# AnnaUshnova/tinyrenderder

Hardware: AMD Instinct MI355X
Metric: triangles/sec (+ Mpixels/sec) at 4096x4096; achieved HBM GB/s vs peak (higher is better)
Workload: dtype f64

## Files before the change

### profiles/summarize_rocprof.py

```python
import csv
import re
import glob
import os
import sys
from collections import defaultdict

out = sys.argv[1]


def short(name):
    m = re.search(r"k_raster<(\d)(?:, (\d))?(?:, (true|false))?>", name)
    if m:
        return "k_raster<" + ["flat", "gouraud", "phong", "eye", "checker", "any"][int(m.group(1))] + (", bpp " + m.group(2) if m.group(2) and m.group(2) != "0" else "") + (", all well scaled" if m.group(3) == "true" else "") + ">"
    m = re.search(r"k_shade<(\d)>", name)
    if m:
        return "k_shade<" + ["flat", "gouraud", "phong", "eye", "checker", "any"][int(m.group(1))] + ">"
    for k in ("k_setup", "k_chunk_spine", "k_radix_scan_rows", "k_expand", "k_radix_hist", "k_radix_scatter",
              "k_bounds", "k_make_items", "k_fold_stats", "k_selftest_division"):
        if k in name:
            return k
    return name.split("(")[0][:60]


print("== kernel trace stats (rocprofv3 --kernel-trace --stats) ==")
def newest(pattern):
    files = sorted(glob.glob(pattern, recursive=True), key=os.path.getmtime)
    return files[-1:]


for f in newest(os.path.join(out, "trace", "**", "*kernel_stats.csv")):
    rows = list(csv.DictReader(open(f)))
    print(f"{'kernel':28s} {'calls':>6s} {'total_ms':>10s} {'avg_us':>10s} {'min_us':>10s} {'max_us':>10s} {'%':>6s}")
    for r in rows:
        print(f"{short(r['Name']):28s} {r['Calls']:>6s} {float(r['TotalDurationNs'])/1e6:10.3f} {float(r['AverageNs'])/1e3:10.1f} "
              f"{float(r['MinNs'])/1e3:10.1f} {float(r['MaxNs'])/1e3:10.1f} {float(r['Percentage']):6.2f}")

for f in newest(os.path.join(out, "trace_writeout", "**", "*kernel_stats.csv")):
    print("\n== write-out-only frames at 4096x4096 (profiles/writeout_probe.py 4096: RGB then RGBA framebuffer, 25 frames each) ==")
    for r in csv.DictReader(open(f)):
        if "k_raster" in r["Name"]:
            avg = float(r["AverageNs"])
            print(f"{short(r['Name']):28s} calls {r['Calls']}  avg {avg/1e3:.1f} us  min {float(r['MinNs'])/1e3:.1f} us  -> "
                  f"{4096*4096*11.5/avg:.0f} GB/s average over RGB (11 B/px) and RGBA (12 B/px) frames = {4096*4096*11.5/avg/8000*100:.1f} % of 8 TB/s")
    log = os.path.join(out, "writeout.log")
    if os.path.exists(log):
        print("\n".join(l for l in open(log).read().splitlines() if l[:1].isdigit()))

for tag in ("pmc_fetch", "pmc_write", "pmc_sq"):
    files = newest(os.path.join(out, tag, "**", "*counter_collection.csv"))
    if not files:
        continue
    acc = defaultdict(lambda: defaultdict(list))
    for f in files:
        for r in csv.DictReader(open(f)):
            acc[short(r["Kernel_Name"])][r["Counter_Name"]].append(float(r["Counter_Value"]))
    print(f"\n== {tag}: per-dispatch mean of each counter ==")
    for k, cs in sorted(acc.items()):
        print(f"{k:28s} " + "  ".join(f"{c}={sum(v)/len(v):.4g} (n={len(v)})" for c, v in sorted(cs.items())))

def per_launch(tag, counter, kernel="k_raster"):
    vals = []
    for f in newest(os.path.join(out, tag, "**", "*counter_collection.csv")):
        for r in csv.DictReader(open(f)):
            if kernel in r["Kernel_Name"] and r["Counter_Name"] == counter:
                vals.append(float(r["Counter_Value"]))
    vals = [v for v in vals if v > 0.2 * max(vals)] if vals else vals
    return sum(vals) / len(vals) if vals else None


fetch, write = per_launch("pmc_fetch", "FETCH_SIZE"), per_launch("pmc_write", "WRITE_SIZE")
if fetch and write:
    import json
    traffic = (2.0 * fetch + write) * 1024.0
    print(f"\n== k_raster HBM traffic per launch: FETCH_SIZE={fetch:.4g} KiB (x2 gfx950 wide-read correction), "
          f"WRITE_SIZE={write:.4g} KiB -> {traffic/1e6:.1f} MB ==")
    json.dump({"workload": "c4_4096x4096_10000000", "round": os.path.basename(os.path.normpath(out)).replace("prof_", ""), "raster_hbm_bytes_per_launch": traffic,
               "fetch_size_kib": fetch, "write_size_kib": write,
               "note": "rocprofv3 --pmc FETCH_SIZE / WRITE_SIZE in separate passes; bytes = (2*FETCH_SIZE + WRITE_SIZE)*1024"},
              open(os.path.join(out, "traffic.json"), "w"), indent=1)
```

### tinyrenderder_amd/csrc/kernels_bin.hip

```cpp
#include <hip/hip_runtime.h>
#include "trgl_device.h"
#include "launch.h"

namespace {

__device__ __forceinline__ double dmin3(double a, double b, double c) { double m = a; if (b < m) m = b; if (c < m) m = c; return m; }
__device__ __forceinline__ double dmax3(double a, double b, double c) { double m = a; if (m < b) m = b; if (m < c) m = c; return m; }
__device__ __forceinline__ double dot4(const double* m, const double* v) {
    double sum = 0;
    sum += m[0] * v[0]; sum += m[1] * v[1]; sum += m[2] * v[2]; sum += m[3] * v[3];
    return sum;
}

__device__ __forceinline__ int wave_min_i(int v) {
    for (int o = 32; o; o >>= 1) { int t = __shfl_xor(v, o); v = t < v ? t : v; }
    return v;
}
__device__ __forceinline__ int wave_max_i(int v) {
    for (int o = 32; o; o >>= 1) { int t = __shfl_xor(v, o); v = t > v ? t : v; }
    return v;
}

constexpr int SETUP_THREADS = 256;

__global__ __launch_bounds__(SETUP_THREADS) void k_setup(FrameParams fp, DrawDesc d, DrawDesc* __restrict__ draws_out, int draw_idx,
                                                         TriRec* __restrict__ recs, TriW* __restrict__ recs_w, uint32_t* __restrict__ cnt,
                                                         uint2* __restrict__ tilebox, DevStats* __restrict__ stats,
                                                         uint32_t* __restrict__ blk_sums, uint32_t blk_base) {
    __shared__ __attribute__((aligned(16))) double s_buf[SETUP_THREADS * 16];
    if (blockIdx.x == 0 && threadIdx.x == 0) draws_out[draw_idx] = d;
    const uint32_t b0 = blockIdx.x * SETUP_THREADS;
    const uint32_t nb = min((uint32_t)SETUP_THREADS, d.n - b0);
    const uint32_t tid = threadIdx.x;
    const uint32_t i = b0 + tid;
    const bool in_range = tid < nb;

    const double* src = d.clip + (size_t)b0 * 12;
    if ((reinterpret_cast<uintptr_t>(src) & 15) == 0) {
        const double2* s2 = reinterpret_cast<const double2*>(src);
        double2* l2 = reinterpret_cast<double2*>(s_buf);
        typedef double f64x2 __attribute__((ext_vector_type(2)));
        for (uint32_t k = tid; k < nb * 6; k += SETUP_THREADS)
            *reinterpret_cast<f64x2*>(&l2[k]) = __builtin_nontemporal_load(reinterpret_cast<const f64x2*>(&s2[k]));
    } else {
        for (uint32_t k = tid; k < nb * 12; k += SETUP_THREADS) s_buf[k] = src[k];
    }
    __syncthreads();
    double v[12];
#pragma unroll
    for (int k = 0; k < 12; ++k) v[k] = in_range ? s_buf[tid * 12 + k] : 0.0;
    __syncthreads();

    int bx0 = INT_MAX, by0 = INT_MAX, bx1 = INT_MIN, by1 = INT_MIN;
    uint32_t ntiles = 0;
    bool large = false;
    uint2 tb = make_uint2(0, 0);
    TriRec r;
    {
        uint4* z4 = reinterpret_cast<uint4*>(&r);
#pragma unroll
        for (int k = 0; k < 8; ++k) z4[k] = make_uint4(0, 0, 0, 0);
    }
    if (in_range) {
        bool ok = !(v[3] <= 1e-12 || v[7] <= 1e-12 || v[11] <= 1e-12);
        double ndc[12];
#pragma unroll
        for (int q = 0; q < 3; ++q) {
#pragma unroll
            for (int k = 0; k < 3; ++k) ndc[4 * q + k] = v[4 * q + k] / v[4 * q + 3];
            ndc[4 * q + 3] = __builtin_isfinite(v[4 * q + 3]) ? 1.0 : __builtin_nan("");
        }
        bool zo0 = (ndc[2] < -1.0 || ndc[2] > 1.0), zo1 = (ndc[6] < -1.0 || ndc[6] > 1.0),
             zo2 = (ndc[10] < -1.0 || ndc[10] > 1.0);
        ok = ok && !(zo0 && zo1 && zo2);
#pragma unroll
        for (int k = 0; k < 12; ++k) ok = ok && __builtin_isfinite(ndc[k]);
        double sx[3], sy[3];
#pragma unroll
        for (int q = 0; q < 3; ++q) { sx[q] = dot4(fp.vp, ndc + 4 * q); sy[q] = dot4(fp.vp + 4, ndc + 4 * q); }
        double e1x = sx[1] - sx[0], e1y = sy[1] - sy[0], e2x = sx[2] - sx[0], e2y = sy[2] - sy[0];
        double cross_product = e1x * e2y - e1y * e2x;
        ok = ok && !(cross_product <= 0);
        int min_x_px = max(0, x86_cvttsd2si(floor(dmin3(sx[0], sx[1], sx[2]))));
        int max_x_px = min(fp.W - 1, x86_cvttsd2si(ceil(dmax3(sx[0], sx[1], sx[2]))));
        int min_y_px = max(0, x86_cvttsd2si(floor(dmin3(sy[0], sy[1], sy[2]))));
        int max_y_px = min(fp.H - 1, x86_cvttsd2si(ceil(dmax3(sy[0], sy[1], sy[2]))));
        ok = ok && !(min_x_px > max_x_px || min_y_px > max_y_px);
        if (ok) {
            bx0 = min_x_px; by0 = min_y_px; bx1 = max_x_px; by1 = max_y_px;
            r.ax = sx[0]; r.ay = sy[0];
            r.s0x = sx[2] - sx[0]; r.s0y = sx[1] - sx[0];
            r.s1x = sy[2] - sy[0]; r.s1y = sy[1] - sy[0];
            r.uz = r.s0x * r.s1y - r.s0y * r.s1x;
            {
                const double BIG = 0x1p200, SMALL = 0x1p-250;
                bool ws = r.uz < 0.0 && !(fabs(r.uz) < 1e-12);
#pragma unroll
                for (int q = 0; q < 3; ++q) ws = ws && fabs(sx[q]) < BIG && fabs(sy[q]) < BIG;
                const double dl[4] = { r.s0x, r.s0y, r.s1x, r.s1y };
#pragma unroll
                for (int q = 0; q < 4; ++q) ws = ws && (dl[q] == 0.0 || fabs(dl[q]) >= SMALL);
                {
                    const double S = (fabs(r.s0x) + fabs(r.s0y)) + (fabs(r.s1x) + fabs(r.s1y));
                    const double rx = fmax(fabs(r.ax - ((double)bx0 + 0.5)), fabs(r.ax - ((double)bx1 + 0.5)));
                    const double ry = fmax(fabs(r.ay - ((double)by0 + 0.5)), fabs(r.ay - ((double)by1 + 0.5)));
                    ws = ws && 0x1p-40 * (S * S) * (rx + ry + 17.0 + S) < fabs(r.uz);
                }
                r.ruz = ws ? 1.0 / r.uz : 0.0;
            }
            r.z0 = ndc[2]; r.z1 = ndc[6]; r.z2 = ndc[10];
            r.bx0 = (uint16_t)bx0; r.by0 = (uint16_t)by0; r.bx1 = (uint16_t)bx1; r.by1 = (uint16_t)by1;
            r.color = d.colors ? d.colors[i] : 0xffffffffu;
            r.dl = ((uint32_t)draw_idx << 24) | i | (r.ruz == 0.0 ? TRGL_DL_LITERAL : 0u);
            r.c0 = -__builtin_inf(); r.g1 = 0.0; r.g2 = 0.0;
            if (r.ruz != 0.0) {
                const double zabs = dmax3(fabs(r.z0), fabs(r.z1), fabs(r.z2));
                const double dz1 = r.z1 - r.z0, dz2 = r.z2 - r.z0;
                const double h1 = (r.s1x * dz1 - r.s1y * dz2) * r.ruz, h2 = (r.s0y * dz2 - r.s0x * dz1) * r.ruz;
                const double rx = fmax(fabs(r.ax - ((double)bx0 + 0.5)), fabs(r.ax - ((double)bx1 + 0.5)));
                const double ry = fmax(fabs(r.ay - ((double)by0 + 0.5)), fabs(r.ay - ((double)by1 + 0.5)));
                const double Ssum = (fabs(r.s0x) + fabs(r.s0y)) + (fabs(r.s1x) + fabs(r.s1y));
                const double R = rx + ry + 1.0 + Ssum;
                const double mz = zabs * 0x1p-39 * (R * Ssum * fabs(r.ruz) + 1.0) + 0x1p-600;
                const bool okp = zabs < 0x1p1000 && R * fabs(h1) < 0x1p900 && R * fabs(h2) < 0x1p900 && mz < 0x1p1000;
                if (okp) { r.c0 = r.z0 - mz; r.g1 = h1; r.g2 = h2; }
            }
            if (d.kind != TRGL_SHADER_FLAT) {
                TriW w;
                w.iw0 = (fabs(v[3]) > 1e-12) ? (1.0 / v[3]) : 0.0;
                w.iw1 = (fabs(v[7]) > 1e-12) ? (1.0 / v[7]) : 0.0;
                w.iw2 = (fabs(v[11]) > 1e-12) ? (1.0 / v[11]) : 0.0;
                w.pad = 0.0;
                recs_w[d.first + i] = w;
            }
            int y_lo = max(by0, fp.strip_y0), y_hi = min(by1, fp.strip_y1 - 1);
            if (!(fabs(r.uz) < 1e-12) && y_lo <= y_hi) {
                uint32_t tx0 = bx0 >> TRGL_TILE_LOG2, tx1 = bx1 >> TRGL_TILE_LOG2;
                uint32_t ty0 = y_lo >> TRGL_TILE_LOG2, ty1 = y_hi >> TRGL_TILE_LOG2;
                const uint32_t rows = fp.il_tiles ? (uint32_t)(il_owned_below(fp, (int)ty1 + 1) - il_owned_below(fp, (int)ty0)) : ty1 - ty0 + 1;
                ntiles = (tx1 - tx0 + 1) * rows;
                tb = make_uint2(((uint32_t)bx0 >> TRGL_BLOCK_LOG2) | (((uint32_t)y_lo >> TRGL_BLOCK_LOG2) << 16),
                                ((uint32_t)bx1 >> TRGL_BLOCK_LOG2) | (((uint32_t)y_hi >> TRGL_BLOCK_LOG2) << 16));
                uint32_t zq = 0;
                if (r.c0 > -__builtin_inf()) {
                    const double zv = dmin3(r.c0, __builtin_fma(-r.s0y, r.g1, __builtin_fma(-r.s1y, r.g2, r.c0)),
                                            __builtin_fma(-r.s0x, r.g1, __builtin_fma(-r.s1x, r.g2, r.c0)));
                    const double t = (zv + 1.0) * 64.0 - 0x1p-20;
                    if (t >= 1.0) zq = t >= 127.0 ? 127u : (uint32_t)x86_cvttsd2si(floor(t));
                }
                tb.x |= (zq & 7u) << 13; tb.y |= ((zq >> 3) & 7u) << 13; tb.y |= (zq >> 6) << 29;
                large = bx1 - bx0 >= 64 || y_hi - y_lo >= 64;
            }
        }
        cnt[d.first + i] = ntiles;
        tilebox[d.first + i] = tb;
    }
    const uint32_t lane = tid & 63, wbase = tid & ~63u;
    {
        uint4* l4 = reinterpret_cast<uint4*>(s_buf);
        const uint4* r4 = reinterpret_cast<const uint4*>(&r);
#pragma unroll
        for (int c = 0; c < 8; ++c) l4[tid * 8 + (c ^ (tid & 7))] = r4[c];
        const unsigned long long keep = __ballot(ntiles != 0);
        __builtin_amdgcn_wave_barrier();
        uint4* dst = reinterpret_cast<uint4*>(recs + d.first + b0 + wbase);
#pragma unroll
        for (int it = 0; it < 8; ++it) {
            const uint32_t k = lane + 64u * it, t = k >> 3, c = k & 7;
            if ((keep >> t) & 1ull) {
                typedef uint32_t u32x4 __attribute__((ext_vector_type(4)));
                __builtin_nontemporal_store(*reinterpret_cast<const u32x4*>(&l4[(wbase + t) * 8 + (c ^ (t & 7))]), reinterpret_cast<u32x4*>(&dst[k]));
            }
        }
    }
    {
        uint32_t ws = ntiles;
        for (int o = 32; o; o >>= 1) ws += __shfl_xor(ws, o);
        __syncthreads();
        uint32_t* s_ws = reinterpret_cast<uint32_t*>(s_buf);
        if (lane == 0) s_ws[tid >> 6] = ws;
        __syncthreads();
        if (tid == 0) blk_sums[blk_base + blockIdx.x] = s_ws[0] + s_ws[1] + s_ws[2] + s_ws[3];
    }
    {
        const unsigned long long lit = __ballot(ntiles != 0 && r.ruz == 0.0);
        if (lit && lane == 0) atomicAdd(&stats->literal_tris, (unsigned long long)__popcll(lit));
        const unsigned long long lrg = __ballot(large);
        if (lrg && lane == 0) atomicAdd(&stats->large_tris, (unsigned long long)__popcll(lrg));
    }
    int wx0 = wave_min_i(bx0), wy0 = wave_min_i(by0), wx1 = wave_max_i(bx1), wy1 = wave_max_i(by1);
    if ((threadIdx.x & 63) == 0 && wx0 != INT_MAX) {
        if (wx0 < __builtin_nontemporal_load(&stats->min_x)) atomicMin(&stats->min_x, wx0);
        if (wy0 < __builtin_nontemporal_load(&stats->min_y)) atomicMin(&stats->min_y, wy0);
        if (wx1 > __builtin_nontemporal_load(&stats->max_x)) atomicMax(&stats->max_x, wx1);
        if (wy1 > __builtin_nontemporal_load(&stats->max_y)) atomicMax(&stats->max_y, wy1);
    }
}

constexpr int SCAN_THREADS = 256;

__device__ __forceinline__ uint32_t wave_incl_scan(uint32_t v) {
    int lane = threadIdx.x & 63;
    for (int o = 1; o < 64; o <<= 1) { uint32_t t = __shfl_up(v, o); if (lane >= o) v += t; }
    return v;
}

__device__ __forceinline__ uint32_t block_excl_scan(uint32_t v, uint32_t* smem , uint32_t* total) {
    uint32_t inc = wave_incl_scan(v);
    int w = threadIdx.x >> 6, lane = threadIdx.x & 63;
    __syncthreads();
    if (lane == 63) smem[w] = inc;
    __syncthreads();
    uint32_t base = 0, tot = 0;
#pragma unroll
    for (int k = 0; k < SCAN_THREADS / 64; ++k) { uint32_t s = smem[k]; if (k < w) base += s; tot += s; }
    *total = tot;
    return base + inc - v;
}

constexpr int EXPAND_CHUNK = 16;

constexpr int SPINE_THREADS = 1024;
__global__ __launch_bounds__(SPINE_THREADS) void k_chunk_spine(const uint32_t* __restrict__ blk_sums, uint32_t nblk,
                                                               uint32_t* __restrict__ chunk_off,
                                                               unsigned long long* __restrict__ total64, unsigned long long* __restrict__ host_copy,
                                                               uint4* __restrict__ zero16, uint32_t n_zero16) {
    __shared__ unsigned long long s_wave[SPINE_THREADS / 64];
    for (uint32_t k = threadIdx.x; k < n_zero16; k += SPINE_THREADS) zero16[k] = make_uint4(0, 0, 0, 0);
    const uint32_t nchunks = (nblk + EXPAND_CHUNK - 1) / EXPAND_CHUNK;
    const int lane = threadIdx.x & 63, w = threadIdx.x >> 6;
    unsigned long long running = 0;
    for (uint32_t start = 0; start < nchunks; start += SPINE_THREADS) {
        const uint32_t c = start + threadIdx.x;
        unsigned long long v = 0;
        if (c < nchunks) {
            const uint32_t q0 = c * EXPAND_CHUNK;
            if (q0 + EXPAND_CHUNK <= nblk) {
                const uint4* p4 = reinterpret_cast<const uint4*>(blk_sums + q0);
#pragma unroll
                for (int k = 0; k < EXPAND_CHUNK / 4; ++k) { const uint4 t = p4[k]; v += (unsigned long long)t.x + t.y + t.z + t.w; }
            } else {
                for (uint32_t q = q0; q < nblk; ++q) v += blk_sums[q];
            }
        }
        unsigned long long inc = v;
        for (int o = 1; o < 64; o <<= 1) { const unsigned long long t = __shfl_up(inc, o); if (lane >= o) inc += t; }
        if (lane == 63) s_wave[w] = inc;
        __syncthreads();
        unsigned long long base = 0, tot = 0;
#pragma unroll
        for (int k = 0; k < SPINE_THREADS / 64; ++k) { const unsigned long long t = s_wave[k]; if (k < w) base += t; tot += t; }
        if (c < nchunks) chunk_off[c] = (uint32_t)(running + base + inc - v);
        running += tot;
        __syncthreads();
    }
    if (threadIdx.x == 0) {
        *total64 = running;
        host_copy[0] = running; host_copy[1] = total64[1]; host_copy[2] = total64[2];
        __threadfence_system();
    }
}

constexpr uint32_t EXPAND_STAGE = 3072;
__device__ __forceinline__ uint32_t tile_block_mask(uint32_t tx, uint32_t ty, uint32_t qx0, uint32_t qy0, uint32_t qx1, uint32_t qy1) {
    const uint32_t c0 = qx0 > 4 * tx ? qx0 - 4 * tx : 0u, c1 = qx1 < 4 * tx + 3 ? qx1 - 4 * tx : 3u;
    const uint32_t r0 = qy0 > 4 * ty ? qy0 - 4 * ty : 0u, r1 = qy1 < 4 * ty + 3 ? qy1 - 4 * ty : 3u;
    return (((2u << c1) - (1u << c0)) & 0xfu) * 0x1111u & ((0xffffu >> (12 - 4 * r1)) & (0xffffu << (4 * r0)));
}
template <typename K>
__global__ __launch_bounds__(256) void k_expand(FrameParams fp, uint32_t first, uint32_t n, int tiles_x, const uint32_t* __restrict__ cnt,
                                                const uint32_t* __restrict__ blk_sums, const uint32_t* __restrict__ chunk_off,
                                                uint32_t blk_base, const uint2* __restrict__ tilebox,
                                                K* __restrict__ keys, uint32_t* __restrict__ vals, uint16_t* __restrict__ bmask,
                                                const unsigned long long* __restrict__ pairs_total, uint32_t cap) {
    __shared__ uint32_t smem[4];
    __shared__ uint32_t s_v[EXPAND_STAGE];
    __shared__ K s_k[EXPAND_STAGE];
    __shared__ uint16_t s_m[EXPAND_STAGE];
    if (*pairs_total > cap) return;
    const uint32_t local = blockIdx.x * blockDim.x + threadIdx.x;
    const uint32_t i = first + local;
    const uint32_t blk = blk_base + blockIdx.x;
    uint32_t c = 0; uint2 tb = make_uint2(0, 0);
    if (local < n) { c = cnt[i]; if (c) tb = tilebox[i]; }
    uint32_t base;
    {
        const uint32_t q0 = blk - blk % EXPAND_CHUNK, l = threadIdx.x & 63u;
        uint32_t part = l < blk - q0 ? blk_sums[q0 + l] : 0u;
        for (int o = 8; o; o >>= 1) part += __shfl_xor(part, o);
        base = chunk_off[blk / EXPAND_CHUNK] + (uint32_t)__builtin_amdgcn_readfirstlane((int)part);
    }
    uint32_t tot;
    const uint32_t o = block_excl_scan(c, smem, &tot);
    const bool staged = tot <= EXPAND_STAGE;
    K* const kdst = keys + base; uint32_t* const vdst = vals + base; uint16_t* const mdst = bmask + base;
    constexpr uint32_t SMALL = 8;
    if (c && c <= SMALL) {
        const uint32_t qx0 = tb.x & 0x1fff, qy0 = (tb.x >> 16) & 0x1fff, qx1 = tb.y & 0x1fff, qy1 = (tb.y >> 16) & 0x1fff;
        const uint32_t iz = i | ((((tb.x >> 13) & 7u) | (((tb.y >> 13) & 7u) << 3) | ((tb.y >> 29) << 6)) << 25);
        const uint32_t tx0 = qx0 >> 2, ty0 = qy0 >> 2, tx1 = qx1 >> 2;
        uint32_t tx = tx0, row = 0;
        uint32_t ty = fp.il_tiles ? (uint32_t)il_nth_owned_from(fp, (int)ty0, 0) : ty0;
        for (uint32_t k = 0; k < c; ++k) {
            const K key = (K)(ty * tiles_x + tx);
            const uint16_t m = (uint16_t)tile_block_mask(tx, ty, qx0, qy0, qx1, qy1);
            if (staged) { s_k[o + k] = key; s_v[o + k] = iz; s_m[o + k] = m; } else { kdst[o + k] = key; vdst[o + k] = iz; mdst[o + k] = m; }
            if (++tx > tx1) { tx = tx0; ++row; ty = fp.il_tiles ? (uint32_t)il_nth_owned_from(fp, (int)ty0, (int)row) : ty0 + row; }
        }
    }
    unsigned long long big = __ballot(c > SMALL);
    int lane = threadIdx.x & 63;
    while (big) {
        int src = __ffsll((long long)big) - 1;
        big &= big - 1;
        uint32_t cc = __shfl(c, src), oo = __shfl(o, src), ii = __shfl(i, src);
        uint32_t bx = __shfl(tb.x, src), by = __shfl(tb.y, src);
        const uint32_t qx0 = bx & 0x1fff, qy0 = (bx >> 16) & 0x1fff, qx1 = by & 0x1fff, qy1 = (by >> 16) & 0x1fff;
        ii |= (((bx >> 13) & 7u) | (((by >> 13) & 7u) << 3) | ((by >> 29) << 6)) << 25;
        uint32_t tx0 = qx0 >> 2, ty0 = qy0 >> 2, tx1 = qx1 >> 2;
        uint32_t wdt = tx1 - tx0 + 1;
        for (uint32_t k = lane; k < cc; k += 64) {
            uint32_t ty = fp.il_tiles ? (uint32_t)il_nth_owned_from(fp, (int)ty0, (int)(k / wdt)) : ty0 + k / wdt, tx = tx0 + k % wdt;
            const K key = (K)(ty * tiles_x + tx);
            const uint16_t m = (uint16_t)tile_block_mask(tx, ty, qx0, qy0, qx1, qy1);
            if (staged) { s_k[oo + k] = key; s_v[oo + k] = ii; s_m[oo + k] = m; } else { kdst[oo + k] = key; vdst[oo + k] = ii; mdst[oo + k] = m; }
        }
    }
    if (staged) {
        __syncthreads();
        for (uint32_t j = threadIdx.x; j < tot; j += 256) { kdst[j] = s_k[j]; vdst[j] = s_v[j]; mdst[j] = s_m[j]; }
    }
}

constexpr int RADIX_CHUNK = 4096;
constexpr int RADIX_WAVE_CHUNK = RADIX_CHUNK / 4;
constexpr int RADIX_ROUNDS = RADIX_WAVE_CHUNK / 64;
constexpr int RADIX_MAX_BITS = 8;

template <typename K> __device__ __forceinline__ void load4(const K* __restrict__ keys, uint64_t p, uint32_t k[4]);
template <> __device__ __forceinline__ void load4<uint32_t>(const uint32_t* __restrict__ keys, uint64_t p, uint32_t k[4]) {
    const uint4 q = *reinterpret_cast<const uint4*>(keys + p);
    k[0] = q.x; k[1] = q.y; k[2] = q.z; k[3] = q.w;
}
template <> __device__ __forceinline__ void load4<uint16_t>(const uint16_t* __restrict__ keys, uint64_t p, uint32_t k[4]) {
    const uint2 q = *reinterpret_cast<const uint2*>(keys + p);
    k[0] = q.x & 0xffffu; k[1] = q.x >> 16; k[2] = q.y & 0xffffu; k[3] = q.y >> 16;
}

template <typename K>
__global__ __launch_bounds__(256) void k_radix_hist(const K* __restrict__ keys, const unsigned long long* __restrict__ pairs_total,
                                                    uint32_t cap, int shift, int bits,
                                                    uint32_t nblocks, uint32_t* __restrict__ hist) {
    __shared__ uint32_t s_cnt[1 << RADIX_MAX_BITS];
    const unsigned long long P64 = *pairs_total;
    const uint32_t P = P64 > cap ? 0u : (uint32_t)P64;
    const uint32_t nb = 1u << bits, mask = nb - 1;
    for (uint32_t b = threadIdx.x; b < nb; b += 256) s_cnt[b] = 0;
    __syncthreads();
    const uint64_t beg = (uint64_t)blockIdx.x * RADIX_CHUNK;
    uint64_t end = beg + RADIX_CHUNK; if (end > P) end = P;
    for (uint64_t p = beg + 4u * threadIdx.x; p < end; p += 1024) {
        uint32_t k[4];
        load4<K>(keys, p, k);
#pragma unroll
        for (int q = 0; q < 4; ++q) if (p + q < end) atomicAdd(&s_cnt[(k[q] >> shift) & mask], 1u);
    }
    __syncthreads();
    for (uint32_t b = threadIdx.x; b < nb; b += 256) hist[(size_t)b * nblocks + blockIdx.x] = s_cnt[b];
}

constexpr int ROWSCAN_THREADS = 1024, ROWSCAN_PER = 8;
__global__ __launch_bounds__(ROWSCAN_THREADS) void k_radix_scan_rows(uint32_t* __restrict__ hist, uint32_t nblocks, uint32_t* __restrict__ totals) {
    __shared__ uint32_t s_wave[ROWSCAN_THREADS / 64];
    uint32_t* row = hist + (size_t)blockIdx.x * nblocks;
    const int lane = threadIdx.x & 63, w = threadIdx.x >> 6;
    uint32_t running = 0;
    for (uint32_t start = 0; start < nblocks; start += ROWSCAN_THREADS * ROWSCAN_PER) {
        const uint32_t base = start + threadIdx.x * ROWSCAN_PER;
        uint32_t v[ROWSCAN_PER], sum = 0;
#pragma unroll
        for (int k = 0; k < ROWSCAN_PER; ++k) { v[k] = (base + k < nblocks) ? row[base + k] : 0; sum += v[k]; }
        uint32_t inc = sum;
        for (int o = 1; o < 64; o <<= 1) { const uint32_t t = __shfl_up(inc, o); if (lane >= o) inc += t; }
        if (lane == 63) s_wave[w] = inc;
        __syncthreads();
        uint32_t wbase = 0, tot = 0;
#pragma unroll
        for (int k = 0; k < ROWSCAN_THREADS / 64; ++k) { const uint32_t t = s_wave[k]; if (k < w) wbase += t; tot += t; }
        uint32_t run = running + wbase + inc - sum;
#pragma unroll
        for (int k = 0; k < ROWSCAN_PER; ++k) { if (base + k < nblocks) row[base + k] = run; run += v[k]; }
        running += tot;
        __syncthreads();
    }
    if (threadIdx.x == 0) totals[blockIdx.x] = running;
}

template <typename K>
__global__ __launch_bounds__(256) void k_radix_scatter(const K* __restrict__ keys_in, const uint32_t* __restrict__ vals_in,
                                                       const uint16_t* __restrict__ msk_in,
                                                       const unsigned long long* __restrict__ pairs_total, uint32_t cap,
                                                       int shift, int bits, uint32_t nblocks,
                                                       const uint32_t* __restrict__ base, const uint32_t* __restrict__ totals,
                                                       K* __restrict__ keys_out, uint32_t* __restrict__ vals_out, uint16_t* __restrict__ msk_out) {
    __shared__ uint32_t s_cnt[4][1 << RADIX_MAX_BITS];
    __shared__ uint32_t s_start[1 << RADIX_MAX_BITS];
    __shared__ uint32_t s_gbase[1 << RADIX_MAX_BITS];
    __shared__ uint32_t s_val[RADIX_CHUNK];
    __shared__ K s_key[RADIX_CHUNK];
    __shared__ uint16_t s_msk[RADIX_CHUNK];
    const int w = threadIdx.x >> 6, lane = threadIdx.x & 63;
    const unsigned long long P64 = *pairs_total;
    const uint32_t P = P64 > cap ? 0u : (uint32_t)P64;
    if ((uint64_t)blockIdx.x * RADIX_CHUNK >= P) return;
    const uint32_t nb = 1u << bits, mask = nb - 1;
    for (uint32_t b = threadIdx.x; b < nb; b += 256) {
        s_cnt[0][b] = 0; s_cnt[1][b] = 0; s_cnt[2][b] = 0; s_cnt[3][b] = 0;
        s_gbase[b] = base[(size_t)b * nblocks + blockIdx.x];
    }
    if (w == 0) {
        uint32_t tot[4], run = 0;
#pragma unroll
        for (int q = 0; q < 4; ++q) { const uint32_t d = lane * 4 + q; tot[q] = d < nb ? totals[d] : 0; run += tot[q]; }
        uint32_t inc = run;
        for (int o = 1; o < 64; o <<= 1) { const uint32_t t = __shfl_up(inc, o); if (lane >= o) inc += t; }
        uint32_t ex = inc - run;
#pragma unroll
        for (int q = 0; q < 4; ++q) { const uint32_t d = lane * 4 + q; if (d < nb) s_start[d] = ex; ex += tot[q]; }
    }
    __syncthreads();
    for (uint32_t b = threadIdx.x; b < nb; b += 256) s_gbase[b] += s_start[b];
    __syncthreads();
    const uint64_t cbeg = (uint64_t)blockIdx.x * RADIX_CHUNK;
    uint64_t cend = cbeg + RADIX_CHUNK; if (cend > P) cend = P;
    const uint32_t n_chunk = (uint32_t)(cend - cbeg);
    const uint64_t wbeg = cbeg + (uint64_t)w * RADIX_WAVE_CHUNK;
    const unsigned long long lt = (1ull << lane) - 1ull;

    uint32_t k[RADIX_ROUNDS], v[RADIX_ROUNDS], rk[RADIX_ROUNDS];
    uint16_t mk[RADIX_ROUNDS];
#pragma unroll
    for (int r = 0; r < RADIX_ROUNDS; ++r) {
        const uint64_t p = wbeg + (uint64_t)r * 64 + lane;
        const bool act = p < cend;
        k[r] = act ? (uint32_t)keys_in[p] : 0; v[r] = act ? vals_in[p] : 0; mk[r] = act ? msk_in[p] : (uint16_t)0;
    }
#pragma unroll
    for (int r = 0; r < RADIX_ROUNDS; ++r) {
        const bool act = wbeg + (uint64_t)r * 64 + lane < cend;
        const uint32_t dgt = (k[r] >> shift) & mask;
        unsigned long long same = __ballot(act);
        for (int b = 0; b < bits; ++b) {
            const unsigned long long bal = __ballot((dgt >> b) & 1u);
            same &= ((dgt >> b) & 1u) ? bal : ~bal;
        }
        const uint32_t cur = act ? s_cnt[w][dgt] : 0;
        __builtin_amdgcn_wave_barrier();
        const uint32_t r_in = __popcll(same & lt);
        rk[r] = cur + r_in;
        if (act && r_in == 0) s_cnt[w][dgt] = cur + (uint32_t)__popcll(same);
        __builtin_amdgcn_wave_barrier();
    }
    __syncthreads();
    if (w == 0) {
        uint32_t tot[4], run = 0;
#pragma unroll
        for (int q = 0; q < 4; ++q) {
            const uint32_t d = lane * 4 + q;
            tot[q] = d < nb ? s_cnt[0][d] + s_cnt[1][d] + s_cnt[2][d] + s_cnt[3][d] : 0;
            run += tot[q];
        }
        uint32_t inc = run;
        for (int o = 1; o < 64; o <<= 1) { const uint32_t t = __shfl_up(inc, o); if (lane >= o) inc += t; }
        uint32_t ex = inc - run;
#pragma unroll
        for (int q = 0; q < 4; ++q) { const uint32_t d = lane * 4 + q; if (d < nb) s_start[d] = ex; ex += tot[q]; }
    }
    __syncthreads();
    for (uint32_t d = threadIdx.x; d < nb; d += 256) {
        uint32_t run = s_start[d];
#pragma unroll
        for (int ww = 0; ww < 4; ++ww) { const uint32_t c = s_cnt[ww][d]; s_cnt[ww][d] = run; run += c; }
    }
    __syncthreads();
#pragma unroll
    for (int r = 0; r < RADIX_ROUNDS; ++r) {
        if (wbeg + (uint64_t)r * 64 + lane < cend) {
            const uint32_t dgt = (k[r] >> shift) & mask;
            const uint32_t lp = s_cnt[w][dgt] + rk[r];
            s_key[lp] = (K)k[r]; s_val[lp] = v[r]; s_msk[lp] = mk[r];
        }
    }
    __syncthreads();
    for (uint32_t i = threadIdx.x; i < n_chunk; i += 256) {
        const uint32_t key = s_key[i];
        const uint32_t dgt = (key >> shift) & mask;
        const uint32_t dst = s_gbase[dgt] + (i - s_start[dgt]);
        keys_out[dst] = (K)key; vals_out[dst] = s_val[i]; msk_out[dst] = s_msk[i];
    }
}

template <typename K>
__global__ __launch_bounds__(256) void k_bounds(const K* __restrict__ keys, const unsigned long long* __restrict__ pairs_total, uint32_t cap,
                                                uint32_t* __restrict__ tile_start, uint32_t* __restrict__ tile_end) {
    const unsigned long long P64 = *pairs_total;
    const uint32_t P = P64 > cap ? 0u : (uint32_t)P64;
    const uint32_t p0 = (blockIdx.x * blockDim.x + threadIdx.x) * 4u;
    if (p0 >= P) return;
    uint32_t k[4];
    load4<K>(keys, p0, k);
    uint32_t prev = p0 ? (uint32_t)keys[p0 - 1] : 0u;
    const uint32_t after = (p0 + 4 < P) ? (uint32_t)keys[p0 + 4] : 0u;
#pragma unroll
    for (int i = 0; i < 4; ++i) {
        const uint32_t p = p0 + (uint32_t)i;
        if (p < P) {
            const uint32_t next = i < 3 ? k[i + 1] : after;
            if (p == 0 || prev != k[i]) tile_start[k[i]] = p;
            if (p == P - 1 || next != k[i]) tile_end[k[i]] = p + 1;
        }
        prev = k[i];
    }
}

}

namespace trgl {

uint32_t setup_num_blocks(uint32_t n) { return (n + SETUP_THREADS - 1) / SETUP_THREADS; }

void launch_setup(hipStream_t s, const FrameParams& fp, const DrawDesc& draw, DrawDesc* draws_dev, int draw_idx, uint32_t n,
                  TriRec* recs, TriW* recs_w, uint32_t* cnt, uint2* tilebox, DevStats* stats, uint32_t* blk_sums, uint32_t blk_base) {
    if (!n) return;
    hipLaunchKernelGGL(k_setup, dim3(setup_num_blocks(n)), dim3(SETUP_THREADS), 0, s, fp, draw, draws_dev, draw_idx, recs, recs_w, cnt, tilebox,
                       stats, blk_sums, blk_base);
}

void launch_chunk_spine(hipStream_t s, const uint32_t* blk_sums, uint32_t nblk, uint32_t* chunk_off, unsigned long long* total64, unsigned long long* host_copy,
                        void* zero, size_t zero_bytes) {
    hipLaunchKernelGGL(k_chunk_spine, dim3(1), dim3(SPINE_THREADS), 0, s, blk_sums, nblk, chunk_off, total64, host_copy, (uint4*)zero, (uint32_t)(zero_bytes / 16));
}

void launch_expand(hipStream_t s, const FrameParams& fp, uint32_t first, uint32_t n, int tiles_x, const uint32_t* cnt, const uint32_t* blk_sums,
                   const uint32_t* chunk_off, uint32_t blk_base, const uint2* tilebox, void* keys, bool key16, uint32_t* vals, uint16_t* bmask,
                   const unsigned long long* pairs_total, uint32_t cap) {
    if (!n) return;
    if (key16)
        hipLaunchKernelGGL(k_expand<uint16_t>, dim3(setup_num_blocks(n)), dim3(SETUP_THREADS), 0, s, fp, first, n, tiles_x, cnt, blk_sums, chunk_off,
                           blk_base, tilebox, (uint16_t*)keys, vals, bmask, pairs_total, cap);
    else
        hipLaunchKernelGGL(k_expand<uint32_t>, dim3(setup_num_blocks(n)), dim3(SETUP_THREADS), 0, s, fp, first, n, tiles_x, cnt, blk_sums, chunk_off,
                           blk_base, tilebox, (uint32_t*)keys, vals, bmask, pairs_total, cap);
}

uint32_t radix_num_workers(uint32_t P) { return (uint32_t)(((uint64_t)P + RADIX_CHUNK - 1) / RADIX_CHUNK); }

template <typename K>
static void radix_pass_t(hipStream_t s, const K* keys_in, const uint32_t* vals_in, const uint16_t* msk_in, K* keys_out, uint32_t* vals_out, uint16_t* msk_out,
                         const unsigned long long* pairs_total, uint32_t cap, int shift, int bits, uint32_t* hist, uint32_t* scan_tmp) {
    uint32_t nblk = radix_num_workers(cap);
    hipLaunchKernelGGL(k_radix_hist<K>, dim3(nblk), dim3(256), 0, s, keys_in, pairs_total, cap, shift, bits, nblk, hist);
    hipLaunchKernelGGL(k_radix_scan_rows, dim3(1u << bits), dim3(ROWSCAN_THREADS), 0, s, hist, nblk, scan_tmp);
    hipLaunchKernelGGL(k_radix_scatter<K>, dim3(nblk), dim3(256), 0, s, keys_in, vals_in, msk_in, pairs_total, cap, shift, bits, nblk, hist, scan_tmp,
                       keys_out, vals_out, msk_out);
}

void launch_radix_pass(hipStream_t s, const void* keys_in, const uint32_t* vals_in, const uint16_t* msk_in, void* keys_out,
                       uint32_t* vals_out, uint16_t* msk_out, bool key16, const unsigned long long* pairs_total, uint32_t cap, int shift, int bits,
                       uint32_t* hist, uint32_t* scan_tmp) {
    if (!cap) return;
    if (key16) radix_pass_t<uint16_t>(s, (const uint16_t*)keys_in, vals_in, msk_in, (uint16_t*)keys_out, vals_out, msk_out, pairs_total, cap, shift, bits, hist, scan_tmp);
    else radix_pass_t<uint32_t>(s, (const uint32_t*)keys_in, vals_in, msk_in, (uint32_t*)keys_out, vals_out, msk_out, pairs_total, cap, shift, bits, hist, scan_tmp);
}

void launch_bounds(hipStream_t s, const void* keys, bool key16, const unsigned long long* pairs_total, uint32_t cap,
                   uint32_t* tile_start, uint32_t* tile_end) {
    if (!cap) return;
    if (key16) hipLaunchKernelGGL(k_bounds<uint16_t>, dim3((unsigned)(((uint64_t)cap + 1023) / 1024)), dim3(256), 0, s, (const uint16_t*)keys, pairs_total, cap, tile_start, tile_end);
    else hipLaunchKernelGGL(k_bounds<uint32_t>, dim3((unsigned)(((uint64_t)cap + 1023) / 1024)), dim3(256), 0, s, (const uint32_t*)keys, pairs_total, cap, tile_start, tile_end);
}

}
```

### tinyrenderder_amd/csrc/kernels_raster.hip

```cpp
#include <hip/hip_runtime.h>
#include "trgl_device.h"
#include "launch.h"
#include "shade_common.h"

namespace {
using namespace trgl_shade;

__device__ __forceinline__ double vmax(double a, double b) { double r; asm("v_max_f64 %0, %1, %2" : "=v"(r) : "v"(a), "v"(b)); return r; }
__device__ __forceinline__ double vmin(double a, double b) { double r; asm("v_min_f64 %0, %1, %2" : "=v"(r) : "v"(a), "v"(b)); return r; }
__device__ __forceinline__ float fmin3(float a, float b, float c) { float r; asm("v_min3_f32 %0, %1, %2, %3" : "=v"(r) : "v"(a), "v"(b), "v"(c)); return r; }
__device__ __forceinline__ float fmax2(float a, float b) { float r; asm("v_max_f32 %0, %1, %2" : "=v"(r) : "v"(a), "v"(b)); return r; }
__device__ __forceinline__ float wave_max_f32(float v) {
    float t;
    asm volatile("s_nop 1\n\tv_max_f32_dpp %0, %1, %1 quad_perm:[1,0,3,2] row_mask:0xf bank_mask:0xf" : "=&v"(t) : "v"(v)); v = t;
    asm volatile("s_nop 1\n\tv_max_f32_dpp %0, %1, %1 quad_perm:[2,3,0,1] row_mask:0xf bank_mask:0xf" : "=&v"(t) : "v"(v)); v = t;
    asm volatile("s_nop 1\n\tv_max_f32_dpp %0, %1, %1 row_half_mirror row_mask:0xf bank_mask:0xf" : "=&v"(t) : "v"(v)); v = t;
    asm volatile("s_nop 1\n\tv_max_f32_dpp %0, %1, %1 row_mirror row_mask:0xf bank_mask:0xf" : "=&v"(t) : "v"(v)); v = t;
    asm volatile("s_nop 1\n\tv_max_f32_dpp %0, %1, %1 row_bcast:15 row_mask:0xa bank_mask:0xf" : "=&v"(t) : "v"(v), "0"(v)); v = t;
    asm volatile("s_nop 1\n\tv_max_f32_dpp %0, %1, %1 row_bcast:31 row_mask:0xc bank_mask:0xf" : "=&v"(t) : "v"(v), "0"(v)); v = t;
    return __builtin_bit_cast(float, __builtin_amdgcn_readlane(__builtin_bit_cast(int, v), 63));
}
__device__ __forceinline__ float f32_up(double d) {
    float f = (float)d;
    if ((double)f < d) { const uint32_t b = __float_as_uint(f); f = __uint_as_float((b >> 31) ? b - 1u : b + 1u); }
    return f;
}
__device__ __forceinline__ float f32_down(double d) {
    float f = (float)d;
    if ((double)f > d) { const uint32_t b = __float_as_uint(f); f = __uint_as_float((b >> 31) ? b + 1u : b - 1u); }
    return f;
}
__device__ __forceinline__ double dot3(const double* a, const double* b) {
    double sum = 0; sum += a[0] * b[0]; sum += a[1] * b[1]; sum += a[2] * b[2]; return sum;
}
__device__ __forceinline__ void normalized3(const double* v, double* out) {
    double length = sqrt(dot3(v, v));
    if (length == 0) { out[0] = v[0]; out[1] = v[1]; out[2] = v[2]; return; }
    out[0] = v[0] / length; out[1] = v[1] / length; out[2] = v[2] / length;
}

__device__ __forceinline__ void interp(const double* v0, const double* v1, const double* v2, const double* b, int n, double* out) {
    for (int i = 0; i < n; ++i) out[i] = (v0[i] * b[0] + v1[i] * b[1]) + v2[i] * b[2];
}
__device__ __forceinline__ double spec_pow(double x, double y) {
    return (y == 1.0) ? x : pow(x, y);
}

template <class UN, class TX>
__device__ __forceinline__ Color frag_phong(const UN& u, TX tx, const double* vary, const double* b) {
    const double* uvv = vary; const double* pos = vary + 6; const double* nrm = vary + 15;
    double position_eye[3], geometry_normal[3], uv[2];
    interp(pos, pos + 3, pos + 6, b, 3, position_eye);
    interp(nrm, nrm + 3, nrm + 6, b, 3, geometry_normal);
    interp(uvv, uvv + 2, uvv + 4, b, 2, uv);

    const TX td = tex_slot(tx, u.tex_diffuse);
    const TX ts = tex_slot(tx, u.tex_specular);
    const TX tn = tex_slot(tx, u.tex_normal);
    uint32_t raw_d = 0, raw_s = 0, raw_n = 0;
    if (td) raw_d = tex_fetch_raw(td, uv);
    if (ts) raw_s = tex_fetch_raw(ts, uv);
    if (tn) raw_n = tex_fetch_raw(tn, uv);
    Color base = td ? Color{ raw_d & tex_mask(td), td->bpp } : Color{ 0xffffffffu, 4 };
    float specf = ts ? (float)(int)(raw_s & 0xff) / 255.0f : 1.0f;
    double specular_power = dmax(1.0, (double)specf);

    int bsum = (int)(base.bgra & 0xff) + (int)((base.bgra >> 8) & 0xff) + (int)((base.bgra >> 16) & 0xff);
    double brightness = bsum / (3.0 * 255.0);
    bool is_eye_pixel = (brightness >= 0.85) && (specular_power <= 5.0);

    double nmv[3] = { 0, 0, 1 };
    if (tn) {
        const uint32_t c = raw_n & tex_mask(tn);
        double n[3];
        n[0] = (double)((c >> 16) & 0xff) / 255.0 * 2.0 - 1.0;
        n[1] = (double)((c >> 8) & 0xff) / 255.0 * 2.0 - 1.0;
        n[2] = (double)(c & 0xff) / 255.0 * 2.0 - 1.0;
        normalized3(n, nmv);
    }
    double nme[3];
    for (int r = 0; r < 3; ++r) {
        const auto* m = u.model_view + 4 * r;
        double sum = 0; sum += m[0] * nmv[0]; sum += m[1] * nmv[1]; sum += m[2] * nmv[2]; sum += m[3] * 0.0;
        nme[r] = sum;
    }
    double N[3];
    if (is_eye_pixel) { N[0] = geometry_normal[0]; N[1] = geometry_normal[1]; N[2] = geometry_normal[2]; }
    else {
        double s = u.normal_map_strength, mix[3];
        for (int i = 0; i < 3; ++i) mix[i] = geometry_normal[i] * (1.0 - s) + nme[i] * s;
        normalized3(mix, N);
    }
    double negp[3], V[3];
    for (int i = 0; i < 3; ++i) negp[i] = position_eye[i] * -1.0;
    normalized3(negp, V);

    const double Lk[3] = { u.key_light_dir_eye[0], u.key_light_dir_eye[1], u.key_light_dir_eye[2] };
    double key_diffuse = dmax(0.0, dot3(N, Lk)) * 1.0;
    double k2 = 2.0 * dot3(N, Lk), rr[3], R[3];
    for (int i = 0; i < 3; ++i) rr[i] = N[i] * k2 - Lk[i];
    normalized3(rr, R);
    double rvd = dmax(0.0, dot3(R, V));
    double key_specular = (rvd > 0.0 ? spec_pow(rvd, specular_power) : 0.0) * 1.0;
    const double Lf[3] = { u.fill_light_dir_eye[0], u.fill_light_dir_eye[1], u.fill_light_dir_eye[2] };
    double fill_diffuse = dmax(0.0, dot3(N, Lf)) * 0.35;
    const double Lr[3] = { u.rim_light_dir_eye[0], u.rim_light_dir_eye[1], u.rim_light_dir_eye[2] };
    double rim_diffuse = dmax(0.0, dot3(N, Lr)) * 0.6;
    double total_diffuse = key_diffuse + fill_diffuse + rim_diffuse;
    double total_specular = key_specular;
    double ambient = 0.10;

    uint32_t out = base.bgra & 0xff000000u;
    for (int ch = 0; ch < 3; ++ch) {
        double channel_value = (double)((base.bgra >> (8 * ch)) & 0xff);
        double final_value = channel_value * (ambient + total_diffuse) + 255.0 * (0.35 * total_specular);
        out |= (uint32_t)(unsigned char)dmin(255.0, final_value) << (8 * ch);
    }
    return Color{ out, base.bytespp };
}

template <class UN, class TX>
__device__ __forceinline__ Color frag_eye(const UN& u, TX tx, const double* vary, const double* b) {
    const double* uvv = vary; const double* pos = vary + 6; const double* nrm = vary + 15;
    double position_eye[3], ni[3], N[3], uv[2];
    interp(pos, pos + 3, pos + 6, b, 3, position_eye);
    interp(nrm, nrm + 3, nrm + 6, b, 3, ni);
    normalized3(ni, N);
    interp(uvv, uvv + 2, uvv + 4, b, 2, uv);

    const TX td = tex_slot(tx, u.tex_diffuse);
    const TX ts = tex_slot(tx, u.tex_specular);
    uint32_t raw_d = 0, raw_s = 0;
    if (td) raw_d = tex_fetch_raw(td, uv);
    if (ts) raw_s = tex_fetch_raw(ts, uv);
    Color base = td ? Color{ raw_d & tex_mask(td), td->bpp } : Color{ 0xffffffffu, 4 };
    double negp[3], V[3];
    for (int i = 0; i < 3; ++i) negp[i] = position_eye[i] * -1.0;
    normalized3(negp, V);

    const double Lk[3] = { u.key_light_dir_eye[0], u.key_light_dir_eye[1], u.key_light_dir_eye[2] };
    double key_diffuse = dmax(0.0, dot3(N, Lk)) * 1.0;
    const double Lr[3] = { u.rim_light_dir_eye[0], u.rim_light_dir_eye[1], u.rim_light_dir_eye[2] };
    double rim_diffuse = dmax(0.0, dot3(N, Lr)) * 0.6;
    double total_diffuse = key_diffuse + rim_diffuse;

    float specf = ts ? (float)(int)(raw_s & 0xff) / 255.0f : 1.0f;
    double specular_power = dmax(1.0, (double)specf) * 8.0;
    double k2 = 2.0 * dot3(N, Lk), rr[3], R[3];
    for (int i = 0; i < 3; ++i) rr[i] = N[i] * k2 - Lk[i];
    normalized3(rr, R);
    double rvd = dmax(0.0, dot3(R, V));
    double specular = (rvd > 0.0 ? spec_pow(rvd, specular_power) : 0.0);

    uint32_t out = base.bgra & 0xff000000u;
    for (int ch = 0; ch < 3; ++ch) {
        double channel_value = (double)((base.bgra >> (8 * ch)) & 0xff);
        double final_value = channel_value * (0.1 + total_diffuse) + 255.0 * (1.5 * specular);
        out |= (uint32_t)(unsigned char)dmin(255.0, final_value) << (8 * ch);
    }
    return Color{ out, base.bytespp };
}

__device__ __forceinline__ uint32_t frag_gouraud(uint32_t base, const double* vary, const double* b) {
    double id = (vary[0] * b[0] + vary[1] * b[1]) + vary[2] * b[2];
    float intensity = (float)id;
    if (intensity < 0.f) intensity = 0.f;
    if (intensity > 1.f) intensity = 1.f;
    uint32_t out = 0;
    for (int i = 0; i < 4; ++i) {
        float c = (float)(int)((base >> (8 * i)) & 0xff) * intensity;
        out |= (uint32_t)(uint8_t)c << (8 * i);
    }
    return out;
}


__device__ __forceinline__ bool frag_checker_discards(int cells, const double* b) {
    const int a = x86_cvttsd2si(b[0] * (double)cells), c = x86_cvttsd2si(b[1] * (double)cells);
    return ((a ^ c) & 1) != 0;
}

constexpr int KIND_ANY = TRGL_NUM_SHADERS;
constexpr int RING = 512;

#ifdef TRGL_DEBUG_COUNTERS
#define TRGL_DBG(i, n) do { S.dbg[i] += (unsigned long long)(n); } while (0)
#ifdef TRGL_DEBUG_NOSTAMP
#define TRGL_STAMP(i) ((void)0)
#else
#define TRGL_STAMP(i) do { const unsigned long long t_ = __builtin_amdgcn_s_memtime(); S.dbg[i] += t_ - S.t_prev; S.t_prev = t_; } while (0)
#endif
#else
#define TRGL_DBG(i, n) ((void)0)
#define TRGL_STAMP(i) ((void)0)
#endif

typedef const __attribute__((address_space(4))) TriRec CRec;
typedef unsigned short us2 __attribute__((ext_vector_type(2)));

struct TriScan {
    double ax, ay, s0x, s0y, s1x, s1y, c0, uz, g1, g2;
    uint32_t bx, by;
    uint32_t color, dl;
    double ruz, z0, z1, z2;
    typedef uint32_t u32x16 __attribute__((ext_vector_type(16)));
    u32x16 lo, hi;
};
__device__ __forceinline__ TriScan load_scan(const TriRec* __restrict__ recs, uint32_t tri) {
    TriScan T;
#ifdef TRGL_EXP_SAMEREC
    tri &= 63u;
#endif
#if __HIP_DEVICE_COMPILE__
    TriScan::u32x16 g, h;
    asm volatile("s_load_dwordx16 %0, %2, %3 offset:0x0\n\ts_load_dwordx16 %1, %2, %3 offset:0x40" : "=&s"(g), "=&s"(h) : "s"(recs), "s"(tri << 7));
    T.lo = g; T.hi = h;
#ifdef TRGL_DEBUG_COUNTERS
    asm volatile("s_waitcnt lgkmcnt(0)" : "+s"(T.lo), "+s"(T.hi) :: "memory");
    g = T.lo; h = T.hi;
#endif
    auto dg = [&](int i) { return __builtin_bit_cast(double, ((unsigned long long)g[i + 1] << 32) | g[i]); };
    auto dh = [&](int i) { return __builtin_bit_cast(double, ((unsigned long long)h[i + 1] << 32) | h[i]); };
    T.ax = dg(0); T.ay = dg(2); T.s0x = dg(4); T.s0y = dg(6); T.s1x = dg(8); T.s1y = dg(10); T.c0 = dg(12); T.uz = dg(14);
    T.g1 = dh(0); T.g2 = dh(2); T.ruz = dh(4); T.z0 = dh(6); T.z1 = dh(8); T.z2 = dh(10);
    T.bx = h[12]; T.by = h[13]; T.color = h[14]; T.dl = h[15];
#endif
    return T;
}
__device__ __forceinline__ void scan_wait(const TriScan& T) { asm volatile("s_waitcnt lgkmcnt(0)" :: "s"(T.lo), "s"(T.hi) : "memory"); }

struct BlockState {
    double z;
    uint32_t color;
    uint32_t id;
    double pxc, pyc;
    double pux, puy; uint32_t ptri;
    double puz, pruz, pz0, pz1, pz2;
    uint32_t pcd;
    uint32_t frags; double zmax;
    us2 xy;
#ifdef TRGL_DEBUG_COUNTERS
    unsigned long long dbg[16];
    unsigned long long t_prev;
#endif
};

template <int KIND, bool ALLWS, bool DEFERRED>
__device__ __forceinline__ void resolve(BlockState& S, unsigned long long pend, const TriRec* __restrict__ recs, const TriW* __restrict__ recs_w,
                                        const DrawDesc* __restrict__ draws, DevStats* __restrict__ stats, bool zero_locked) {
    TRGL_DBG(6, 1); TRGL_DBG(7, __popcll(pend));
#ifdef TRGL_DEBUG_COUNTERS
    const unsigned long long t_res = __builtin_amdgcn_s_memtime();
#endif
    constexpr bool PLAIN = KIND == TRGL_SHADER_FLAT || KIND == TRGL_SHADER_PHONG || KIND == TRGL_SHADER_EYE;
    if (__builtin_amdgcn_inverse_ballot_w64(pend)) {
        const double uz = S.puz, ruz = S.pruz, z0 = S.pz0, z1 = S.pz1, z2 = S.pz2;
        const double ux = S.pux, uy = S.puy, us = ux + uy;
        double b0, b1, b2;
        if (ALLWS || ruz != 0.0) {
            b0 = 1.0 - div_by_uz(us, uz, ruz);
            b1 = div_by_uz(uy, uz, ruz);
            b2 = div_by_uz(ux, uz, ruz);
        } else {
            b0 = 1.0 - us / uz;
            b1 = uy / uz;
            b2 = ux / uz;
        }
        const double z = b0 * z0 + b1 * z1 + b2 * z2;
        if (__builtin_isfinite(z) && (z < S.z)) {
            uint32_t color = S.pcd, id = 0xffffffffu;
            bool discard = false;
            if (KIND == TRGL_SHADER_PHONG || KIND == TRGL_SHADER_EYE) id = TRGL_DL_ID(S.pcd);
            if (!PLAIN) {
                const uint32_t dl = S.pcd;
                color = recs[S.ptri].color;
                const DrawDesc* d = draws + TRGL_DL_DRAW(dl);
                const int kind = KIND == KIND_ANY ? d->kind : KIND;
                if (kind == TRGL_SHADER_PHONG || kind == TRGL_SHADER_EYE || kind >= TRGL_SHADER_USER_FIRST) {
                    id = TRGL_DL_ID(dl);
                } else if (kind != TRGL_SHADER_FLAT) {
                    const TriW w = recs_w[S.ptri];
                    double pc[3];
                    const double denom = b0 * w.iw0 + b1 * w.iw1 + b2 * w.iw2;
                    if (fabs(denom) < 1e-15) { pc[0] = b0; pc[1] = b1; pc[2] = b2; }
                    else { pc[0] = (b0 * w.iw0) / denom; pc[1] = (b1 * w.iw1) / denom; pc[2] = (b2 * w.iw2) / denom; }
                    if (kind == TRGL_SHADER_GOURAUD) {
                        const double* vary = d->vary + (size_t)TRGL_DL_LOCAL(dl) * 3;
                        const double vv[3] = { vary[0], vary[1], vary[2] };
                        color = frag_gouraud(color, vv, pc);
                    } else {
                        discard = frag_checker_discards(d->u.reserved, pc);
                    }
                }
            }
            if (!discard) {
                asm volatile(
                    "v_mov_b64 %[sz], %[z]\n\t"
                    "v_add_u32 %[fr], 1, %[fr]\n\t"
                    "v_max_f64 %[zmax], %[zmax], %[z]"
                    : [sz] "+v"(S.z), [fr] "+v"(S.frags), [zmax] "+v"(S.zmax)
                    : [z] "v"(z));
                if (KIND == TRGL_SHADER_PHONG || KIND == TRGL_SHADER_EYE) {
                    asm volatile("v_mov_b32 %0, %1" : "+v"(S.id) : "v"(id));
                } else {
                    const uint32_t ncol = (!DEFERRED || id == 0xffffffffu) ? color : S.color;
                    asm volatile("v_mov_b32 %0, %1" : "+v"(S.color) : "v"(ncol));
                    if (DEFERRED) asm volatile("v_mov_b32 %0, %1" : "+v"(S.id) : "v"(id));
                }
                TRGL_DBG(8, 1);
                if (z == 0.0 && !zero_locked) {
                    const uint32_t xy = __builtin_bit_cast(uint32_t, S.xy);
                    unsigned long long order = ((unsigned long long)S.ptri << 32) | ((unsigned long long)(xy & 0xffffu) << 16) | (unsigned long long)(xy >> 16);
                    atomicMin(__builtin_signbit(z) ? &stats->zero_neg_key : &stats->zero_pos_key, order);
                }
            }
        }
    }
#if defined(TRGL_DEBUG_COUNTERS) && !defined(TRGL_DEBUG_NOSTAMP)
    S.dbg[14] += __builtin_amdgcn_s_memtime() - t_res;
#endif
}

#ifndef TRGL_RASTER_WAVES
#define TRGL_RASTER_WAVES 5
#endif

template <int KIND, int BPP = 0, bool ALLWS = false>
__global__ __launch_bounds__(256) __attribute__((amdgpu_waves_per_eu(TRGL_RASTER_WAVES, 8))) void k_raster(FrameParams fp, const TriRec* __restrict__ recs, const TriW* __restrict__ recs_w,
                                                const uint32_t* __restrict__ vals, const uint16_t* __restrict__ bmask,
                                                const uint32_t* __restrict__ tile_start,
                                                const uint32_t* __restrict__ tile_end,
                                                const DrawDesc* __restrict__ draws, DevStats* __restrict__ stats,
                                                const uint4* __restrict__ items, const uint32_t* __restrict__ n_items,
                                                unsigned long long* __restrict__ item_stats) {
    constexpr bool DEFERRED = KIND == TRGL_SHADER_PHONG || KIND == TRGL_SHADER_EYE || KIND == KIND_ANY;
    __shared__ uint32_t s_ring[4][RING];
    __shared__ uint32_t s_out[4][64];
    const int lane = threadIdx.x & 63;
    const int w = __builtin_amdgcn_readfirstlane(threadIdx.x >> 6);
    const uint32_t G = n_items[0];
    const uint32_t per = (G + 7u) >> 3, xj = blockIdx.x >> 3;
    const uint32_t g = (blockIdx.x & 7u) * per + xj;
    if (xj >= per || g >= G) return;
    const uint4 item4 = items[g];
    const uint32_t item = item4.x;
    const int t = (int)(item & 0xffffffu);
    const int tile_y = t / fp.tiles_x, tile_x = t - tile_y * fp.tiles_x;
    const int px0 = tile_x << TRGL_TILE_LOG2, py0 = tile_y << TRGL_TILE_LOG2;
    unsigned long long* my_stats = item_stats + (size_t)g * 4;
    if (item & TRGL_ITEM_CLEAR) {
        const int ya = max(py0 + 8 * w, fp.strip_y0), yb = min(min(py0 + 8 * w + 7, fp.H - 1), fp.strip_y1 - 1);
        if (ya <= yb) clear_rows(fp, lane, px0, ya, yb);
        if (threadIdx.x == 0) {
            ulonglong2* dst = reinterpret_cast<ulonglong2*>(my_stats);
            dst[0] = make_ulonglong2(0ull, ~0ull); dst[1] = make_ulonglong2(0ull, 0ull);
        }
        return;
    }
    const int brow = (int)((item >> 24) & 3u);
    const int kblk = 4 * brow + w;
    const int X0 = px0 + 8 * w, Y0 = py0 + 8 * brow;

    BlockState S;
    const int lx = X0 + (lane & 7), ly = Y0 + (lane >> 3);
    S.xy = __builtin_bit_cast(us2, (uint32_t)lx | ((uint32_t)ly << 16));
    const bool owned = lx < fp.W && ly < fp.H && ly >= fp.strip_y0 && ly < fp.strip_y1;
    const size_t pix = (size_t)lx + (size_t)ly * fp.W;
    S.pxc = (double)lx + 0.5; S.pyc = (double)ly + 0.5;
    S.z = -__builtin_inf();
    if (owned) S.z = fp.init_from_clear ? fp.clear_z : fp.zb[pix];
    S.color = fp.clear_color;
    S.id = 0xffffffffu;
    S.pux = 0.0; S.puy = 0.0; S.ptri = 0;
    S.puz = -1.0; S.pruz = -1.0; S.pz0 = 0.0; S.pz1 = 0.0; S.pz2 = 0.0; S.pcd = 0;
    S.frags = 0; S.zmax = -__builtin_inf();
    const bool zero_locked = stats->zero_locked != 0;
#ifdef TRGL_DEBUG_COUNTERS
    for (int k = 0; k < 16; ++k) S.dbg[k] = 0;
    S.t_prev = __builtin_amdgcn_s_memtime();
#endif
    unsigned long long pend = 0;

    const uint32_t beg = item4.y, end = item4.z;
    uint32_t* ring = s_ring[w];
    uint32_t head = 0, cnt = 0;
    uint32_t pn = 0, ptri = 0;
    double2 pq0 = make_double2(0, 0), pq1 = pq0, pq2 = pq0, pq3 = pq0, pq4 = pq0;
    uint4 pq5 = make_uint4(0, 0, 0, 0);
    auto visit = [&](const TriScan& T, uint32_t tcur) {
        auto note = [&](unsigned long long m, double ux, double uy) {
            unsigned long long sv;
            asm volatile("s_mov_b64 %[sv], exec\n\ts_mov_b64 exec, %[m]\n\tv_mov_b64 %[px], %[ux]\n\tv_mov_b64 %[py], %[uy]\n\t"
                         "v_mov_b32 %[pt], %[t]\n\tv_mov_b64 %[puz], %[uz]\n\tv_mov_b64 %[pruz], %[ruz]\n\t"
                         "v_mov_b64 %[pz0], %[z0]\n\tv_mov_b64 %[pz1], %[z1]\n\tv_mov_b64 %[pz2], %[z2]\n\tv_mov_b32 %[pcd], %[cd]\n\ts_mov_b64 exec, %[sv]"
                         : [px] "+v"(S.pux), [py] "+v"(S.puy), [pt] "+v"(S.ptri), [sv] "=&s"(sv),
                           [puz] "+v"(S.puz), [pruz] "+v"(S.pruz), [pz0] "+v"(S.pz0), [pz1] "+v"(S.pz1), [pz2] "+v"(S.pz2), [pcd] "+v"(S.pcd)
                         : [ux] "v"(ux), [uy] "v"(uy), [t] "s"(tcur), [m] "s"(m), [cd] "s"(KIND == TRGL_SHADER_FLAT ? T.color : T.dl),
                           [uz] "s"(T.uz), [ruz] "s"(T.ruz), [z0] "s"(T.z0), [z1] "s"(T.z1), [z2] "s"(T.z2));
        };
        double ux, uy;
        unsigned long long cm;
        unsigned long long both, sv, sx;
#ifdef TRGL_DEBUG_COUNTERS
        unsigned long long am = 0;
#endif
        const uint32_t ext = T.by - T.bx;
        if (ALLWS || !(T.dl & TRGL_DL_LITERAL)) {
            double s0z, s1z, ta, tb2;
#ifdef TRGL_DEBUG_COUNTERS
            am = __ballot(__builtin_bit_cast(uint32_t, __builtin_elementwise_max(S.xy - __builtin_bit_cast(us2, T.bx), __builtin_bit_cast(us2, ext))) == ext);
#endif
            asm volatile(
                "v_add_f64 %[s0z], %[ax], -%[pxc]\n\t"
                "v_add_f64 %[s1z], %[ay], -%[pyc]\n\t"
                "v_mov_b64 %[ta], %[c0]\n\t"
                "v_fmac_f64 %[ta], %[g2], %[s1z]\n\t"
                "v_fmac_f64 %[ta], %[g1], %[s0z]\n\t"
                "v_cmp_nge_f64_e32 vcc, %[ta], %[z]\n\t"
#ifdef TRGL_DEBUG_COUNTERS
                "s_mov_b64 %[cm], 0\n\t"
#endif
                "s_cbranch_vccz .Lvisit_end%=\n\t"
                "v_mul_f64 %[ta], %[s0y], %[s1z]\n\t"
                "v_mul_f64 %[tb], %[s1y], %[s0z]\n\t"
                "v_add_f64 %[ux], %[ta], -%[tb]\n\t"
                "v_mul_f64 %[ta], %[s1x], %[s0z]\n\t"
                "v_mul_f64 %[tb], %[s0x], %[s1z]\n\t"
                "v_add_f64 %[uy], %[ta], -%[tb]\n\t"
                "v_add_f64 %[ta], %[ux], %[uy]\n\t"
                "v_max_f64 %[tb], %[ux], %[uy]\n\t"
                "v_cmp_nlt_f64_e64 %[cm], %[ta], %[uz]\n\t"
                "s_and_b64 %[cm], %[cm], vcc\n\t"
                "v_cmp_nlt_f64_e32 vcc, 0, %[tb]\n\t"
                "s_and_b64 %[cm], %[cm], vcc\n\t"
                "s_cbranch_scc0 .Lvisit_end%=\n\t"
                "s_andn2_b64 %[sv], %[cm], %[pend]\n\t"
                "s_cbranch_scc0 .Lvisit_noted%=\n\t"
                "s_mov_b64 %[sx], exec\n\t"
                "s_mov_b64 exec, %[sv]\n\t"
                "v_mov_b64 %[pux], %[ux]\n\t"
                "v_mov_b64 %[puy], %[uy]\n\t"
                "v_mov_b32 %[ptri], %[tcur]\n\t"
                "v_mov_b64 %[puz], %[uz]\n\t"
                "v_mov_b64 %[pruz], %[ruz]\n\t"
                "v_mov_b64 %[pz0], %[z0]\n\t"
                "v_mov_b64 %[pz1], %[z1]\n\t"
                "v_mov_b64 %[pz2], %[z2]\n\t"
                "v_mov_b32 %[pcd], %[cd]\n\t"
                "s_mov_b64 exec, %[sx]\n"
                ".Lvisit_noted%=:\n\t"
                "s_or_b64 %[pend], %[pend], %[cm]\n\t"
                "s_xor_b64 %[both], %[cm], %[sv]\n\t"
                "s_branch .Lvisit_done%=\n"
                ".Lvisit_end%=:\n\t"
                "s_mov_b64 %[both], 0\n"
                ".Lvisit_done%=:"
                : [cm] "=&s"(cm), [ux] "=&v"(ux), [uy] "=&v"(uy), [s0z] "=&v"(s0z), [s1z] "=&v"(s1z), [ta] "=&v"(ta), [tb] "=&v"(tb2),
                  [both] "=&s"(both), [sv] "=&s"(sv), [sx] "=&s"(sx), [pend] "+s"(pend), [pux] "+v"(S.pux), [puy] "+v"(S.puy), [ptri] "+v"(S.ptri),
                  [puz] "+v"(S.puz), [pruz] "+v"(S.pruz), [pz0] "+v"(S.pz0), [pz1] "+v"(S.pz1), [pz2] "+v"(S.pz2), [pcd] "+v"(S.pcd)
                : [pxc] "v"(S.pxc), [pyc] "v"(S.pyc), [z] "v"(S.z), [tcur] "s"(tcur),
                  [ax] "s"(T.ax), [ay] "s"(T.ay), [c0] "s"(T.c0), [g1] "s"(T.g1), [g2] "s"(T.g2),
                  [s0x] "s"(T.s0x), [s0y] "s"(T.s0y), [s1x] "s"(T.s1x), [s1y] "s"(T.s1y), [uz] "s"(T.uz),
                  [ruz] "s"(T.ruz), [z0] "s"(T.z0), [z1] "s"(T.z1), [z2] "s"(T.z2), [cd] "s"(KIND == TRGL_SHADER_FLAT ? T.color : T.dl)
                : "vcc", "scc");
        } else {
            const us2 off = S.xy - __builtin_bit_cast(us2, T.bx);
            const bool act = __builtin_bit_cast(uint32_t, __builtin_elementwise_max(off, __builtin_bit_cast(us2, ext))) == ext;
            const double s0z = T.ax - S.pxc, s1z = T.ay - S.pyc;
            const double zpl = __builtin_fma(s0z, T.g1, __builtin_fma(s1z, T.g2, T.c0));
            ux = T.s0y * s1z - s0z * T.s1y;
            uy = s0z * T.s1x - T.s0x * s1z;
            const double us = ux + uy;
            const double b0 = 1.0 - us / T.uz, b1 = uy / T.uz, b2 = ux / T.uz;
            cm = __ballot(act && !(zpl >= S.z) && !(b0 < 0 || b1 < 0 || b2 < 0));
#ifdef TRGL_DEBUG_COUNTERS
            am = __ballot(act);
#endif
            both = cm & pend;
            note(cm & ~pend, ux, uy);
            pend |= cm;
        }
        TRGL_DBG(2, tcur < fp.n_tris ? 1 : 0); TRGL_DBG(3, __popcll(am)); TRGL_DBG(4, cm ? 1 : 0); TRGL_DBG(5, __popcll(cm));
        if (both) {
            resolve<KIND, ALLWS, DEFERRED>(S, pend, recs, recs_w, draws, stats, zero_locked);
            note(both, ux, uy);
            asm volatile("s_mov_b64 %0, %1" : "+s"(pend) : "s"(both));
        }
    };
    const uint32_t p_first = beg & ~3u;
    auto load_step = [&](uint32_t p0, uint4& tri4, uint2& m) {
        const uint32_t pl = p0 + 4u * (uint32_t)lane, p = min(pl, (end - 1u) & ~3u);
        tri4 = *reinterpret_cast<const uint4*>(vals + p);
        m = *reinterpret_cast<const uint2*>(bmask + p);
    };
    uint4 tri_n = make_uint4(0, 0, 0, 0); uint2 m_n = make_uint2(0, 0);
    if (beg < end) load_step(p_first, tri_n, m_n);
    for (uint32_t p0 = p_first; p0 < end; p0 += 256) {
        const uint4 tri_c = tri_n; const uint2 m_c = m_n;
        TRGL_STAMP(10);
        load_step(p0 + 256, tri_n, m_n);
        {
            uint32_t c0 = (m_c.x >> kblk) & 1u, c1 = (m_c.x >> (16 + kblk)) & 1u, c2 = (m_c.y >> kblk) & 1u, c3 = (m_c.y >> (16 + kblk)) & 1u;
            if (p0 < beg || p0 + 256u > end) {
                const uint32_t pl = p0 + 4u * (uint32_t)lane;
                const uint32_t lo = min(beg - min(pl, beg), 4u), hi = min(end - min(pl, end), 4u);
                const uint32_t v = (0xfu << lo) & (0xfu >> (4u - hi));
                c0 &= v; c1 &= v >> 1; c2 &= v >> 2; c3 &= v >> 3;
            }
            if (fp.zq_cull) {
                const float zmb = wave_max_f32(f32_up(S.z));
                const float tq = (zmb + 1.0f) * 64.0f + 0x1p-10f;
                const uint32_t qb = !(tq < 128.0f) ? 128u : (tq <= 1.0f ? 1u : (uint32_t)__builtin_ceilf(tq));
                c0 = TRGL_VAL_ZQ(tri_c.x) < qb ? c0 : 0u; c1 = TRGL_VAL_ZQ(tri_c.y) < qb ? c1 : 0u;
                c2 = TRGL_VAL_ZQ(tri_c.z) < qb ? c2 : 0u; c3 = TRGL_VAL_ZQ(tri_c.w) < qb ? c3 : 0u;
            }
            const unsigned long long b0 = __ballot(c0), b1 = __ballot(c1), b2 = __ballot(c2), b3 = __ballot(c3);
            if (b0 | b1 | b2 | b3) {
                uint32_t pos = head + cnt;
                pos += __builtin_amdgcn_mbcnt_hi((uint32_t)(b0 >> 32), __builtin_amdgcn_mbcnt_lo((uint32_t)b0, 0u));
                pos += __builtin_amdgcn_mbcnt_hi((uint32_t)(b1 >> 32), __builtin_amdgcn_mbcnt_lo((uint32_t)b1, 0u));
                pos += __builtin_amdgcn_mbcnt_hi((uint32_t)(b2 >> 32), __builtin_amdgcn_mbcnt_lo((uint32_t)b2, 0u));
                pos += __builtin_amdgcn_mbcnt_hi((uint32_t)(b3 >> 32), __builtin_amdgcn_mbcnt_lo((uint32_t)b3, 0u));
                if (c0) ring[pos & (RING - 1)] = tri_c.x;
                pos += c0;
                if (c1) ring[pos & (RING - 1)] = tri_c.y;
                pos += c1;
                if (c2) ring[pos & (RING - 1)] = tri_c.z;
                pos += c2;
                if (c3) ring[pos & (RING - 1)] = tri_c.w;
#ifdef TRGL_DEBUG_COUNTERS
                {
                    const uint32_t trs[4] = { tri_c.x, tri_c.y, tri_c.z, tri_c.w };
                    const uint32_t cs[4] = { c0, c1, c2, c3 };
                    for (int j = 0; j < 4; ++j)
                        if (cs[j] && TRGL_VAL_TRI(trs[j]) >= fp.n_tris && atomicCAS(&stats->dbg[10], 0ull, 1ull) == 0ull) {
                            stats->dbg[11] = ((unsigned long long)(p0 + 4u * (uint32_t)lane + (uint32_t)j) << 32) | trs[j];
                            stats->dbg[12] = ((unsigned long long)beg << 32) | end;
                            stats->dbg[13] = ((unsigned long long)(uint32_t)t << 32) | (uint32_t)kblk;
                        }
                }
#endif
                const uint32_t added = (uint32_t)(__popcll(b0) + __popcll(b1) + __popcll(b2) + __popcll(b3));
                cnt += added;
                TRGL_DBG(0, added);
            }
        }
        const bool last = p0 + 256 >= end;
        TRGL_STAMP(11);
        for (;;) {
            const bool can = cnt >= 64 || (last && cnt);
            bool keep = false;
            if (pn) {
                if (!can && !last) break;
                const double zmaxb = (double)wave_max_f32(f32_up(S.z));
                keep = (uint32_t)lane < pn;
#ifdef TRGL_DEBUG_COUNTERS
                if (keep && ptri >= fp.n_tris) { atomicAdd(&stats->dbg[9], 1ull); keep = false; }
#endif
                if (keep) {
                    const double2 q0 = pq0, q1 = pq1, q2 = pq2, q3 = pq3, q4 = pq4;
                    const uint4 q5 = pq5;
                    if (ALLWS || !(q5.w & TRGL_DL_LITERAL)) {
                        const double ax = q0.x, ay = q0.y, s0x = q1.x, s0y = q1.y, s1x = q2.x, s1y = q2.y, c0 = q3.x, uz = q3.y, g1 = q4.x, g2 = q4.y;
                        const int bx0 = (int)(q5.x & 0xffffu), by0 = (int)(q5.x >> 16), bx1 = (int)(q5.y & 0xffffu), by1 = (int)(q5.y >> 16);
                        const int xl = max(bx0, X0), xr = min(bx1, X0 + 7), yl = max(by0, Y0), yr = min(by1, Y0 + 7);
                        const double xm = __builtin_fma((double)(xl + xr), 0.5, 0.5), xh = (double)(xr - xl) * 0.5;
                        const double ym = __builtin_fma((double)(yl + yr), 0.5, 0.5), yh = (double)(yr - yl) * 0.5;
                        const double dxm = ax - xm, dym = ay - ym;
                        const double uxc = s0y * dym - dxm * s1y;
                        const double uyc = dxm * s1x - s0x * dym;
                        const double gx = s1y - s1x, gy = s0x - s0y;
                        const double sp1 = __builtin_fma(fabs(s1y), xh, fabs(s0y) * yh);
                        const double sp2 = __builtin_fma(fabs(s1x), xh, fabs(s0x) * yh);
                        const double sp3 = __builtin_fma(fabs(gx), xh, fabs(gy) * yh);
                        const double R = ((fabs(dxm) + xh) + (fabs(dym) + yh)) + 16.0;
                        const double ma = 0x1p-40 * ((fabs(s0y) + fabs(s1y)) * R) + 0x1p-1000;
                        const double mb = 0x1p-40 * ((fabs(s0x) + fabs(s1x)) * R) + 0x1p-1000;
                        const double zpl = __builtin_fma(dxm, g1, __builtin_fma(dym, g2, c0)) - __builtin_fma(fabs(g1), xh, fabs(g2) * yh);
                        const double zv = vmin(vmin(c0, __builtin_fma(-s0y, g1, __builtin_fma(-s1y, g2, c0))), __builtin_fma(-s0x, g1, __builtin_fma(-s1x, g2, c0)));
                        if (uxc - sp1 > ma || uyc - sp2 > mb || (uxc + uyc) + sp3 < uz - (ma + mb) || vmax(zpl, zv) >= zmaxb) keep = false;
                    }
                }
            } else if (!can) break;
            const unsigned long long surv = __ballot(keep);
            const uint32_t tri = ptri;
            TRGL_DBG(1, __popcll(surv));
            TRGL_STAMP(12);
            if (can) {
                const uint32_t n = cnt < 64 ? cnt : 64;
                __builtin_amdgcn_wave_barrier();
                ptri = TRGL_VAL_TRI(ring[(head + lane) & (RING - 1)]);
                __builtin_amdgcn_wave_barrier();
                head += n; cnt -= n; pn = n;
                if ((uint32_t)lane < n
#ifdef TRGL_DEBUG_COUNTERS
                    && ptri < fp.n_tris
#endif
                    ) {
                    const double2* q = reinterpret_cast<const double2*>(recs + ptri);
                    pq0 = q[0]; pq1 = q[1]; pq2 = q[2]; pq3 = q[3]; pq4 = q[4];
                    pq5 = reinterpret_cast<const uint4*>(q)[7];
                }
            } else pn = 0;
            if (surv) {
                const uint32_t ns = (uint32_t)__popcll(surv);
                uint32_t* comp = s_out[w];
                if (keep) comp[__builtin_amdgcn_mbcnt_hi((uint32_t)(surv >> 32), __builtin_amdgcn_mbcnt_lo((uint32_t)surv, 0u))] = tri;
                __builtin_amdgcn_wave_barrier();
                uint32_t tri_s = comp[lane];
                if ((uint32_t)lane >= ns) tri_s = fp.n_tris;
                uint32_t i = 0;
                uint32_t ta = (uint32_t)__builtin_amdgcn_readlane((int)tri_s, 0), tb;
                TriScan A = load_scan(recs, ta), B;
                scan_wait(A);
                do {
                    tb = (uint32_t)__builtin_amdgcn_readlane((int)tri_s, (int)(i + 1u));
                    B = load_scan(recs, tb);
                    __builtin_amdgcn_sched_barrier(0);
                    visit(A, ta);
                    __builtin_amdgcn_sched_barrier(0);
                    scan_wait(B);
                    ta = (uint32_t)__builtin_amdgcn_readlane((int)tri_s, (int)(i + 2u));
                    A = load_scan(recs, ta);
                    __builtin_amdgcn_sched_barrier(0);
                    visit(B, tb);
                    __builtin_amdgcn_sched_barrier(0);
                    scan_wait(A);
                    i += 2;
                } while (i < ns);
            }
            TRGL_STAMP(13);
        }
    }
    if (pend) resolve<KIND, ALLWS, DEFERRED>(S, pend, recs, recs_w, draws, stats, zero_locked);

    TRGL_STAMP(13);
    if (owned) __builtin_nontemporal_store(S.z, &fp.zb[pix]);
    if (DEFERRED && fp.idbuf && owned) fp.idbuf[pix] = S.id;
    {
        const int bpp = BPP ? BPP : fp.bpp;
        const bool whole = fp.init_from_clear && X0 + 7 < fp.W;
        if (bpp == 4) {
            if (owned && (fp.init_from_clear || S.frags)) *reinterpret_cast<uint32_t*>(fp.fb + pix * 4) = S.color;
        } else if (bpp == 3 && whole) {
            uint32_t* so = s_out[w];
            so[lane] = S.color;
            __builtin_amdgcn_wave_barrier();
            const int r = lane >> 3, dw = lane & 7;
            if (dw < 6) {
                const int y = Y0 + r;
                if (y < fp.H && y >= fp.strip_y0 && y < fp.strip_y1) {
                    const int p0 = (4 * dw) / 3, sh = (4 * dw) % 3;
                    const uint32_t ca = so[8 * r + p0] & 0xffffffu, cb2 = so[8 * r + p0 + 1] & 0xffffffu;
                    const unsigned long long bytes = ((unsigned long long)ca | ((unsigned long long)cb2 << 24)) >> (8 * sh);
                    uint32_t* dst = reinterpret_cast<uint32_t*>(fp.fb + ((size_t)X0 + (size_t)y * fp.W) * 3) + dw;
                    *dst = (uint32_t)bytes;
                }
            }
        } else {
            if (owned && (fp.init_from_clear || S.frags)) {
                uint8_t* dst = fp.fb + pix * bpp;
                if (bpp == 3) { *reinterpret_cast<uint16_t*>(dst) = (uint16_t)S.color; dst[2] = (uint8_t)(S.color >> 16); }
                else dst[0] = (uint8_t)S.color;
            }
        }
    }

    TRGL_STAMP(15);
    {
        unsigned long long* red = reinterpret_cast<unsigned long long*>(ring);
        red[lane] = zkey(S.frags ? S.z : __builtin_inf());
        red[64 + lane] = zkey(S.zmax);
        ring[256 + lane] = S.frags;
    }
#ifdef TRGL_DEBUG_COUNTERS
    for (int o = 32; o; o >>= 1) S.dbg[8] += __shfl_xor(S.dbg[8], o);
    if (lane == 0) for (int k = 0; k < 16; ++k) if (S.dbg[k]) atomicAdd(&stats->dbg[k], S.dbg[k]);
#endif
    __syncthreads();
    if (w == 0) {
        unsigned long long frags = 0, kmin = ~0ull, kmax = 0ull;
        for (int k = 0; k < 4; ++k) {
            const unsigned long long* red = reinterpret_cast<const unsigned long long*>(s_ring[k]);
            const unsigned long long a = red[lane], b = red[64 + lane];
            frags += s_ring[k][256 + lane]; kmin = a < kmin ? a : kmin; kmax = b > kmax ? b : kmax;
        }
        for (int o = 32; o; o >>= 1) {
            frags += __shfl_xor(frags, o);
            unsigned long long a = __shfl_xor(kmin, o); kmin = a < kmin ? a : kmin;
            unsigned long long b = __shfl_xor(kmax, o); kmax = b > kmax ? b : kmax;
        }
        if (lane == 0) {
            ulonglong2* dst = reinterpret_cast<ulonglong2*>(my_stats);
            dst[0] = make_ulonglong2(frags, kmin);
            dst[1] = make_ulonglong2(kmax, 0ull);
        }
    }
}

template <int KIND>
__global__ __launch_bounds__(256) __attribute__((amdgpu_waves_per_eu(4, 4))) void k_shade(FrameParams fp, const TriRec* __restrict__ recs, const TriW* __restrict__ recs_w,
                                                const DrawDesc* __restrict__ draws,
                                                const DevTexture* __restrict__ tex, const uint4* __restrict__ items,
                                                const uint32_t* __restrict__ n_items) {
    const int lane = threadIdx.x & 63;
    const uint32_t item_idx = blockIdx.x;
    if (item_idx >= *n_items) return;
    const uint32_t item = items[item_idx].x;
    if (item & TRGL_ITEM_CLEAR) return;
    const int t = (int)(item & 0xffffffu);
    const int tile_y = t / fp.tiles_x, tile_x = t - tile_y * fp.tiles_x;
    const int x = (tile_x << TRGL_TILE_LOG2) + 8 * (int)(threadIdx.x >> 6) + (lane & 7);
    const int y = (tile_y << TRGL_TILE_LOG2) + 8 * (int)((item >> 24) & 3u) + (lane >> 3);
    const bool mine = x < fp.W && y < fp.H && y >= fp.strip_y0 && y < fp.strip_y1;
    const size_t idx = (size_t)x + (size_t)y * fp.W;
    const uint32_t dl = mine ? fp.idbuf[idx] : 0xffffffffu;
    if (dl == 0xffffffffu) return;
    uint32_t color = 0;
    bool user = false;
    typedef const __attribute__((address_space(4))) DrawDesc CDrawK;
    unsigned long long todo = __ballot(true);
    while (todo) {
        const int src = __builtin_ctzll(todo);
        const uint32_t di = (uint32_t)__builtin_amdgcn_readlane((int)(dl >> 24), src);
        const bool here = (dl >> 24) == di;
        todo &= ~__ballot(here);
        if (KIND == KIND_ANY && here && ((CDrawK*)draws)[di].kind >= TRGL_SHADER_USER_FIRST) {
            user = true;
        } else if (here) {
            typedef const __attribute__((address_space(4))) DrawDesc CDraw;
            typedef const __attribute__((address_space(4))) DevTexture CTex;
            const uint32_t di_s = (uint32_t)__builtin_amdgcn_readfirstlane((int)(dl >> 24));
            CDraw& d = ((CDraw*)draws)[di_s];
            CTex* const ctex = (CTex*)tex;
            const uint32_t local = dl & 0xffffffu;
            const TriRec& r = recs[d.first + local];
            const TriW& rw = recs_w[d.first + local];
            const double* vary = d.vary + (size_t)local * 24;
            double pc[3];
            TRGL_OWNER_BARYCENTRICS(r, rw, x, y, pc);
            const int kind = KIND == KIND_ANY ? d.kind : KIND;
            color = kind == TRGL_SHADER_PHONG ? frag_phong(d.u, ctex, vary, pc).bgra : frag_eye(d.u, ctex, vary, pc).bgra;
        }
    }
    if (KIND == KIND_ANY && user) return;
    store_pixel(fp, idx, color);
}

__device__ __forceinline__ unsigned long long sm64(unsigned long long& st) {
    unsigned long long z = (st += 0x9E3779B97F4A7C15ull);
    z = (z ^ (z >> 30)) * 0xBF58476D1CE4E5B9ull; z = (z ^ (z >> 27)) * 0x94D049BB133111EBull;
    return z ^ (z >> 31);
}
__device__ __forceinline__ double mk_double(unsigned long long mant, int exp2, bool neg) {
    unsigned long long bits = (mant & 0x000fffffffffffffull) | ((unsigned long long)(exp2 + 1023) << 52) | (neg ? 0x8000000000000000ull : 0ull);
    return __longlong_as_double((long long)bits);
}
__global__ void k_selftest_division(unsigned long long n_per_thread, unsigned long long seed, unsigned long long* mismatches) {
    unsigned long long st = seed + 0x1000003ull * (blockIdx.x * (unsigned long long)blockDim.x + threadIdx.x);
    unsigned long long bad = 0;
    for (unsigned long long it = 0; it < n_per_thread; ++it) {
        unsigned long long r0 = sm64(st), r1 = sm64(st), r2 = sm64(st);
        int mode = (int)(r2 & 7);
        int eb = (int)((r2 >> 8) % 440) - 40;
        int ea = (int)((r2 >> 24) % 700) - 350;
        unsigned long long mb = r1;
        if (mode == 1) mb = 0x000fffffffffffffull;
        if (mode == 2) mb = 0x000fffffffffffffull ^ (1ull << (r1 % 52));
        if (mode == 3) mb = 0;
        double uz = mk_double(mb, eb, true);
        double a = mk_double(r0, ea, (r2 >> 40) & 1);
        if (mode >= 4 && mode <= 6) {
            double q = mk_double(r0, ea - eb, (r2 >> 41) & 1);
            double half_ulp = mk_double(0, ea - eb - 53, false);
            a = __builtin_fma(uz, q, uz * half_ulp);
            if (mode == 5) a = __longlong_as_double(__double_as_longlong(a) + 1);
            if (mode == 6) a = __longlong_as_double(__double_as_longlong(a) - 1);
        }
        if (mode == 7) a = (r2 >> 42) & 1 ? 0.0 : -0.0;
        double ruz = 1.0 / uz;
        double ref = a / uz, got = div_by_uz(a, uz, ruz);
        if (__double_as_longlong(ref) != __double_as_longlong(got)) ++bad;
        if ((ref < 0) != (a > 0.0)) ++bad;
        if (((1.0 - ref) < 0) != (a < uz)) ++bad;
        double a2 = __longlong_as_double(__double_as_longlong(uz) + (long long)(r1 % 5) - 2);
        double ref2 = a2 / uz;
        if (__double_as_longlong(ref2) != __double_as_longlong(div_by_uz(a2, uz, ruz))) ++bad;
        if (((1.0 - ref2) < 0) != (a2 < uz)) ++bad;
    }
    if (bad) atomicAdd(mismatches, bad);
}

__global__ void k_selftest_sampler(const DevTexture* __restrict__ tex, int slot, const double* __restrict__ uv, unsigned long long n,
                                   uint8_t* __restrict__ out) {
    const unsigned long long i = blockIdx.x * (unsigned long long)blockDim.x + threadIdx.x;
    if (i >= n) return;
    const DevTexture* t = tex_slot(tex, slot);
    Color c = t ? tex_fetch(t, uv + 2 * i) : Color{ 0xffffffffu, 4 };
    for (int k = 0; k < 4; ++k) out[5 * i + k] = (uint8_t)(c.bgra >> (8 * k));
    out[5 * i + 4] = (uint8_t)c.bytespp;
}

__global__ __launch_bounds__(256) void k_make_items(FrameParams fp, const uint32_t* __restrict__ tile_start,
                                                    const uint32_t* __restrict__ tile_end,
                                                    uint4* __restrict__ items, uint32_t* __restrict__ n_items, TriRec* __restrict__ recs) {
    const int ntiles_strip = (fp.strip_ty1 - fp.strip_ty0) * fp.tiles_x;
    const int k = blockIdx.x * blockDim.x + threadIdx.x;
    if (k == 0 && fp.n_tris) {
        TriRec d;
        d.ax = d.ay = d.s0x = d.s0y = d.s1x = d.s1y = 0.0; d.c0 = __builtin_inf(); d.uz = 1.0; d.g1 = d.g2 = 0.0;
        d.ruz = 0.0; d.z0 = d.z1 = d.z2 = 0.0; d.bx0 = d.by0 = 1; d.bx1 = d.by1 = 0; d.color = 0; d.dl = 0;
        recs[fp.n_tris] = d;
    }
    uint32_t nb = 0, t = 0, rows = 0;
    uint32_t beg = 0, end = 0;
    bool clear_only = false;
    if (k < ntiles_strip) {
        t = (uint32_t)(fp.strip_ty0 * fp.tiles_x + k);
        beg = tile_start[t]; end = tile_end[t];
        const uint32_t n = end - beg;
        const int ty = (int)(t / (uint32_t)fp.tiles_x);
        if ((n || fp.init_from_clear) && tile_row_owned(fp, ty)) {
            if (n) {
                for (int r = 0; r < 4; ++r) {
                    const int y0 = ty * TRGL_TILE + 8 * r, y1 = y0 + 7;
                    if (y0 < fp.H && y1 >= fp.strip_y0 && y0 < fp.strip_y1) rows |= 1u << r;
                }
                nb = (uint32_t)__popc(rows);
            } else { clear_only = true; nb = 1; }
        }
    }
    uint32_t inc = nb;
    const int lane = threadIdx.x & 63;
    for (int o = 1; o < 64; o <<= 1) { const uint32_t v = __shfl_up(inc, o); if (lane >= o) inc += v; }
    const uint32_t total = __shfl(inc, 63);
    uint32_t base = 0;
    if (lane == 63 && total) base = atomicAdd(n_items, total);
    base = __shfl(base, 63) + inc - nb;
    if (clear_only) items[base] = make_uint4(t | TRGL_ITEM_CLEAR, 0u, 0u, 0u);
    else for (uint32_t r = 0; r < 4; ++r) if ((rows >> r) & 1u) items[base++] = make_uint4(t | (r << 24), beg, end, 0u);
}

constexpr int FOLD_BLOCKS = 32;
__global__ __launch_bounds__(1024) void k_fold_stats(DevStats* __restrict__ s, uint32_t* __restrict__ n_items,
                                                     const unsigned long long* __restrict__ item_stats) {
    __shared__ unsigned long long sh[3][16];
    __shared__ bool s_last;
    const uint32_t n = *n_items;
    unsigned long long fr = 0, kmin = ~0ull, kmax = 0ull;
    for (uint32_t i = blockIdx.x * blockDim.x + threadIdx.x; i < n; i += gridDim.x * blockDim.x) {
        const ulonglong2 a = reinterpret_cast<const ulonglong2*>(item_stats + (size_t)i * 4)[0];
        const unsigned long long c = item_stats[(size_t)i * 4 + 2];
        fr += a.x; kmin = a.y < kmin ? a.y : kmin; kmax = c > kmax ? c : kmax;
    }
    for (int o = 32; o; o >>= 1) {
        fr += __shfl_xor(fr, o);
        unsigned long long a = __shfl_xor(kmin, o); kmin = a < kmin ? a : kmin;
        unsigned long long b = __shfl_xor(kmax, o); kmax = b > kmax ? b : kmax;
    }
    const int w = threadIdx.x >> 6, lane = threadIdx.x & 63;
    if (lane == 0) { sh[0][w] = fr; sh[1][w] = kmin; sh[2][w] = kmax; }
    __syncthreads();
    if (threadIdx.x == 0) {
        for (int k = 1; k < (int)(blockDim.x >> 6); ++k) {
            fr += sh[0][k]; kmin = sh[1][k] < kmin ? sh[1][k] : kmin; kmax = sh[2][k] > kmax ? sh[2][k] : kmax;
        }
        if (fr) {
            atomicAdd(&s->fragments, fr);
            atomicMin(&s->zmin_key, kmin);
            atomicMax(&s->zmax_key, kmax);
        }
        __threadfence();
        s_last = atomicAdd(&n_items[1], 1u) == gridDim.x - 1;
    }
    __syncthreads();
    if (s_last && threadIdx.x == 0) {
        __threadfence();
        if (!s->zero_locked && (s->zero_pos_key != TRGL_ZERO_KEY_EMPTY || s->zero_neg_key != TRGL_ZERO_KEY_EMPTY)) {
            s->zero_sign = s->zero_neg_key < s->zero_pos_key ? 1u : 0u;
            s->zero_locked = 1u;
        }
        s->literal_tris = 0; s->large_tris = 0;
        s->zero_pos_key = TRGL_ZERO_KEY_EMPTY;
        s->zero_neg_key = TRGL_ZERO_KEY_EMPTY;
        n_items[0] = 0;
        n_items[1] = 0;
    }
}

}

namespace trgl {

void launch_selftest_division(hipStream_t s, unsigned long long n_per_thread, unsigned long long seed, unsigned long long* mismatches) {
    hipLaunchKernelGGL(k_selftest_division, dim3(1024), dim3(256), 0, s, n_per_thread, seed, mismatches);
}

void launch_selftest_sampler(hipStream_t s, const DevTexture* tex, int slot, const double* uv, unsigned long long n, uint8_t* out) {
    if (n) hipLaunchKernelGGL(k_selftest_sampler, dim3((unsigned)((n + 255) / 256)), dim3(256), 0, s, tex, slot, uv, n, out);
}

uint32_t owned_tiles(const FrameParams& fp) {
    if (fp.il_tiles == 0) return (uint32_t)((fp.strip_ty1 - fp.strip_ty0) * fp.tiles_x);
    return (uint32_t)(il_owned_below(fp, fp.tiles_y) * fp.tiles_x);
}

uint32_t raster_max_items(const FrameParams& fp) { return owned_tiles(fp) * 4u; }

void launch_raster(hipStream_t s, const FrameParams& fp, int kind , bool all_well_scaled,
                   const TriRec* recs, const TriW* recs_w, const uint32_t* vals, const uint16_t* bmask,
                   const uint32_t* tile_start, const uint32_t* tile_end, const DrawDesc* draws,
                   const DevTexture* tex, DevStats* stats, uint32_t max_items, uint4* items,
                   uint32_t* n_items, unsigned long long* item_stats, bool builtin_shade, const UserShade* user, int n_user,
                   hipFunction_t user_raster, hipEvent_t ev_before, hipEvent_t ev_after) {
    const int tiles = (fp.strip_ty1 - fp.strip_ty0) * fp.tiles_x;
    if (tiles <= 0 || max_items == 0) {
        if (ev_before) (void)hipEventRecord(ev_before, s);
        if (ev_after) (void)hipEventRecord(ev_after, s);
        hipLaunchKernelGGL(k_fold_stats, dim3(FOLD_BLOCKS), dim3(1024), 0, s, stats, n_items, item_stats);
        return;
    }
    hipLaunchKernelGGL(k_make_items, dim3((tiles + 255) / 256), dim3(256), 0, s, fp, tile_start, tile_end, items, n_items, const_cast<TriRec*>(recs));
    dim3 grid(((max_items + 7u) / 8u) * 8u);
    if (ev_before) (void)hipEventRecord(ev_before, s);
    if (user_raster) {
        FrameParams fpa = fp; const TriRec* a1 = recs; const TriW* a2 = recs_w; const uint32_t* a3 = vals; const uint16_t* a4 = bmask;
        const DrawDesc* a5 = draws; const DevTexture* a6 = tex; DevStats* a7 = stats; const uint4* a8 = items; const uint32_t* a9 = n_items;
        unsigned long long* a10 = item_stats;
        void* args[] = { &fpa, &a1, &a2, &a3, &a4, &a5, &a6, &a7, &a8, &a9, &a10 };
        (void)hipModuleLaunchKernel(user_raster, grid.x, 1, 1, 256, 1, 1, 0, s, args, nullptr);
        if (ev_after) (void)hipEventRecord(ev_after, s);
        hipLaunchKernelGGL(k_fold_stats, dim3(FOLD_BLOCKS), dim3(1024), 0, s, stats, n_items, item_stats);
        return;
    }
#define TRGL_LAUNCH_RASTER(...) hipLaunchKernelGGL((k_raster<__VA_ARGS__>), grid, dim3(256), 0, s, fp, recs, recs_w, vals, bmask, tile_start, tile_end, draws, stats, items, n_items, item_stats)
    switch (kind) {
    case TRGL_SHADER_FLAT:
        if (all_well_scaled) {
            if (fp.bpp == 3) TRGL_LAUNCH_RASTER(TRGL_SHADER_FLAT, 3, true);
            else if (fp.bpp == 4) TRGL_LAUNCH_RASTER(TRGL_SHADER_FLAT, 4, true);
            else TRGL_LAUNCH_RASTER(TRGL_SHADER_FLAT, 0, true);
        } else {
            TRGL_LAUNCH_RASTER(TRGL_SHADER_FLAT);
        }
        break;
    case TRGL_SHADER_GOURAUD: if (all_well_scaled) TRGL_LAUNCH_RASTER(TRGL_SHADER_GOURAUD, 0, true); else TRGL_LAUNCH_RASTER(TRGL_SHADER_GOURAUD); break;
    case TRGL_SHADER_PHONG:   if (all_well_scaled) TRGL_LAUNCH_RASTER(TRGL_SHADER_PHONG, 0, true); else TRGL_LAUNCH_RASTER(TRGL_SHADER_PHONG); break;
    case TRGL_SHADER_EYE:     if (all_well_scaled) TRGL_LAUNCH_RASTER(TRGL_SHADER_EYE, 0, true); else TRGL_LAUNCH_RASTER(TRGL_SHADER_EYE); break;
    case TRGL_SHADER_CHECKER: TRGL_LAUNCH_RASTER(TRGL_SHADER_CHECKER); break;
    default:                  TRGL_LAUNCH_RASTER(KIND_ANY); break;
    }
#undef TRGL_LAUNCH_RASTER
    if (ev_after) (void)hipEventRecord(ev_after, s);
    if (fp.idbuf && builtin_shade) {
#define TRGL_LAUNCH_SHADE(K) hipLaunchKernelGGL(k_shade<K>, dim3(max_items), dim3(256), 0, s, fp, recs, recs_w, draws, tex, items, n_items)
        if (kind == TRGL_SHADER_PHONG) TRGL_LAUNCH_SHADE(TRGL_SHADER_PHONG);
        else if (kind == TRGL_SHADER_EYE) TRGL_LAUNCH_SHADE(TRGL_SHADER_EYE);
        else TRGL_LAUNCH_SHADE(KIND_ANY);
#undef TRGL_LAUNCH_SHADE
    }
    for (int i = 0; i < n_user && fp.idbuf; ++i) {
        FrameParams fpa = fp; const TriRec* a1 = recs; const TriW* a2 = recs_w; const DrawDesc* a3 = draws; const DevTexture* a4 = tex;
        const uint4* a5 = items; const uint32_t* a6 = n_items; int a7 = user[i].kind;
        void* args[] = { &fpa, &a1, &a2, &a3, &a4, &a5, &a6, &a7 };
        (void)hipModuleLaunchKernel(user[i].fn, max_items, 1, 1, 256, 1, 1, 0, s, args, nullptr);
    }
    hipLaunchKernelGGL(k_fold_stats, dim3(FOLD_BLOCKS), dim3(1024), 0, s, stats, n_items, item_stats);
}

}
```

### tinyrenderder_amd/csrc/launch.h

```cpp
#pragma once
#include <hip/hip_runtime.h>
#include "trgl_device.h"

namespace trgl {

uint32_t setup_num_blocks(uint32_t n);
void launch_setup(hipStream_t s, const FrameParams& fp, const DrawDesc& draw, DrawDesc* draws_dev, int draw_idx, uint32_t n,
                  TriRec* recs, TriW* recs_w, uint32_t* cnt, uint2* tilebox, DevStats* stats, uint32_t* blk_sums, uint32_t blk_base);
void launch_chunk_spine(hipStream_t s, const uint32_t* blk_sums, uint32_t nblk, uint32_t* chunk_off, unsigned long long* total64, unsigned long long* host_copy,
                        void* zero, size_t zero_bytes);


void launch_expand(hipStream_t s, const FrameParams& fp, uint32_t first, uint32_t n, int tiles_x, const uint32_t* cnt, const uint32_t* blk_sums,
                   const uint32_t* chunk_off, uint32_t blk_base, const uint2* tilebox, void* keys, bool key16, uint32_t* vals, uint16_t* bmask,
                   const unsigned long long* pairs_total, uint32_t cap);

uint32_t radix_num_workers(uint32_t P);
void launch_radix_pass(hipStream_t s, const void* keys_in, const uint32_t* vals_in, const uint16_t* msk_in, void* keys_out,
                       uint32_t* vals_out, uint16_t* msk_out, bool key16, const unsigned long long* pairs_total, uint32_t cap, int shift, int bits,
                       uint32_t* hist, uint32_t* scan_tmp);

void launch_bounds(hipStream_t s, const void* keys, bool key16, const unsigned long long* pairs_total, uint32_t cap,
                   uint32_t* tile_start, uint32_t* tile_end);

uint32_t owned_tiles(const FrameParams& fp);
uint32_t raster_max_items(const FrameParams& fp);
struct UserShade { hipFunction_t fn; int kind; };
void launch_raster(hipStream_t s, const FrameParams& fp, int kind, bool all_well_scaled, const TriRec* recs, const TriW* recs_w,
                   const uint32_t* vals, const uint16_t* bmask,
                   const uint32_t* tile_start, const uint32_t* tile_end, const DrawDesc* draws,
                   const DevTexture* tex, DevStats* stats, uint32_t max_items, uint4* items,
                   uint32_t* n_items, unsigned long long* item_stats, bool builtin_shade, const UserShade* user, int n_user,
                   hipFunction_t user_raster,
                   hipEvent_t ev_before = nullptr, hipEvent_t ev_after = nullptr);

void launch_vertex_stage(hipStream_t s, const double mv[16], const double proj[16], const double* vertices, int stride,
                         const uint32_t* indices, uint32_t nfaces, double* clip, double* vary);
void launch_zimage(hipStream_t s, const double* zb, int W, int H, unsigned long long* keys2, uint8_t* out);
void launch_ssao(hipStream_t s, const double* zb, int W, int H, const double* dir_x, const double* dir_y, int ndir, int steps,
                 double radius, double threshold, double intensity, uint8_t* out);
void launch_composite(hipStream_t s, const uint8_t* fb, int bpp, const uint8_t* ao, int W, int H, uint8_t* out);

void launch_selftest_sampler(hipStream_t s, const DevTexture* tex, int slot, const double* uv, unsigned long long n, uint8_t* out);
void launch_selftest_division(hipStream_t s, unsigned long long n_per_thread, unsigned long long seed,
                              unsigned long long* mismatches);

}
```

### tinyrenderder_amd/csrc/trgl_api.cpp

```cpp
#include <hip/hip_runtime.h>
#include <dlfcn.h>

#include <cmath>
#include <cstdio>
#include <cstdlib>
#include <cstring>
#include <limits>
#include <new>
#include <string>
#include <vector>

#include "../../include/trgl.h"
#include "launch.h"
#include "trgl_device.h"
#include "user_shaders.h"
#include "../shim/trgl_image.h"
#include "../shim/trgl_obj.h"

using namespace trgl;

static thread_local std::string g_create_error;
void trgl::set_global_error(const std::string& msg) { g_create_error = msg; }

struct StageChunk { char* base; size_t cap, used; };
struct trgl_ctx;

static size_t headroom(size_t need) { return need + need / 4 + 1024; }
template <class T> struct DevBuf {
    T* p = nullptr;
    size_t cap = 0;
    DevBuf() = default;
    DevBuf(const DevBuf&) = delete;
    ~DevBuf() { if (p) (void)hipFree(p); }
    int alloc(trgl_ctx* c, size_t n);
    int grow(trgl_ctx* c, size_t need, size_t ncap) { return need <= cap ? TRGL_OK : alloc(c, ncap); }
    int grow(trgl_ctx* c, size_t need) { return grow(c, need, headroom(need)); }
};
static size_t pair_capacity(size_t need) {
    const size_t ncap = (headroom(need) + 3) & ~size_t(3);
    return ncap > 0xffffe000ull ? 0xffffe000ull : ncap;
}

struct PendingRaster { bool active = false; FrameParams fp; int flush_kind = 0; uint32_t cap = 0; int cur = 0; uint64_t N = 0;
                       bool builtin_shade = false; uint32_t user_kinds = 0; };
struct UserKind { hipModule_t mod; hipFunction_t fn; int K; bool may_discard; };

struct trgl_ctx {
    int device = 0;
    int num_cus = 256;
    int W = 0, H = 0, bpp = 0, tiles_x = 0, tiles_y = 0;
    hipStream_t stream = nullptr;
    hipStream_t own_stream = nullptr;
    DevBuf<uint8_t> fb;
    DevBuf<double> zb;
    double vp[16];
    bool clear_pending = true;
    uint32_t clear_color = 0xff000000u;
    double clear_z = std::numeric_limits<double>::infinity();
    int strip_y0 = 0, strip_y1 = 0;
    int il_tiles = 0, il_world = 1, il_rank = 0;

    DevTexture tex_host[TRGL_MAX_TEXTURES];
    DevBuf<DevTexture> tex_dev;

    std::vector<DrawDesc> draws;
    uint64_t queued_tris = 0;
    std::vector<StageChunk> stage;
    int stage_hold = 0;

    DevBuf<TriRec> recs; DevBuf<TriW> recs_w; DevBuf<uint32_t> cnt; DevBuf<uint2> tilebox;
    PendingRaster rp;
    hipEvent_t ev_pairs = nullptr;
    DevBuf<uint32_t> idbuf;
    DevBuf<uint8_t> pp_out;
    DevBuf<uint32_t> blk_sums;
    DevBuf<uint32_t> chunk_off;
    DevBuf<uint32_t> keys[2], vals[2]; DevBuf<uint16_t> bmask[2];
    DevBuf<uint32_t> hist, scan_tmp;
    DevBuf<uint32_t> tile_start;
    DevBuf<uint4> items; DevBuf<uint32_t> n_items;
    DevBuf<unsigned long long> item_stats;
    DevBuf<DrawDesc> draws_dev;
    DevBuf<DevStats> stats_dev;
    DevStats* stats_pinned = nullptr;

    uint64_t triangles_total = 0;
    uint64_t last_tris = 0, last_pairs = 0;

    bool profiling = false, events_pending = false;
    hipEvent_t ev[6] = { nullptr, nullptr, nullptr, nullptr, nullptr, nullptr };
    double phase_ms[TRGL_NUM_PHASES] = { 0, 0, 0, 0, 0 };
    uint64_t flushes_timed = 0;

    std::vector<UserKind> user;

    std::string err;

    uint32_t* tile_end() const { return tile_start.p + (size_t)tiles_x * tiles_y; }
};

#define HIPCHK(ctx, expr)                                                                      \
    do {                                                                                       \
        hipError_t e_ = (expr);                                                                \
        if (e_ != hipSuccess) {                                                                \
            (ctx)->err = std::string(#expr) + ": " + hipGetErrorString(e_);                    \
            return TRGL_E_HIP;                                                                 \
        }                                                                                      \
    } while (0)

#define CHKCTX(ctx) do { if (!(ctx)) return TRGL_E_INVALID; if (hipSetDevice((ctx)->device) != hipSuccess) return TRGL_E_HIP; } while (0)

template <class T> int DevBuf<T>::alloc(trgl_ctx* c, size_t n) {
    if (p) { HIPCHK(c, hipStreamSynchronize(c->stream)); HIPCHK(c, hipFree(p)); p = nullptr; cap = 0; }
    HIPCHK(c, hipMalloc((void**)&p, n * sizeof(T)));
    cap = n;
    return TRGL_OK;
}

struct StageHold { trgl_ctx* c; explicit StageHold(trgl_ctx* x) : c(x) { ++c->stage_hold; } ~StageHold() { --c->stage_hold; } };

static int fail(trgl_ctx* c, int code, const char* msg) { c->err = msg; return code; }

static int reset_dev_stats(trgl_ctx* c) {
    DevStats s;
    s.fragments = 0;
    s.zmin_key = zkey(std::numeric_limits<double>::infinity());
    s.zmax_key = zkey(-std::numeric_limits<double>::infinity());
    s.min_x = INT32_MAX; s.min_y = INT32_MAX; s.max_x = INT32_MIN; s.max_y = INT32_MIN;
    s.pairs_total = 0; s.literal_tris = 0; s.large_tris = 0;
    s.zero_pos_key = s.zero_neg_key = TRGL_ZERO_KEY_EMPTY;
    s.zero_locked = 0; s.zero_sign = 0;
    for (int k = 0; k < 16; ++k) s.dbg[k] = 0;
    *c->stats_pinned = s;
    HIPCHK(c, hipMemcpyAsync(c->stats_dev.p, c->stats_pinned, sizeof(DevStats), hipMemcpyHostToDevice, c->stream));
    HIPCHK(c, hipStreamSynchronize(c->stream));
    return TRGL_OK;
}

static int end_pending_raster(trgl_ctx* c) { return c->rp.active ? trgl_flush_end(c) : TRGL_OK; }
static int flush_queued(trgl_ctx* c) { return c->draws.empty() ? TRGL_OK : trgl_flush(c); }
static int flush_sync(trgl_ctx* c) {
    int r = trgl_flush(c); if (r) return r;
    HIPCHK(c, hipStreamSynchronize(c->stream));
    return TRGL_OK;
}

static int init_ctx(trgl_ctx* c) {
    const size_t npx = (size_t)c->W * c->H, ntiles = (size_t)c->tiles_x * c->tiles_y;
    HIPCHK(c, hipStreamCreateWithFlags(&c->own_stream, hipStreamNonBlocking));
    c->stream = c->own_stream;
    int r;
    if ((r = c->fb.alloc(c, npx * c->bpp)) || (r = c->zb.alloc(c, npx)) || (r = c->tex_dev.alloc(c, TRGL_MAX_TEXTURES))) return r;
    HIPCHK(c, hipMemset(c->tex_dev.p, 0, sizeof(c->tex_host)));
    if ((r = c->tile_start.alloc(c, ntiles * 2 + 4))) return r;
    if ((r = c->n_items.alloc(c, 2))) return r;
    HIPCHK(c, hipMemset(c->n_items.p, 0, 8));
    if ((r = c->draws_dev.alloc(c, TRGL_MAX_DRAWS)) || (r = c->stats_dev.alloc(c, 1))) return r;
    HIPCHK(c, hipHostMalloc((void**)&c->stats_pinned, sizeof(DevStats)));
    for (int i = 0; i < 6; ++i) HIPCHK(c, hipEventCreate(&c->ev[i]));
    HIPCHK(c, hipEventCreateWithFlags(&c->ev_pairs, hipEventDisableTiming));
    trgl_init_viewport(c, 0, 0, c->W, c->H);
    return reset_dev_stats(c);
}

extern "C" {

const char* trgl_last_error(const trgl_ctx* ctx) { return ctx ? ctx->err.c_str() : g_create_error.c_str(); }

int trgl_create(int device, int width, int height, int bpp, trgl_ctx** out) {
    if (!out || width <= 0 || height <= 0 || width > 65535 || height > 65535 || !(bpp == 1 || bpp == 3 || bpp == 4)) {
        g_create_error = "trgl_create: bad arguments (width/height in 1..65535, bpp in {1,3,4})";
        return TRGL_E_INVALID;
    }
    hipError_t e = hipSetDevice(device);
    if (e != hipSuccess) { g_create_error = std::string("hipSetDevice: ") + hipGetErrorString(e); return TRGL_E_HIP; }
    trgl_ctx* c = new trgl_ctx();
    c->device = device; c->W = width; c->H = height; c->bpp = bpp;
    c->tiles_x = (width + TRGL_TILE - 1) / TRGL_TILE;
    c->tiles_y = (height + TRGL_TILE - 1) / TRGL_TILE;
    c->strip_y0 = 0; c->strip_y1 = height;
    { int n = 0; if (hipDeviceGetAttribute(&n, hipDeviceAttributeMultiprocessorCount, device) == hipSuccess && n > 0) c->num_cus = n; }
    std::memset(c->tex_host, 0, sizeof(c->tex_host));
    if (int r = init_ctx(c)) { g_create_error = c->err; trgl_destroy(c); return r; }
    *out = c;
    return TRGL_OK;
}

int trgl_destroy(trgl_ctx* c) {
    if (!c) return TRGL_E_INVALID;
    (void)hipSetDevice(c->device);
    if (c->stream) (void)hipStreamSynchronize(c->stream);
    for (auto& s : c->stage) (void)hipFree(s.base);
    for (int i = 0; i < TRGL_MAX_TEXTURES; ++i) if (c->tex_host[i].data) (void)hipFree((void*)c->tex_host[i].data);
    if (c->stats_pinned) (void)hipHostFree(c->stats_pinned);
    for (int i = 0; i < 6; ++i) if (c->ev[i]) (void)hipEventDestroy(c->ev[i]);
    if (c->ev_pairs) (void)hipEventDestroy(c->ev_pairs);
    for (auto& u : c->user) (void)hipModuleUnload(u.mod);
    if (c->own_stream) (void)hipStreamDestroy(c->own_stream);
    delete c;
    return TRGL_OK;
}

int trgl_set_viewport(trgl_ctx* c, const double m[16]) {
    CHKCTX(c);
    int r = end_pending_raster(c); if (r) return r;
    if (!m) return fail(c, TRGL_E_INVALID, "trgl_set_viewport: null matrix");
    if (std::memcmp(c->vp, m, sizeof(c->vp)) != 0 && (r = flush_queued(c))) return r;
    std::memcpy(c->vp, m, sizeof(c->vp));
    return TRGL_OK;
}

int trgl_init_viewport(trgl_ctx* c, int x, int y, int w, int h) {
    if (!c) return TRGL_E_INVALID;
    double m[16];
    for (int r = 0; r < 4; ++r) for (int k = 0; k < 4; ++k) m[4 * r + k] = (r == k) ? 1.0 : 0.0;
    m[0] = w / 2.0; m[5] = h / 2.0; m[3] = x + w / 2.0; m[7] = y + h / 2.0; m[10] = 1.0; m[11] = 0.0;
    if (c->stream == nullptr || c->draws.empty()) { std::memcpy(c->vp, m, sizeof(m)); return TRGL_OK; }
    return trgl_set_viewport(c, m);
}

int trgl_clear(trgl_ctx* c, const uint8_t bgra[4], double z_clear) {
    CHKCTX(c);
    int r = end_pending_raster(c); if (r) return r;
    if ((r = flush_queued(c))) return r;
    static const uint8_t dflt[4] = { 0, 0, 0, 255 };
    const uint8_t* p = bgra ? bgra : dflt;
    c->clear_color = (uint32_t)p[0] | ((uint32_t)p[1] << 8) | ((uint32_t)p[2] << 16) | ((uint32_t)p[3] << 24);
    c->clear_z = z_clear;
    c->clear_pending = true;
    return TRGL_OK;
}

int trgl_upload_texture(trgl_ctx* c, int slot, const uint8_t* texels, int w, int h, int bpp) {
    CHKCTX(c);
    int r = end_pending_raster(c); if (r) return r;
    if (slot < 0 || slot >= TRGL_MAX_TEXTURES) return fail(c, TRGL_E_INVALID, "trgl_upload_texture: bad slot");
    if ((r = flush_queued(c))) return r;
    HIPCHK(c, hipStreamSynchronize(c->stream));
    if (c->tex_host[slot].data) { HIPCHK(c, hipFree((void*)c->tex_host[slot].data)); c->tex_host[slot] = DevTexture{ nullptr, 0, 0, 0, 0 }; }
    if (texels && w > 0 && h > 0) {
        if (!(bpp == 1 || bpp == 3 || bpp == 4)) return fail(c, TRGL_E_INVALID, "trgl_upload_texture: bpp must be 1, 3 or 4");
        uint8_t* d = nullptr; size_t bytes = (size_t)w * h * bpp;
        HIPCHK(c, hipMalloc((void**)&d, bytes + 8));
        HIPCHK(c, hipMemset(d + bytes, 0, 8));
        HIPCHK(c, hipMemcpy(d, texels, bytes, hipMemcpyHostToDevice));
        c->tex_host[slot] = DevTexture{ d, w, h, bpp, 0 };
    }
    HIPCHK(c, hipMemcpy(c->tex_dev.p, c->tex_host, sizeof(c->tex_host), hipMemcpyHostToDevice));
    return TRGL_OK;
}

int trgl_set_strip(trgl_ctx* c, int y0, int y1) {
    CHKCTX(c);
    int r = end_pending_raster(c); if (r) return r;
    if (y0 < 0 || y1 > c->H || y0 > y1) return fail(c, TRGL_E_INVALID, "trgl_set_strip: need 0 <= y0 <= y1 <= H");
    if ((r = flush_queued(c))) return r;
    c->strip_y0 = y0; c->strip_y1 = y1;
    c->il_tiles = 0; c->il_world = 1; c->il_rank = 0;
    return TRGL_OK;
}

int trgl_set_interleave(trgl_ctx* c, int band_rows, int rank, int world) {
    CHKCTX(c);
    int r = end_pending_raster(c); if (r) return r;
    if (band_rows <= 0 || band_rows % TRGL_TILE || world < 1 || rank < 0 || rank >= world)
        return fail(c, TRGL_E_INVALID, "trgl_set_interleave: band_rows must be a positive multiple of 32, 0 <= rank < world");
    if ((r = flush_queued(c))) return r;
    c->strip_y0 = 0; c->strip_y1 = c->H;
    c->il_tiles = world > 1 ? band_rows / TRGL_TILE : 0; c->il_world = world; c->il_rank = rank;
    return TRGL_OK;
}

static int vary_count(int kind) {
    switch (kind) {
    case TRGL_SHADER_GOURAUD: return TRGL_VARY_GOURAUD;
    case TRGL_SHADER_PHONG: return TRGL_VARY_PHONG;
    case TRGL_SHADER_EYE: return TRGL_VARY_EYE;
    case TRGL_SHADER_CHECKER: return TRGL_VARY_CHECKER;
    default: return 0;
    }
}

static int stage_alloc(trgl_ctx* c, size_t bytes, void** dev) {
    size_t need = (bytes + 255) & ~size_t(255);
    StageChunk* ch = nullptr;
    for (auto& s : c->stage) if (s.cap - s.used >= need) { ch = &s; break; }
    if (!ch) {
        StageChunk s; s.cap = need > (size_t(64) << 20) ? need : (size_t(64) << 20); s.used = 0; s.base = nullptr;
        HIPCHK(c, hipMalloc((void**)&s.base, s.cap));
        c->stage.push_back(s); ch = &c->stage.back();
    }
    *dev = ch->base + ch->used; ch->used += need;
    return TRGL_OK;
}
static int stage_copy(trgl_ctx* c, const void* src, size_t bytes, void** dev) {
    int r = stage_alloc(c, bytes, dev); if (r) return r;
    HIPCHK(c, hipMemcpy(*dev, src, bytes, hipMemcpyHostToDevice));
    return TRGL_OK;
}

static bool discarding_kind(const trgl_ctx* c, int kind) {
    return kind >= TRGL_SHADER_USER_FIRST && kind - TRGL_SHADER_USER_FIRST < (int)c->user.size() && c->user[kind - TRGL_SHADER_USER_FIRST].may_discard;
}

int trgl_draw(trgl_ctx* c, int kind, const trgl_uniforms* u, const double* clip, const double* vary,
              const uint32_t* colors, uint64_t n, int mem_kind) {
    CHKCTX(c);
    int r = end_pending_raster(c); if (r) return r;
    const bool user = kind >= TRGL_SHADER_USER_FIRST && kind - TRGL_SHADER_USER_FIRST < (int)c->user.size();
    if ((kind < 0 || kind >= TRGL_NUM_SHADERS) && !user) return fail(c, TRGL_E_INVALID, "trgl_draw: unknown shader kind");
    if (n == 0) return TRGL_OK;
    if (!clip) return fail(c, TRGL_E_INVALID, "trgl_draw: clip is null");
    int K = user ? c->user[kind - TRGL_SHADER_USER_FIRST].K : vary_count(kind);
    if (K && !vary) return fail(c, TRGL_E_INVALID, "trgl_draw: this shader kind needs varyings");
    if ((kind == TRGL_SHADER_PHONG || kind == TRGL_SHADER_EYE) && !u) return fail(c, TRGL_E_INVALID, "trgl_draw: PHONG/EYE need uniforms");
    if (kind == TRGL_SHADER_CHECKER && (!u || u->reserved < 1)) return fail(c, TRGL_E_INVALID, "trgl_draw: CHECKER needs uniforms with reserved = cells >= 1");
    if (mem_kind != TRGL_MEM_HOST && mem_kind != TRGL_MEM_DEVICE) return fail(c, TRGL_E_INVALID, "trgl_draw: bad mem_kind");
    if (c->queued_tris + n > 0xffffffffull && (r = trgl_flush(c))) return r;
    if (n > 0xffffffffull) return fail(c, TRGL_E_UNSUPPORTED, "trgl_draw: more than 2^32-1 triangles in one draw");

    const double* dclip = clip; const double* dvary = K ? vary : nullptr; const uint32_t* dcol = colors;
    StageHold hold(c);
    if (mem_kind == TRGL_MEM_HOST) {
        void* p = nullptr;
        if ((r = stage_copy(c, clip, n * 12 * sizeof(double), &p))) return r;
        dclip = (const double*)p;
        if (K) { if ((r = stage_copy(c, vary, n * K * sizeof(double), &p))) return r; dvary = (const double*)p; }
        if (colors) { if ((r = stage_copy(c, colors, n * sizeof(uint32_t), &p))) return r; dcol = (const uint32_t*)p; }
    }
    for (uint64_t done = 0; done < n;) {
        uint64_t m = n - done; if (m > TRGL_DRAW_MAX_TRIS) m = TRGL_DRAW_MAX_TRIS;
        const bool kind_cut = !c->draws.empty() && c->draws.back().kind != kind && (discarding_kind(c, kind) || discarding_kind(c, c->draws.back().kind));
        if ((c->draws.size() >= TRGL_MAX_DRAWS || c->queued_tris + m > TRGL_FLUSH_MAX_TRIS || kind_cut) && (r = trgl_flush(c))) return r;
        DrawDesc d; std::memset(&d, 0, sizeof(d));
        d.n = (uint32_t)m; d.first = (uint32_t)c->queued_tris; d.kind = kind; d.K = K;
        if (u) d.u = *u; else { d.u.tex_diffuse = d.u.tex_normal = d.u.tex_specular = -1; }
        d.clip = dclip + done * 12;
        d.vary = dvary ? dvary + done * K : nullptr;
        d.colors = dcol ? dcol + done : nullptr;
        c->draws.push_back(d);
        c->queued_tris += m;
        done += m;
    }
    return TRGL_OK;
}

int trgl_draw_indexed(trgl_ctx* c, int kind, const trgl_uniforms* u, const double projection[16], const double* vertices,
                      int stride, uint64_t n_vertices, const uint32_t* indices, uint64_t n_faces, int mem_kind) {
    CHKCTX(c);
    int r = end_pending_raster(c); if (r) return r;
    const bool user24 = kind >= TRGL_SHADER_USER_FIRST && kind - TRGL_SHADER_USER_FIRST < (int)c->user.size() &&
                        c->user[kind - TRGL_SHADER_USER_FIRST].K == TRGL_VARY_PHONG;
    if (kind != TRGL_SHADER_PHONG && kind != TRGL_SHADER_EYE && !user24)
        return fail(c, TRGL_E_INVALID, "trgl_draw_indexed: kind must be PHONG, EYE or a user kind registered with 24 varyings");
    if (!u || !projection || !vertices || !indices) return fail(c, TRGL_E_INVALID, "trgl_draw_indexed: null argument");
    if (stride < 8) return fail(c, TRGL_E_INVALID, "trgl_draw_indexed: vertex stride must be >= 8 doubles (pos3, normal3, uv2)");
    if (mem_kind != TRGL_MEM_HOST && mem_kind != TRGL_MEM_DEVICE) return fail(c, TRGL_E_INVALID, "trgl_draw_indexed: bad mem_kind");
    if (n_faces == 0) return TRGL_OK;
    if (n_faces > 0xffffffffull / 3) return fail(c, TRGL_E_UNSUPPORTED, "trgl_draw_indexed: too many faces in one call");
    const double* dv = vertices; const uint32_t* di = indices;
    void* p = nullptr;
    StageHold hold(c);
    if (mem_kind == TRGL_MEM_HOST) {
        for (uint64_t k = 0; k < 3 * n_faces; ++k)
            if (indices[k] >= n_vertices) return fail(c, TRGL_E_INVALID, "trgl_draw_indexed: index out of range");
        if ((r = stage_copy(c, vertices, n_vertices * (size_t)stride * sizeof(double), &p))) return r;
        dv = (const double*)p;
        if ((r = stage_copy(c, indices, 3 * n_faces * sizeof(uint32_t), &p))) return r;
        di = (const uint32_t*)p;
    }
    double* clip = nullptr; double* vary = nullptr;
    if ((r = stage_alloc(c, n_faces * 12 * sizeof(double), &p))) return r;
    clip = (double*)p;
    if ((r = stage_alloc(c, n_faces * 24 * sizeof(double), &p))) return r;
    vary = (double*)p;
    launch_vertex_stage(c->stream, u->model_view, projection, dv, stride, di, (uint32_t)n_faces, clip, vary);
    HIPCHK(c, hipGetLastError());
    return trgl_draw(c, kind, u, clip, vary, nullptr, n_faces, TRGL_MEM_DEVICE);
}

void trgl_ssao_defaults(trgl_ssao_params* p) {
    if (!p) return;
    p->num_directions = 8; p->steps_per_direction = 8; p->sample_radius = 16.0; p->occlusion_threshold = 1e-3; p->intensity = 0.35;
}

int trgl_postprocess(trgl_ctx* c, const trgl_ssao_params* params, uint8_t* zimg, uint8_t* ao, uint8_t* fin) {
    CHKCTX(c);
    trgl_ssao_params sp; trgl_ssao_defaults(&sp);
    if (params) sp = *params;
    if (sp.num_directions < 1 || sp.num_directions > 16 || sp.steps_per_direction < 1)
        return fail(c, TRGL_E_INVALID, "trgl_postprocess: 1..16 directions, >= 1 step");
    int r = flush_sync(c); if (r) return r;
    const size_t npx = (size_t)c->W * c->H;
    const size_t img = (npx * 3 + 15) & ~size_t(15);
    if ((r = c->pp_out.grow(c, img * 3 + 64))) return r;
    uint8_t* d_out = c->pp_out.p;
    unsigned long long* d_keys = reinterpret_cast<unsigned long long*>(d_out + img * 3);
    uint8_t* d_z = d_out; uint8_t* d_ao = d_out + img; uint8_t* d_fin = d_out + img * 2;
    hipStream_t s = c->stream;
    if (zimg) launch_zimage(s, c->zb.p, c->W, c->H, d_keys, d_z);
    if (ao || fin) {
        double dx[16], dy[16];
        for (int d = 0; d < sp.num_directions; ++d) {
            double angle = 2.0 * 3.14159265358979323846 * d / sp.num_directions;
            dx[d] = std::cos(angle); dy[d] = std::sin(angle);
        }
        launch_ssao(s, c->zb.p, c->W, c->H, dx, dy, sp.num_directions, sp.steps_per_direction, sp.sample_radius,
                    sp.occlusion_threshold, sp.intensity, d_ao);
    }
    if (fin) {
        if (c->bpp < 3) return fail(c, TRGL_E_UNSUPPORTED, "trgl_postprocess: composite needs an RGB(A) framebuffer");
        launch_composite(s, c->fb.p, c->bpp, d_ao, c->W, c->H, d_fin);
    }
    HIPCHK(c, hipGetLastError());
    if (zimg) HIPCHK(c, hipMemcpyAsync(zimg, d_z, npx * 3, hipMemcpyDeviceToHost, s));
    if (ao) HIPCHK(c, hipMemcpyAsync(ao, d_ao, npx * 3, hipMemcpyDeviceToHost, s));
    if (fin) HIPCHK(c, hipMemcpyAsync(fin, d_fin, npx * 3, hipMemcpyDeviceToHost, s));
    HIPCHK(c, hipStreamSynchronize(s));
    return TRGL_OK;
}

static int resolve_events(trgl_ctx* c) {
    if (!c->events_pending) return TRGL_OK;
    HIPCHK(c, hipEventSynchronize(c->ev[3]));
    float ms;
    HIPCHK(c, hipEventElapsedTime(&ms, c->ev[0], c->ev[1])); c->phase_ms[TRGL_PHASE_SETUP] += ms;
    HIPCHK(c, hipEventElapsedTime(&ms, c->ev[1], c->ev[2])); c->phase_ms[TRGL_PHASE_BIN] += ms;
    HIPCHK(c, hipEventElapsedTime(&ms, c->ev[2], c->ev[3])); c->phase_ms[TRGL_PHASE_RASTER] += ms;
    HIPCHK(c, hipEventElapsedTime(&ms, c->ev[0], c->ev[3])); c->phase_ms[TRGL_PHASE_TOTAL] += ms;
    HIPCHK(c, hipEventElapsedTime(&ms, c->ev[4], c->ev[5])); c->phase_ms[TRGL_PHASE_RASTER_KERNEL] += ms;
    c->flushes_timed++;
    c->events_pending = false;
    return TRGL_OK;
}

int trgl_flush(trgl_ctx* c) {
    CHKCTX(c);
    int r = trgl_flush_begin(c);
    return r ? r : trgl_flush_end(c);
}

static int queue_binning(trgl_ctx* c, const FrameParams& fp, uint32_t cap, int* cur_out) {
    hipStream_t s = c->stream;
    const size_t ntiles = (size_t)c->tiles_x * c->tiles_y;
    const unsigned long long* pairs_dev = &c->stats_dev.p->pairs_total;
    int r;
    uint32_t blk_base = 0;
    const bool key16 = ntiles <= 65536;
    for (auto& d : c->draws) {
        launch_expand(s, fp, d.first, d.n, c->tiles_x, c->cnt.p, c->blk_sums.p, c->chunk_off.p, blk_base, c->tilebox.p, c->keys[0].p, key16, c->vals[0].p,
                      c->bmask[0].p, pairs_dev, cap);
        blk_base += setup_num_blocks(d.n);
    }
    int key_bits = 1; while ((size_t(1) << key_bits) < ntiles) ++key_bits;
    int passes = (key_bits + 7) / 8;
    int bits_per = (key_bits + passes - 1) / passes;
    size_t hist_need = ((size_t)radix_num_workers(cap) << bits_per) + 16;
    if ((r = c->hist.grow(c, hist_need))) return r;
    if ((r = c->scan_tmp.grow(c, 256 + 16))) return r;
    int cur = 0;
    for (int ps = 0; ps < passes; ++ps) {
        launch_radix_pass(s, c->keys[cur].p, c->vals[cur].p, c->bmask[cur].p, c->keys[cur ^ 1].p, c->vals[cur ^ 1].p, c->bmask[cur ^ 1].p, key16, pairs_dev, cap,
                          ps * bits_per, bits_per, c->hist.p, c->scan_tmp.p);
        cur ^= 1;
    }
    launch_bounds(s, c->keys[cur].p, key16, pairs_dev, cap, c->tile_start.p, c->tile_end());
    *cur_out = cur;
    return TRGL_OK;
}

static int grow_pairs(trgl_ctx* c, size_t need) {
    const size_t ncap = pair_capacity(need);
    int r;
    for (int k = 0; k < 2; ++k)
        if ((r = c->keys[k].grow(c, need, ncap)) || (r = c->vals[k].grow(c, need, ncap)) || (r = c->bmask[k].grow(c, need, ncap))) return r;
    return TRGL_OK;
}

static FrameParams frame_params(const trgl_ctx* c) {
    FrameParams fp; std::memset(&fp, 0, sizeof(fp));
    fp.fb = c->fb.p; fp.zb = c->zb.p; fp.W = c->W; fp.H = c->H; fp.bpp = c->bpp;
    fp.tiles_x = c->tiles_x; fp.tiles_y = c->tiles_y;
    fp.strip_y0 = c->strip_y0; fp.strip_y1 = c->strip_y1;
    fp.strip_ty0 = c->strip_y0 / TRGL_TILE;
    fp.strip_ty1 = (c->strip_y1 + TRGL_TILE - 1) / TRGL_TILE;
    if (c->strip_y1 <= c->strip_y0) fp.strip_ty1 = fp.strip_ty0;
    fp.il_tiles = c->il_tiles; fp.il_world = c->il_world; fp.il_rank = c->il_rank;
    fp.init_from_clear = c->clear_pending ? 1 : 0;
    fp.n_tris = (uint32_t)c->queued_tris;
    fp.clear_color = c->clear_color; fp.clear_z = c->clear_z;
    std::memcpy(fp.vp, c->vp, sizeof(fp.vp));
    return fp;
}

int trgl_flush_begin(trgl_ctx* c) {
    CHKCTX(c);
    if (c->rp.active) return TRGL_OK;
    if (c->draws.empty() && !c->clear_pending) return TRGL_OK;
    int r;
    if ((r = resolve_events(c))) return r;
    const uint64_t N = c->queued_tris;
    const size_t ntiles = (size_t)c->tiles_x * c->tiles_y;
    hipStream_t s = c->stream;
    FrameParams fp = frame_params(c);

    int flush_kind = c->draws.empty() ? TRGL_SHADER_FLAT : c->draws[0].kind;
    for (auto& d : c->draws) if (d.kind != flush_kind) flush_kind = -1;
    bool builtin_shade = false;
    uint32_t user_kinds = 0;
    for (auto& d : c->draws) {
        if (d.kind == TRGL_SHADER_PHONG || d.kind == TRGL_SHADER_EYE) builtin_shade = true;
        if (d.kind >= TRGL_SHADER_USER_FIRST && !discarding_kind(c, d.kind)) user_kinds |= 1u << (d.kind - TRGL_SHADER_USER_FIRST);
        if (discarding_kind(c, d.kind) && d.kind != flush_kind) return fail(c, TRGL_E_STATE, "flush: a kind that may discard shares a flush with another kind");
    }
    if (builtin_shade || user_kinds) {
        if ((r = c->idbuf.grow(c, (size_t)c->W * c->H))) return r;
        fp.idbuf = c->idbuf.p;
    }

    if (c->profiling) HIPCHK(c, hipEventRecord(c->ev[0], s));
    uint32_t cap = 0;
    int cur = 0;
    if (N) {
        const size_t tcap = headroom(N);
        if ((r = c->recs.grow(c, N + 1, tcap)) || (r = c->recs_w.grow(c, N + 1, tcap)) || (r = c->cnt.grow(c, N + 1, tcap)) ||
            (r = c->tilebox.grow(c, N + 1, tcap))) return r;
        if (c->keys[0].cap == 0 && (r = grow_pairs(c, (size_t)2 * N + 4096))) return r;
        uint32_t nblk = 0;
        for (auto& d : c->draws) nblk += setup_num_blocks(d.n);
        if ((r = c->blk_sums.grow(c, (size_t)nblk + 16))) return r;
        if ((r = c->chunk_off.grow(c, (size_t)nblk / 16 + 16))) return r;
        {
            uint32_t blk_base = 0;
            for (size_t i = 0; i < c->draws.size(); ++i) {
                launch_setup(s, fp, c->draws[i], c->draws_dev.p, (int)i, c->draws[i].n, c->recs.p, c->recs_w.p, c->cnt.p, c->tilebox.p, c->stats_dev.p,
                             c->blk_sums.p, blk_base);
                blk_base += setup_num_blocks(c->draws[i].n);
            }
        }
        if (c->profiling) HIPCHK(c, hipEventRecord(c->ev[1], s));
        launch_chunk_spine(s, c->blk_sums.p, nblk, c->chunk_off.p, &c->stats_dev.p->pairs_total, &c->stats_pinned->pairs_total,
                           c->tile_start.p, (ntiles * 8 + 15) & ~size_t(15));
        HIPCHK(c, hipEventRecord(c->ev_pairs, s));
        cap = (uint32_t)c->keys[0].cap;
        if ((r = queue_binning(c, fp, cap, &cur))) return r;
    } else {
        if (c->profiling) HIPCHK(c, hipEventRecord(c->ev[1], s));
        HIPCHK(c, hipMemsetAsync(c->tile_start.p, 0, ntiles * 8, s));
    }
    if (c->profiling) HIPCHK(c, hipEventRecord(c->ev[2], s));
    c->rp.active = true; c->rp.fp = fp; c->rp.flush_kind = flush_kind; c->rp.cap = cap; c->rp.cur = cur; c->rp.N = N;
    c->rp.builtin_shade = builtin_shade; c->rp.user_kinds = user_kinds;
    return TRGL_OK;
}

int trgl_flush_end(trgl_ctx* c) {
    CHKCTX(c);
    if (!c->rp.active) return TRGL_OK;
    c->rp.active = false;
    int r;
    hipStream_t s = c->stream;
    FrameParams fp = c->rp.fp;
    const int flush_kind = c->rp.flush_kind;
    int cur = c->rp.cur;
    const uint64_t N = c->rp.N;
    uint32_t P = 0;
    if (N) {
        HIPCHK(c, hipEventSynchronize(c->ev_pairs));
        const unsigned long long P64 = c->stats_pinned->pairs_total;
        if (P64 > 0xffffe000ull) {
            c->draws.clear(); c->queued_tris = 0;
            return fail(c, TRGL_E_UNSUPPORTED, "flush: more than 2^32 triangle-tile pairs; submit in smaller batches");
        }
        P = (uint32_t)P64;
        if (P > c->rp.cap) {
            if ((r = grow_pairs(c, P))) return r;
            if ((r = queue_binning(c, fp, (uint32_t)c->keys[0].cap, &cur))) return r;
            if (c->profiling) HIPCHK(c, hipEventRecord(c->ev[2], s));
        }
    }
    const TriRec* recs_arg = c->recs.p ? c->recs.p : reinterpret_cast<const TriRec*>(c->tile_start.p);
    const uint32_t* vals_arg = (P && c->vals[cur].p) ? c->vals[cur].p : c->tile_start.p;
    const uint16_t* bmask_arg = (P && c->bmask[cur].p) ? c->bmask[cur].p : reinterpret_cast<const uint16_t*>(c->tile_start.p);
    const uint32_t max_items = raster_max_items(fp);
    if ((r = c->items.grow(c, (size_t)max_items + 64))) return r;
    if ((r = c->item_stats.grow(c, ((size_t)max_items + 64) * 4))) return r;
    const bool all_well_scaled = N == 0 || c->stats_pinned->literal_tris == 0;
    fp.zq_cull = (N != 0 && c->stats_pinned->large_tris != 0) ? 1 : 0;
    UserShade user[TRGL_MAX_USER_SHADERS];
    int n_user = 0;
    for (int i = 0; i < (int)c->user.size(); ++i)
        if (c->rp.user_kinds >> i & 1u) user[n_user++] = UserShade{ c->user[i].fn, TRGL_SHADER_USER_FIRST + i };
    const hipFunction_t user_raster = discarding_kind(c, flush_kind) ? c->user[flush_kind - TRGL_SHADER_USER_FIRST].fn : nullptr;
    launch_raster(s, fp, flush_kind, all_well_scaled, recs_arg, c->recs_w.p, vals_arg, bmask_arg, c->tile_start.p, c->tile_end(), c->draws_dev.p, c->tex_dev.p,
                  c->stats_dev.p, max_items, c->items.p, c->n_items.p, c->item_stats.p, c->rp.builtin_shade, user, n_user, user_raster,
                  c->profiling ? c->ev[4] : nullptr, c->profiling ? c->ev[5] : nullptr);
    if (c->profiling) { HIPCHK(c, hipEventRecord(c->ev[3], s)); c->events_pending = true; }
    HIPCHK(c, hipGetLastError());

    c->triangles_total += N;
    c->last_tris = N; c->last_pairs = P;
    c->clear_pending = false;
    bool had_stage = false;
    for (auto& ch : c->stage) if (ch.used) had_stage = true;
    c->draws.clear();
    c->queued_tris = 0;
    if (had_stage) {
        HIPCHK(c, hipStreamSynchronize(s));
        if (!c->stage_hold)
            for (auto& ch : c->stage) ch.used = 0;
    }
    return TRGL_OK;
}

int trgl_register_shader_ex(trgl_ctx* c, const char* source, int n_varyings, uint32_t flags, int* kind) {
    CHKCTX(c);
    if (!kind) return fail(c, TRGL_E_INVALID, "trgl_register_shader: kind is null");
    if (c->user.size() >= TRGL_MAX_USER_SHADERS) return fail(c, TRGL_E_INVALID, "trgl_register_shader: TRGL_MAX_USER_SHADERS already registered");
    std::string log;
    const std::vector<char>* code = nullptr;
    if (int r = user_shader_code(source, n_varyings, flags, &log, &code)) { c->err = "trgl_register_shader: " + log; return r; }
    const bool may_discard = (flags & TRGL_SHADER_MAY_DISCARD) != 0;
    UserKind u{ nullptr, nullptr, n_varyings, may_discard };
    HIPCHK(c, hipModuleLoadData(&u.mod, code->data()));
    const hipError_t e = hipModuleGetFunction(&u.fn, u.mod, may_discard ? USER_RASTER_KERNEL : USER_SHADE_KERNEL);
    if (e != hipSuccess) {
        (void)hipModuleUnload(u.mod);
        c->err = std::string("hipModuleGetFunction: ") + hipGetErrorString(e);
        return TRGL_E_HIP;
    }
    c->user.push_back(u);
    *kind = TRGL_SHADER_USER_FIRST + (int)c->user.size() - 1;
    return TRGL_OK;
}

int trgl_register_shader(trgl_ctx* c, const char* source, int n_varyings, int* kind) {
    return trgl_register_shader_ex(c, source, n_varyings, 0u, kind);
}

int trgl_sync(trgl_ctx* c) {
    CHKCTX(c);
    int r = end_pending_raster(c); if (r) return r;
    HIPCHK(c, hipStreamSynchronize(c->stream));
    return TRGL_OK;
}

int trgl_read_framebuffer(trgl_ctx* c, uint8_t* dst) {
    CHKCTX(c);
    if (!dst) return fail(c, TRGL_E_INVALID, "null destination");
    int r = flush_sync(c); if (r) return r;
    HIPCHK(c, hipMemcpy(dst, c->fb.p, (size_t)c->W * c->H * c->bpp, hipMemcpyDeviceToHost));
    return TRGL_OK;
}
int trgl_write_framebuffer(trgl_ctx* c, const uint8_t* src) {
    CHKCTX(c);
    if (!src) return fail(c, TRGL_E_INVALID, "null source");
    int r = flush_sync(c); if (r) return r;
    HIPCHK(c, hipMemcpy(c->fb.p, src, (size_t)c->W * c->H * c->bpp, hipMemcpyHostToDevice));
    return TRGL_OK;
}
int trgl_read_zbuffer(trgl_ctx* c, double* dst) {
    CHKCTX(c);
    if (!dst) return fail(c, TRGL_E_INVALID, "null destination");
    int r = flush_sync(c); if (r) return r;
    HIPCHK(c, hipMemcpy(dst, c->zb.p, (size_t)c->W * c->H * sizeof(double), hipMemcpyDeviceToHost));
    return TRGL_OK;
}
int trgl_write_zbuffer(trgl_ctx* c, const double* src) {
    CHKCTX(c);
    if (!src) return fail(c, TRGL_E_INVALID, "null source");
    int r = flush_sync(c); if (r) return r;
    HIPCHK(c, hipMemcpy(c->zb.p, src, (size_t)c->W * c->H * sizeof(double), hipMemcpyHostToDevice));
    return TRGL_OK;
}

int trgl_get_stats(trgl_ctx* c, trgl_stats* out) {
    CHKCTX(c);
    if (!out) return fail(c, TRGL_E_INVALID, "null stats");
    int r = flush_sync(c); if (r) return r;
    HIPCHK(c, hipMemcpy(c->stats_pinned, c->stats_dev.p, sizeof(DevStats), hipMemcpyDeviceToHost));
    const DevStats& s = *c->stats_pinned;
    out->triangles_rasterized = c->triangles_total;
    out->fragments_drawn = s.fragments;
    out->min_x = s.min_x; out->min_y = s.min_y; out->max_x = s.max_x; out->max_y = s.max_y;
    out->min_z = zkey_decode(s.zmin_key); out->max_z = zkey_decode(s.zmax_key);
    if (out->min_z == 0.0 && s.zero_locked) out->min_z = s.zero_sign ? -0.0 : 0.0;
    if (out->max_z == 0.0 && s.zero_locked) out->max_z = s.zero_sign ? -0.0 : 0.0;
    return TRGL_OK;
}

int trgl_reset_stats(trgl_ctx* c) {
    CHKCTX(c);
    int r = flush_sync(c); if (r) return r;
    c->triangles_total = 0;
    return reset_dev_stats(c);
}

int trgl_format_stats(const trgl_stats* s, char* buf, size_t buflen) {
    if (!s || !buf) return TRGL_E_INVALID;
    char lo[400], hi[400];
    if (std::isfinite(s->min_z)) std::snprintf(lo, sizeof lo, "%f", s->min_z); else std::snprintf(lo, sizeof lo, "inf");
    if (std::isfinite(s->max_z)) std::snprintf(hi, sizeof hi, "%f", s->max_z); else std::snprintf(hi, sizeof hi, "-inf");
    int n = std::snprintf(buf, buflen, "DEBUG: triangles=%llu fragments_drawn=%llu bbox=[%d,%d] - [%d,%d] z-range=[%s,%s]\n",
                          (unsigned long long)s->triangles_rasterized, (unsigned long long)s->fragments_drawn,
                          s->min_x, s->min_y, s->max_x, s->max_y, lo, hi);
    return (n < 0 || (size_t)n >= buflen) ? TRGL_E_INVALID : TRGL_OK;
}

void* trgl_framebuffer_device_ptr(trgl_ctx* c) { return c ? c->fb.p : nullptr; }
void* trgl_zbuffer_device_ptr(trgl_ctx* c) { return c ? c->zb.p : nullptr; }
void* trgl_stream(trgl_ctx* c) { return c ? (void*)c->stream : nullptr; }

int trgl_obj_load(const char* path, double** vertices, uint64_t* n_vertices, uint32_t** indices, uint64_t* n_faces) {
    if (!path || !vertices || !n_vertices || !indices || !n_faces) return TRGL_E_INVALID;
    trgl_obj::Mesh m;
    try {
        if (!trgl_obj::load(path, m)) { g_create_error = m.error; return TRGL_E_INVALID; }
    } catch (const std::bad_alloc&) {
        g_create_error = "trgl_obj_load: out of memory"; return TRGL_E_NOMEM;
    }
    *n_vertices = m.vertices.size() / 14; *n_faces = m.indices.size() / 3;
    *vertices = (double*)std::malloc(m.vertices.size() * sizeof(double) + 8);
    *indices = (uint32_t*)std::malloc(m.indices.size() * sizeof(uint32_t) + 8);
    if (!*vertices || !*indices) { std::free(*vertices); std::free(*indices); return TRGL_E_NOMEM; }
    std::memcpy(*vertices, m.vertices.data(), m.vertices.size() * sizeof(double));
    std::memcpy(*indices, m.indices.data(), m.indices.size() * sizeof(uint32_t));
    return TRGL_OK;
}
void trgl_obj_free(double* vertices, uint32_t* indices) { std::free(vertices); std::free(indices); }

size_t trgl_tga_max_size(int w, int h, int bpp) {
    if (w <= 0 || h <= 0 || bpp <= 0) return 18;
    return size_t(18) + size_t(w) * h * bpp + size_t(w) * h;
}

int trgl_tga_encode(const uint8_t* pixels, int w, int h, int bpp, int vflip, int rle, uint8_t* out, size_t* out_len) {
    if (!pixels || !out || !out_len || w <= 0 || h <= 0 || w > 65535 || h > 65535 || !(bpp == 1 || bpp == 3 || bpp == 4)) return TRGL_E_INVALID;
    try {
        TGAImage img(w, h, bpp);
        std::memcpy(img.buffer(), pixels, size_t(w) * h * bpp);
        std::vector<uint8_t> bytes = img.encode_tga(vflip != 0, rle != 0);
        std::memcpy(out, bytes.data(), bytes.size());
        *out_len = bytes.size();
    } catch (const std::bad_alloc&) {
        return TRGL_E_NOMEM;
    }
    return TRGL_OK;
}

int trgl_tga_info(const uint8_t* file, size_t size, int* width, int* height, int* bpp) {
    if (!file || !width || !height || !bpp || size < 18) return TRGL_E_INVALID;
    const int w = file[12] | (file[13] << 8), h = file[14] | (file[15] << 8), b = file[16] >> 3;
    if (w <= 0 || h <= 0 || (b != 1 && b != 3 && b != 4)) return TRGL_E_INVALID;
    if (!(file[2] == 2 || file[2] == 3 || file[2] == 10 || file[2] == 11)) return TRGL_E_INVALID;
    *width = w; *height = h; *bpp = b;
    return TRGL_OK;
}

int trgl_tga_decode(const uint8_t* file, size_t size, uint8_t* pixels) {
    if (!file || !pixels) return TRGL_E_INVALID;
    try {
        TGAImage img;
        if (!img.decode_tga(file, size)) return TRGL_E_INVALID;
        std::memcpy(pixels, img.buffer(), size_t(img.width()) * img.height() * img.bytespp());
    } catch (const std::bad_alloc&) {
        return TRGL_E_NOMEM;
    }
    return TRGL_OK;
}

int trgl_selftest_division(trgl_ctx* c, uint64_t samples, uint64_t seed, uint64_t* mismatches) {
    CHKCTX(c);
    if (!mismatches) return fail(c, TRGL_E_INVALID, "null mismatches");
    int r = trgl_flush(c); if (r) return r;
    DevBuf<unsigned long long> d;
    if ((r = d.alloc(c, 1))) return r;
    HIPCHK(c, hipMemsetAsync(d.p, 0, 8, c->stream));
    unsigned long long per_thread = (samples + 1024ull * 256 - 1) / (1024ull * 256);
    launch_selftest_division(c->stream, per_thread, seed, d.p);
    unsigned long long h = 0;
    HIPCHK(c, hipMemcpyAsync(&h, d.p, 8, hipMemcpyDeviceToHost, c->stream));
    HIPCHK(c, hipStreamSynchronize(c->stream));
    *mismatches = h;
    return TRGL_OK;
}

int trgl_selftest_sampler(trgl_ctx* c, int slot, const double* uv, uint64_t n, uint8_t* out) {
    CHKCTX(c);
    if (!uv || !out) return fail(c, TRGL_E_INVALID, "trgl_selftest_sampler: null argument");
    if (slot < 0 || slot >= TRGL_MAX_TEXTURES) return fail(c, TRGL_E_INVALID, "trgl_selftest_sampler: bad slot");
    int r = trgl_flush(c); if (r) return r;
    if (!n) return TRGL_OK;
    DevBuf<double> d_uv; DevBuf<uint8_t> d_out;
    if ((r = d_uv.alloc(c, n * 2)) || (r = d_out.alloc(c, n * 5))) return r;
    HIPCHK(c, hipMemcpyAsync(d_uv.p, uv, n * 16, hipMemcpyHostToDevice, c->stream));
    launch_selftest_sampler(c->stream, c->tex_dev.p, slot, d_uv.p, n, d_out.p);
    HIPCHK(c, hipMemcpyAsync(out, d_out.p, n * 5, hipMemcpyDeviceToHost, c->stream));
    HIPCHK(c, hipStreamSynchronize(c->stream));
    return TRGL_OK;
}

int trgl_set_stream(trgl_ctx* c, void* hip_stream, int use_own) {
    CHKCTX(c);
    int r = end_pending_raster(c); if (r) return r;
    if ((r = flush_queued(c))) return r;
    if ((r = resolve_events(c))) return r;
    HIPCHK(c, hipStreamSynchronize(c->stream));
    c->stream = use_own ? c->own_stream : (hipStream_t)hip_stream;
    return TRGL_OK;
}

int trgl_set_profiling(trgl_ctx* c, int on) {
    CHKCTX(c);
    int r = resolve_events(c); if (r) return r;
    c->profiling = on != 0;
    return TRGL_OK;
}
int trgl_get_phase_ms(trgl_ctx* c, double ms[TRGL_NUM_PHASES], uint64_t* flushes) {
    CHKCTX(c);
    int r = resolve_events(c); if (r) return r;
    if (ms) for (int i = 0; i < TRGL_NUM_PHASES; ++i) ms[i] = c->phase_ms[i];
    if (flushes) *flushes = c->flushes_timed;
    return TRGL_OK;
}
int trgl_reset_phase_ms(trgl_ctx* c) {
    CHKCTX(c);
    int r = resolve_events(c); if (r) return r;
    for (int i = 0; i < TRGL_NUM_PHASES; ++i) c->phase_ms[i] = 0;
    c->flushes_timed = 0;
    return TRGL_OK;
}
extern "C" int trgl_debug_counters(trgl_ctx* c, unsigned long long out[16]) {
    CHKCTX(c);
    int r = flush_sync(c); if (r) return r;
    HIPCHK(c, hipMemcpy(c->stats_pinned, c->stats_dev.p, sizeof(DevStats), hipMemcpyDeviceToHost));
    for (int k = 0; k < 16; ++k) out[k] = c->stats_pinned->dbg[k];
    return TRGL_OK;
}

}

namespace {
struct Rccl {
    struct Id { char b[128]; };
    void* lib = nullptr;
    int (*GetUniqueId)(void*) = nullptr;
    int (*CommInitRank)(void**, int, Id, int) = nullptr;
    int (*CommDestroy)(void*) = nullptr;
    int (*AllGather)(const void*, void*, size_t, int, void*, hipStream_t) = nullptr;
    int (*GroupStart)() = nullptr;
    int (*GroupEnd)() = nullptr;
    const char* (*GetErrorString)(int) = nullptr;
    bool ok = false;
};
Rccl& rccl() {
    static Rccl r;
    if (!r.lib) {
        r.lib = dlopen("librccl.so.1", RTLD_NOW | RTLD_GLOBAL);
        if (!r.lib) r.lib = dlopen("librccl.so", RTLD_NOW | RTLD_GLOBAL);
        if (r.lib) {
            r.GetUniqueId = reinterpret_cast<decltype(r.GetUniqueId)>(dlsym(r.lib, "ncclGetUniqueId"));
            r.CommInitRank = reinterpret_cast<decltype(r.CommInitRank)>(dlsym(r.lib, "ncclCommInitRank"));
            r.CommDestroy = reinterpret_cast<decltype(r.CommDestroy)>(dlsym(r.lib, "ncclCommDestroy"));
            r.AllGather = reinterpret_cast<decltype(r.AllGather)>(dlsym(r.lib, "ncclAllGather"));
            r.GroupStart = reinterpret_cast<decltype(r.GroupStart)>(dlsym(r.lib, "ncclGroupStart"));
            r.GroupEnd = reinterpret_cast<decltype(r.GroupEnd)>(dlsym(r.lib, "ncclGroupEnd"));
            r.GetErrorString = reinterpret_cast<decltype(r.GetErrorString)>(dlsym(r.lib, "ncclGetErrorString"));
            r.ok = r.GetUniqueId && r.CommInitRank && r.CommDestroy && r.AllGather && r.GroupStart && r.GroupEnd;
        }
    }
    return r;
}
std::string rccl_err(const char* what, int code) {
    Rccl& r = rccl();
    return std::string(what) + ": " + (r.GetErrorString ? r.GetErrorString(code) : "RCCL error") + " (" + std::to_string(code) + ")";
}
constexpr int NCCL_UINT8 = 1;
}

extern "C" {

int trgl_rccl_unique_id(uint8_t id[TRGL_RCCL_ID_BYTES]) {
    if (!id) return TRGL_E_INVALID;
    Rccl& r = rccl();
    if (!r.ok) { g_create_error = "librccl.so.1 could not be loaded"; return TRGL_E_UNSUPPORTED; }
    const int rc = r.GetUniqueId(id);
    if (rc) { g_create_error = rccl_err("ncclGetUniqueId", rc); return TRGL_E_HIP; }
    return TRGL_OK;
}
int trgl_rccl_comm_create(const uint8_t id[TRGL_RCCL_ID_BYTES], int rank, int world, int device, void** comm) {
    if (!id || !comm || world < 1 || rank < 0 || rank >= world) return TRGL_E_INVALID;
    Rccl& r = rccl();
    if (!r.ok) { g_create_error = "librccl.so.1 could not be loaded"; return TRGL_E_UNSUPPORTED; }
    if (hipSetDevice(device) != hipSuccess) { g_create_error = "hipSetDevice failed"; return TRGL_E_HIP; }
    Rccl::Id uid; std::memcpy(uid.b, id, 128);
    const int rc = r.CommInitRank(comm, world, uid, rank);
    if (rc) { g_create_error = rccl_err("ncclCommInitRank", rc); return TRGL_E_HIP; }
    return TRGL_OK;
}
int trgl_rccl_comm_destroy(void* comm) {
    if (!comm) return TRGL_E_INVALID;
    Rccl& r = rccl();
    if (!r.ok) return TRGL_E_UNSUPPORTED;
    return r.CommDestroy(comm) ? TRGL_E_HIP : TRGL_OK;
}

int trgl_gather(trgl_ctx* c, void* comm, int rank, int world, int with_z) {
    CHKCTX(c);
    if (!comm || world < 1 || rank < 0 || rank >= world) return fail(c, TRGL_E_INVALID, "trgl_gather: bad communicator / rank / world");
    Rccl& r = rccl();
    if (!r.ok) return fail(c, TRGL_E_UNSUPPORTED, "trgl_gather: librccl.so.1 could not be loaded");
    int fr = trgl_flush(c); if (fr) return fr;
    const size_t row_fb = (size_t)c->W * c->bpp, row_z = (size_t)c->W * sizeof(double);
    int rc = 0;
    if (c->il_tiles == 0) {
        if (c->H % world) return fail(c, TRGL_E_INVALID, "trgl_gather: the height is not divisible by the number of ranks (equal strips are required)");
        const int rows = c->H / world;
        if (c->strip_y0 != rank * rows || c->strip_y1 != (rank + 1) * rows)
            return fail(c, TRGL_E_STATE, "trgl_gather: this context's strip is not rows [rank * H / world, (rank + 1) * H / world)");
        if ((rc = r.GroupStart())) { c->err = rccl_err("ncclGroupStart", rc); return TRGL_E_HIP; }
        rc = r.AllGather(c->fb.p + (size_t)c->strip_y0 * row_fb, c->fb.p, (size_t)rows * row_fb, NCCL_UINT8, comm, c->stream);
        if (!rc && with_z) rc = r.AllGather(reinterpret_cast<uint8_t*>(c->zb.p) + (size_t)c->strip_y0 * row_z, c->zb.p, (size_t)rows * row_z, NCCL_UINT8, comm, c->stream);
        const int rc2 = r.GroupEnd();
        if (!rc) rc = rc2;
    } else {
        if (c->il_world != world || c->il_rank != rank) return fail(c, TRGL_E_STATE, "trgl_gather: rank / world differ from trgl_set_interleave");
        const int band = c->il_tiles * TRGL_TILE, period = band * world;
        if (c->H % period) return fail(c, TRGL_E_INVALID, "trgl_gather: the height is not a multiple of world * band_rows");
        if ((rc = r.GroupStart())) { c->err = rccl_err("ncclGroupStart", rc); return TRGL_E_HIP; }
        for (int p0 = 0; p0 < c->H && !rc; p0 += period) {
            const int y0 = p0 + rank * band;
            rc = r.AllGather(c->fb.p + (size_t)y0 * row_fb, c->fb.p + (size_t)p0 * row_fb, (size_t)band * row_fb, NCCL_UINT8, comm, c->stream);
            if (!rc && with_z) rc = r.AllGather(reinterpret_cast<uint8_t*>(c->zb.p) + (size_t)y0 * row_z, reinterpret_cast<uint8_t*>(c->zb.p) + (size_t)p0 * row_z,
                                                (size_t)band * row_z, NCCL_UINT8, comm, c->stream);
        }
        const int rc2 = r.GroupEnd();
        if (!rc) rc = rc2;
    }
    if (rc) { c->err = rccl_err("ncclAllGather", rc); return TRGL_E_HIP; }
    return TRGL_OK;
}

int trgl_get_last_flush_info(trgl_ctx* c, uint64_t* triangles, uint64_t* pairs, uint64_t* tiles) {
    if (!c) return TRGL_E_INVALID;
    if (triangles) *triangles = c->last_tris;
    if (pairs) *pairs = c->last_pairs;
    if (tiles) *tiles = (uint64_t)c->tiles_x * c->tiles_y;
    return TRGL_OK;
}

}
```

Baseline: 4.008 billion.

## Fold tile bounds into last radix scatter and pack block masks into keys

The binning pipeline drops the separate k_bounds kernel: the last radix scatter pass writes tile_start/tile_end directly, and chunk_spine now initialises start to ~0 and end to 0. For non-wide tile counts the 16-bit block mask is packed into the upper half of a 32-bit key, which removes the separate mask array from expand and scatter traffic. Expand now writes its staged output with aligned 16-byte vector stores. Scatter gains a wave-count template (4 or 8 waves chosen by capacity), so the block size depends on the workload. The raster kernel treats end<=beg as an empty tile. The aim is less binning memory traffic and one fewer launch, at the cost of heavier keys for the small-tile case and more template variants.

```diff
diff --git a/profiles/binning_bytes.py b/profiles/binning_bytes.py
--- /dev/null
+++ b/profiles/binning_bytes.py
@@ -0,0 +1,86 @@
+import argparse
+import csv
+import glob
+import re
+from collections import defaultdict
+
+BIN = ("k_chunk_spine", "k_expand", "k_radix_hist", "k_radix_scan_rows", "k_radix_scatter", "k_bounds", "k_make_items")
+
+
+def short(name):
+    m = re.search(r"k_radix_scatter<(?:\d+, )?(true|false), (true|false)>", name)
+    if m:
+        return "k_radix_scatter" + (" (last pass)" if m.group(2) == "true" else "")
+    for k in BIN + ("k_setup", "k_raster", "k_fold_stats"):
+        if k in name:
+            return k
+    return name.split("(")[0][:38]
+
+
+ap = argparse.ArgumentParser()
+ap.add_argument("--trace")
+ap.add_argument("--pmc", nargs="*", default=[])
+ap.add_argument("--pairs", type=int, required=True)
+ap.add_argument("--tris", type=int, required=True)
+ap.add_argument("--old", action="store_true")
+a = ap.parse_args()
+P, N = a.pairs, a.tris
+
+
+def binning(name):
+    return name.split(" ")[0] in BIN
+
+
+if a.trace:
+    acc = defaultdict(list)
+    for f in glob.glob(f"{a.trace}/**/*kernel_trace.csv", recursive=True):
+        for r in csv.DictReader(open(f)):
+            acc[short(r["Kernel_Name"])].append((int(r["End_Timestamp"]) - int(r["Start_Timestamp"])) / 1e3)
+    frames = len(acc["k_setup"])
+    print(f"== kernel trace: {frames} frames ==")
+    tot = 0.0
+    for n, v in sorted(acc.items(), key=lambda kv: -sum(kv[1])):
+        tot += sum(v) / frames if binning(n) else 0.0
+        print(f"  {n:38s} calls {len(v):4d}  avg {sum(v) / len(v):8.1f} us  median {sorted(v)[len(v) // 2]:8.1f} us  per frame {sum(v) / frames:8.1f} us")
+    print(f"  binning kernels per frame: {tot:.1f} us\n")
+
+if a.pmc:
+    cnt = defaultdict(lambda: defaultdict(list))
+    for d in a.pmc:
+        for f in glob.glob(f"{d}/**/*counter_collection.csv", recursive=True):
+            per = defaultdict(float)
+            for r in csv.DictReader(open(f)):
+                n = short(r["Kernel_Name"])
+                if binning(n):
+                    per[(n, r["Dispatch_Id"], r["Counter_Name"])] += float(r["Counter_Value"])
+            for (n, disp, c), v in per.items():
+                cnt[n][c].append(v)
+    per_frame = {"k_radix_hist": 2, "k_radix_scan_rows": 2, "k_radix_scatter": 2 if a.old else 1}
+    if a.old:
+        model = {"k_expand": (12 * N, 8 * P), "k_radix_hist": (2 * P, 0), "k_radix_scatter": (8 * P, 8 * P), "k_bounds": (2 * P, 0)}
+    else:
+        model = {"k_expand": (12 * N, 8 * P), "k_radix_hist": (4 * P, 0), "k_radix_scatter": (8 * P, 8 * P),
+                 "k_radix_scatter (last pass)": (8 * P, 6 * P)}
+    print("== PMC per dispatch (means) ==")
+    for n in sorted(cnt):
+        cs = cnt[n]
+        print(f"  {n:30s} " + "  ".join(f"{c}={sum(v) / len(v):.4g}" for c, v in sorted(cs.items())))
+        act, conf = sum(cs.get("SQ_LDS_IDX_ACTIVE", [0])), sum(cs.get("SQ_LDS_BANK_CONFLICT", [0]))
+        if act:
+            print(f"  {'':30s} SQ_LDS_BANK_CONFLICT / SQ_LDS_IDX_ACTIVE = {conf / act:.3f}")
+    print(f"\n== bytes per frame (P = {P} pairs, N = {N} triangles; MB = 1e6 B) ==")
+    print(f"  {'kernel':30s} {'x':>2s} {'read':>8s} {'model':>8s} {'write':>8s} {'model':>8s}")
+    tr = tw = mr = mw = 0.0
+    for n in sorted(cnt):
+        cs = cnt[n]
+        if "FETCH_SIZE" not in cs or "WRITE_SIZE" not in cs:
+            continue
+        k = per_frame.get(n, 1)
+        r = 2 * 1024 * sum(cs["FETCH_SIZE"]) / len(cs["FETCH_SIZE"]) * k
+        w = 1024 * sum(cs["WRITE_SIZE"]) / len(cs["WRITE_SIZE"]) * k
+        m_r, m_w = (x * k for x in model.get(n, (0, 0)))
+        tr += r; tw += w; mr += m_r; mw += m_w
+        print(f"  {n:30s} {k:2d} {r / 1e6:8.1f} {m_r / 1e6:8.1f} {w / 1e6:8.1f} {m_w / 1e6:8.1f}"
+              + (f"   read {100 * (r / m_r - 1):+.0f} %" if m_r else "") + (f", write {100 * (w / m_w - 1):+.0f} %" if m_w else ""))
+    print(f"  {'total':30s}    {tr / 1e6:8.1f} {mr / 1e6:8.1f} {tw / 1e6:8.1f} {mw / 1e6:8.1f}")
+    print(f"  measured {(tr + tw) / 1e6:.1f} MB against the model's {(mr + mw) / 1e6:.1f} MB: {100 * ((tr + tw) / (mr + mw) - 1):+.1f} %")
diff --git a/profiles/summarize_rocprof.py b/profiles/summarize_rocprof.py
--- a/profiles/summarize_rocprof.py
+++ b/profiles/summarize_rocprof.py
@@ -12,6 +12,9 @@
     m = re.search(r"k_raster<(\d)(?:, (\d))?(?:, (true|false))?>", name)
     if m:
         return "k_raster<" + ["flat", "gouraud", "phong", "eye", "checker", "any"][int(m.group(1))] + (", bpp " + m.group(2) if m.group(2) and m.group(2) != "0" else "") + (", all well scaled" if m.group(3) == "true" else "") + ">"
+    m = re.search(r"k_radix_scatter<(?:\d+, )?(true|false), (true|false)>", name)
+    if m:
+        return "k_radix_scatter" + (" (last pass)" if m.group(2) == "true" else "")
     m = re.search(r"k_shade<(\d)>", name)
     if m:
         return "k_shade<" + ["flat", "gouraud", "phong", "eye", "checker", "any"][int(m.group(1))] + ">"
diff --git a/tinyrenderder_amd/csrc/kernels_bin.hip b/tinyrenderder_amd/csrc/kernels_bin.hip
--- a/tinyrenderder_amd/csrc/kernels_bin.hip
+++ b/tinyrenderder_amd/csrc/kernels_bin.hip
@@ -224,9 +224,9 @@
 __global__ __launch_bounds__(SPINE_THREADS) void k_chunk_spine(const uint32_t* __restrict__ blk_sums, uint32_t nblk,
                                                                uint32_t* __restrict__ chunk_off,
                                                                unsigned long long* __restrict__ total64, unsigned long long* __restrict__ host_copy,
-                                                               uint4* __restrict__ zero16, uint32_t n_zero16) {
+                                                               uint4* __restrict__ bounds16, uint32_t n_half16) {
     __shared__ unsigned long long s_wave[SPINE_THREADS / 64];
-    for (uint32_t k = threadIdx.x; k < n_zero16; k += SPINE_THREADS) zero16[k] = make_uint4(0, 0, 0, 0);
+    for (uint32_t k = threadIdx.x; k < 2 * n_half16; k += SPINE_THREADS) bounds16[k] = k < n_half16 ? make_uint4(~0u, ~0u, ~0u, ~0u) : make_uint4(0, 0, 0, 0);
     const uint32_t nchunks = (nblk + EXPAND_CHUNK - 1) / EXPAND_CHUNK;
     const int lane = threadIdx.x & 63, w = threadIdx.x >> 6;
     unsigned long long running = 0;
@@ -267,16 +267,16 @@
     const uint32_t r0 = qy0 > 4 * ty ? qy0 - 4 * ty : 0u, r1 = qy1 < 4 * ty + 3 ? qy1 - 4 * ty : 3u;
     return (((2u << c1) - (1u << c0)) & 0xfu) * 0x1111u & ((0xffffu >> (12 - 4 * r1)) & (0xffffu << (4 * r0)));
 }
-template <typename K>
+template <bool WIDE>
 __global__ __launch_bounds__(256) void k_expand(FrameParams fp, uint32_t first, uint32_t n, int tiles_x, const uint32_t* __restrict__ cnt,
                                                 const uint32_t* __restrict__ blk_sums, const uint32_t* __restrict__ chunk_off,
                                                 uint32_t blk_base, const uint2* __restrict__ tilebox,
-                                                K* __restrict__ keys, uint32_t* __restrict__ vals, uint16_t* __restrict__ bmask,
+                                                uint32_t* __restrict__ keys, uint32_t* __restrict__ vals, uint16_t* __restrict__ bmask,
                                                 const unsigned long long* __restrict__ pairs_total, uint32_t cap) {
     __shared__ uint32_t smem[4];
-    __shared__ uint32_t s_v[EXPAND_STAGE];
-    __shared__ K s_k[EXPAND_STAGE];
-    __shared__ uint16_t s_m[EXPAND_STAGE];
+    __shared__ __attribute__((aligned(16))) uint32_t s_k[EXPAND_STAGE + 4];
+    __shared__ __attribute__((aligned(16))) uint32_t s_v[EXPAND_STAGE + 4];
+    __shared__ __attribute__((aligned(16))) uint16_t s_m[WIDE ? EXPAND_STAGE + 4 : 4];
     if (*pairs_total > cap) return;
     const uint32_t local = blockIdx.x * blockDim.x + threadIdx.x;
     const uint32_t i = first + local;
@@ -293,7 +293,13 @@
     uint32_t tot;
     const uint32_t o = block_excl_scan(c, smem, &tot);
     const bool staged = tot <= EXPAND_STAGE;
-    K* const kdst = keys + base; uint32_t* const vdst = vals + base; uint16_t* const mdst = bmask + base;
+    const uint32_t sh = base & 3u;
+    uint32_t* const kdst = keys + base; uint32_t* const vdst = vals + base; uint16_t* const mdst = bmask + base;
+    auto put = [&](uint32_t j, uint32_t key, uint32_t iz, uint32_t m) {
+        const uint32_t word = WIDE ? key : key | (m << 16);
+        if (staged) { s_k[sh + j] = word; s_v[sh + j] = iz; if (WIDE) s_m[sh + j] = (uint16_t)m; }
+        else { kdst[j] = word; vdst[j] = iz; if (WIDE) mdst[j] = (uint16_t)m; }
+    };
     constexpr uint32_t SMALL = 8;
     if (c && c <= SMALL) {
         const uint32_t qx0 = tb.x & 0x1fff, qy0 = (tb.x >> 16) & 0x1fff, qx1 = tb.y & 0x1fff, qy1 = (tb.y >> 16) & 0x1fff;
@@ -302,9 +308,7 @@
         uint32_t tx = tx0, row = 0;
         uint32_t ty = fp.il_tiles ? (uint32_t)il_nth_owned_from(fp, (int)ty0, 0) : ty0;
         for (uint32_t k = 0; k < c; ++k) {
-            const K key = (K)(ty * tiles_x + tx);
-            const uint16_t m = (uint16_t)tile_block_mask(tx, ty, qx0, qy0, qx1, qy1);
-            if (staged) { s_k[o + k] = key; s_v[o + k] = iz; s_m[o + k] = m; } else { kdst[o + k] = key; vdst[o + k] = iz; mdst[o + k] = m; }
+            put(o + k, ty * tiles_x + tx, iz, tile_block_mask(tx, ty, qx0, qy0, qx1, qy1));
             if (++tx > tx1) { tx = tx0; ++row; ty = fp.il_tiles ? (uint32_t)il_nth_owned_from(fp, (int)ty0, (int)row) : ty0 + row; }
         }
     }
@@ -321,35 +325,34 @@
         uint32_t wdt = tx1 - tx0 + 1;
         for (uint32_t k = lane; k < cc; k += 64) {
             uint32_t ty = fp.il_tiles ? (uint32_t)il_nth_owned_from(fp, (int)ty0, (int)(k / wdt)) : ty0 + k / wdt, tx = tx0 + k % wdt;
-            const K key = (K)(ty * tiles_x + tx);
-            const uint16_t m = (uint16_t)tile_block_mask(tx, ty, qx0, qy0, qx1, qy1);
-            if (staged) { s_k[oo + k] = key; s_v[oo + k] = ii; s_m[oo + k] = m; } else { kdst[oo + k] = key; vdst[oo + k] = ii; mdst[oo + k] = m; }
+            put(oo + k, ty * tiles_x + tx, ii, tile_block_mask(tx, ty, qx0, qy0, qx1, qy1));
         }
     }
     if (staged) {
         __syncthreads();
-        for (uint32_t j = threadIdx.x; j < tot; j += 256) { kdst[j] = s_k[j]; vdst[j] = s_v[j]; mdst[j] = s_m[j]; }
-    }
-}
-
-constexpr int RADIX_CHUNK = 4096;
-constexpr int RADIX_WAVE_CHUNK = RADIX_CHUNK / 4;
-constexpr int RADIX_ROUNDS = RADIX_WAVE_CHUNK / 64;
+        uint32_t* const kq = keys + (base - sh); uint32_t* const vq = vals + (base - sh); uint16_t* const mq = bmask + (base - sh);
+        const uint32_t end = sh + tot;
+        for (uint32_t q = threadIdx.x; 4 * q < end; q += 256) {
+            const uint32_t j0 = 4 * q;
+            if (j0 >= sh && j0 + 4 <= end) {
+                *reinterpret_cast<uint4*>(kq + j0) = *reinterpret_cast<const uint4*>(s_k + j0);
+                *reinterpret_cast<uint4*>(vq + j0) = *reinterpret_cast<const uint4*>(s_v + j0);
+                if (WIDE) *reinterpret_cast<uint2*>(mq + j0) = *reinterpret_cast<const uint2*>(s_m + j0);
+            } else {
+                for (uint32_t j = j0; j < j0 + 4; ++j)
+                    if (j >= sh && j < end) { kq[j] = s_k[j]; vq[j] = s_v[j]; if (WIDE) mq[j] = s_m[j]; }
+            }
+        }
+    }
+}
+
+constexpr int RADIX_ROUNDS = 16;
+constexpr int RADIX_WAVE_CHUNK = RADIX_ROUNDS * 64;
+constexpr uint32_t RADIX_BIG_CAP = 4u << 20;
 constexpr int RADIX_MAX_BITS = 8;
 
-template <typename K> __device__ __forceinline__ void load4(const K* __restrict__ keys, uint64_t p, uint32_t k[4]);
-template <> __device__ __forceinline__ void load4<uint32_t>(const uint32_t* __restrict__ keys, uint64_t p, uint32_t k[4]) {
-    const uint4 q = *reinterpret_cast<const uint4*>(keys + p);
-    k[0] = q.x; k[1] = q.y; k[2] = q.z; k[3] = q.w;
-}
-template <> __device__ __forceinline__ void load4<uint16_t>(const uint16_t* __restrict__ keys, uint64_t p, uint32_t k[4]) {
-    const uint2 q = *reinterpret_cast<const uint2*>(keys + p);
-    k[0] = q.x & 0xffffu; k[1] = q.x >> 16; k[2] = q.y & 0xffffu; k[3] = q.y >> 16;
-}
-
-template <typename K>
-__global__ __launch_bounds__(256) void k_radix_hist(const K* __restrict__ keys, const unsigned long long* __restrict__ pairs_total,
-                                                    uint32_t cap, int shift, int bits,
+__global__ __launch_bounds__(256) void k_radix_hist(const uint32_t* __restrict__ keys, const unsigned long long* __restrict__ pairs_total,
+                                                    uint32_t cap, int shift, int bits, uint32_t chunk,
                                                     uint32_t nblocks, uint32_t* __restrict__ hist) {
     __shared__ uint32_t s_cnt[1 << RADIX_MAX_BITS];
     const unsigned long long P64 = *pairs_total;
@@ -357,13 +360,13 @@
     const uint32_t nb = 1u << bits, mask = nb - 1;
     for (uint32_t b = threadIdx.x; b < nb; b += 256) s_cnt[b] = 0;
     __syncthreads();
-    const uint64_t beg = (uint64_t)blockIdx.x * RADIX_CHUNK;
-    uint64_t end = beg + RADIX_CHUNK; if (end > P) end = P;
+    const uint64_t beg = (uint64_t)blockIdx.x * chunk;
+    uint64_t end = beg + chunk; if (end > P) end = P;
     for (uint64_t p = beg + 4u * threadIdx.x; p < end; p += 1024) {
-        uint32_t k[4];
-        load4<K>(keys, p, k);
-#pragma unroll
-        for (int q = 0; q < 4; ++q) if (p + q < end) atomicAdd(&s_cnt[(k[q] >> shift) & mask], 1u);
+        const uint4 q = *reinterpret_cast<const uint4*>(keys + p);
+        const uint32_t k[4] = { q.x, q.y, q.z, q.w };
+#pragma unroll
+        for (int j = 0; j < 4; ++j) if (p + j < end) atomicAdd(&s_cnt[(k[j] >> shift) & mask], 1u);
     }
     __syncthreads();
     for (uint32_t b = threadIdx.x; b < nb; b += 256) hist[(size_t)b * nblocks + blockIdx.x] = s_cnt[b];
@@ -396,26 +399,30 @@
     if (threadIdx.x == 0) totals[blockIdx.x] = running;
 }
 
-template <typename K>
-__global__ __launch_bounds__(256) void k_radix_scatter(const K* __restrict__ keys_in, const uint32_t* __restrict__ vals_in,
-                                                       const uint16_t* __restrict__ msk_in,
-                                                       const unsigned long long* __restrict__ pairs_total, uint32_t cap,
-                                                       int shift, int bits, uint32_t nblocks,
-                                                       const uint32_t* __restrict__ base, const uint32_t* __restrict__ totals,
-                                                       K* __restrict__ keys_out, uint32_t* __restrict__ vals_out, uint16_t* __restrict__ msk_out) {
-    __shared__ uint32_t s_cnt[4][1 << RADIX_MAX_BITS];
+template <int RADIX_WAVES, bool WIDE, bool LAST>
+__global__ __launch_bounds__(RADIX_WAVES * 64) void k_radix_scatter(const uint32_t* __restrict__ keys_in, const uint32_t* __restrict__ vals_in,
+                                                                 const uint16_t* __restrict__ msk_in,
+                                                                 const unsigned long long* __restrict__ pairs_total, uint32_t cap,
+                                                                 int shift, int bits, uint32_t nblocks,
+                                                                 const uint32_t* __restrict__ base, const uint32_t* __restrict__ totals,
+                                                                 uint32_t* __restrict__ keys_out, uint32_t* __restrict__ vals_out,
+                                                                 uint16_t* __restrict__ msk_out,
+                                                                 uint32_t* __restrict__ tile_start, uint32_t* __restrict__ tile_end) {
+    constexpr int RADIX_THREADS = RADIX_WAVES * 64, RADIX_CHUNK = RADIX_WAVES * RADIX_WAVE_CHUNK;
+    __shared__ uint32_t s_cnt[RADIX_WAVES][1 << RADIX_MAX_BITS];
     __shared__ uint32_t s_start[1 << RADIX_MAX_BITS];
     __shared__ uint32_t s_gbase[1 << RADIX_MAX_BITS];
     __shared__ uint32_t s_val[RADIX_CHUNK];
-    __shared__ K s_key[RADIX_CHUNK];
-    __shared__ uint16_t s_msk[RADIX_CHUNK];
+    __shared__ uint32_t s_key[RADIX_CHUNK];
+    __shared__ uint16_t s_msk[WIDE ? RADIX_CHUNK : 2];
     const int w = threadIdx.x >> 6, lane = threadIdx.x & 63;
     const unsigned long long P64 = *pairs_total;
     const uint32_t P = P64 > cap ? 0u : (uint32_t)P64;
     if ((uint64_t)blockIdx.x * RADIX_CHUNK >= P) return;
     const uint32_t nb = 1u << bits, mask = nb - 1;
-    for (uint32_t b = threadIdx.x; b < nb; b += 256) {
-        s_cnt[0][b] = 0; s_cnt[1][b] = 0; s_cnt[2][b] = 0; s_cnt[3][b] = 0;
+    for (uint32_t b = threadIdx.x; b < nb; b += RADIX_THREADS) {
+#pragma unroll
+        for (int ww = 0; ww < RADIX_WAVES; ++ww) s_cnt[ww][b] = 0;
         s_gbase[b] = base[(size_t)b * nblocks + blockIdx.x];
     }
     if (w == 0) {
@@ -429,7 +436,7 @@
         for (int q = 0; q < 4; ++q) { const uint32_t d = lane * 4 + q; if (d < nb) s_start[d] = ex; ex += tot[q]; }
     }
     __syncthreads();
-    for (uint32_t b = threadIdx.x; b < nb; b += 256) s_gbase[b] += s_start[b];
+    for (uint32_t b = threadIdx.x; b < nb; b += RADIX_THREADS) s_gbase[b] += s_start[b];
     __syncthreads();
     const uint64_t cbeg = (uint64_t)blockIdx.x * RADIX_CHUNK;
     uint64_t cend = cbeg + RADIX_CHUNK; if (cend > P) cend = P;
@@ -438,12 +445,13 @@
     const unsigned long long lt = (1ull << lane) - 1ull;
 
     uint32_t k[RADIX_ROUNDS], v[RADIX_ROUNDS], rk[RADIX_ROUNDS];
-    uint16_t mk[RADIX_ROUNDS];
+    uint16_t mk[WIDE ? RADIX_ROUNDS : 1];
 #pragma unroll
     for (int r = 0; r < RADIX_ROUNDS; ++r) {
         const uint64_t p = wbeg + (uint64_t)r * 64 + lane;
         const bool act = p < cend;
-        k[r] = act ? (uint32_t)keys_in[p] : 0; v[r] = act ? vals_in[p] : 0; mk[r] = act ? msk_in[p] : (uint16_t)0;
+        k[r] = act ? keys_in[p] : 0; v[r] = act ? vals_in[p] : 0;
+        if (WIDE) mk[WIDE ? r : 0] = act ? msk_in[p] : (uint16_t)0;
     }
 #pragma unroll
     for (int r = 0; r < RADIX_ROUNDS; ++r) {
@@ -467,7 +475,12 @@
 #pragma unroll
         for (int q = 0; q < 4; ++q) {
             const uint32_t d = lane * 4 + q;
-            tot[q] = d < nb ? s_cnt[0][d] + s_cnt[1][d] + s_cnt[2][d] + s_cnt[3][d] : 0;
+            uint32_t t = 0;
+            if (d < nb) {
+#pragma unroll
+                for (int ww = 0; ww < RADIX_WAVES; ++ww) t += s_cnt[ww][d];
+            }
+            tot[q] = t;
             run += tot[q];
         }
         uint32_t inc = run;
@@ -477,10 +490,10 @@
         for (int q = 0; q < 4; ++q) { const uint32_t d = lane * 4 + q; if (d < nb) s_start[d] = ex; ex += tot[q]; }
     }
     __syncthreads();
-    for (uint32_t d = threadIdx.x; d < nb; d += 256) {
+    for (uint32_t d = threadIdx.x; d < nb; d += RADIX_THREADS) {
         uint32_t run = s_start[d];
 #pragma unroll
-        for (int ww = 0; ww < 4; ++ww) { const uint32_t c = s_cnt[ww][d]; s_cnt[ww][d] = run; run += c; }
+        for (int ww = 0; ww < RADIX_WAVES; ++ww) { const uint32_t c = s_cnt[ww][d]; s_cnt[ww][d] = run; run += c; }
     }
     __syncthreads();
 #pragma unroll
@@ -488,38 +501,26 @@
         if (wbeg + (uint64_t)r * 64 + lane < cend) {
             const uint32_t dgt = (k[r] >> shift) & mask;
             const uint32_t lp = s_cnt[w][dgt] + rk[r];
-            s_key[lp] = (K)k[r]; s_val[lp] = v[r]; s_msk[lp] = mk[r];
-        }
-    }
-    __syncthreads();
-    for (uint32_t i = threadIdx.x; i < n_chunk; i += 256) {
-        const uint32_t key = s_key[i];
-        const uint32_t dgt = (key >> shift) & mask;
+            s_key[lp] = k[r]; s_val[lp] = v[r];
+            if (WIDE) s_msk[lp] = mk[WIDE ? r : 0];
+        }
+    }
+    __syncthreads();
+    constexpr uint32_t KEY_MASK = WIDE ? 0xffffffffu : 0xffffu;
+    for (uint32_t i = threadIdx.x; i < n_chunk; i += RADIX_THREADS) {
+        const uint32_t word = s_key[i];
+        const uint32_t dgt = (word >> shift) & mask;
         const uint32_t dst = s_gbase[dgt] + (i - s_start[dgt]);
-        keys_out[dst] = (K)key; vals_out[dst] = s_val[i]; msk_out[dst] = s_msk[i];
-    }
-}
-
-template <typename K>
-__global__ __launch_bounds__(256) void k_bounds(const K* __restrict__ keys, const unsigned long long* __restrict__ pairs_total, uint32_t cap,
-                                                uint32_t* __restrict__ tile_start, uint32_t* __restrict__ tile_end) {
-    const unsigned long long P64 = *pairs_total;
-    const uint32_t P = P64 > cap ? 0u : (uint32_t)P64;
-    const uint32_t p0 = (blockIdx.x * blockDim.x + threadIdx.x) * 4u;
-    if (p0 >= P) return;
-    uint32_t k[4];
-    load4<K>(keys, p0, k);
-    uint32_t prev = p0 ? (uint32_t)keys[p0 - 1] : 0u;
-    const uint32_t after = (p0 + 4 < P) ? (uint32_t)keys[p0 + 4] : 0u;
-#pragma unroll
-    for (int i = 0; i < 4; ++i) {
-        const uint32_t p = p0 + (uint32_t)i;
-        if (p < P) {
-            const uint32_t next = i < 3 ? k[i + 1] : after;
-            if (p == 0 || prev != k[i]) tile_start[k[i]] = p;
-            if (p == P - 1 || next != k[i]) tile_end[k[i]] = p + 1;
-        }
-        prev = k[i];
+        vals_out[dst] = s_val[i];
+        if (!LAST) {
+            keys_out[dst] = word;
+            if (WIDE) msk_out[dst] = s_msk[i];
+        } else {
+            msk_out[dst] = WIDE ? s_msk[i] : (uint16_t)(word >> 16);
+            const uint32_t key = word & KEY_MASK;
+            if (i == 0 || (s_key[i - 1] & KEY_MASK) != key) atomicMin(&tile_start[key], dst);
+            if (i + 1 == n_chunk || (s_key[i + 1] & KEY_MASK) != key) atomicMax(&tile_end[key], dst + 1);
+        }
     }
 }
 
@@ -537,47 +538,48 @@
 }
 
 void launch_chunk_spine(hipStream_t s, const uint32_t* blk_sums, uint32_t nblk, uint32_t* chunk_off, unsigned long long* total64, unsigned long long* host_copy,
-                        void* zero, size_t zero_bytes) {
-    hipLaunchKernelGGL(k_chunk_spine, dim3(1), dim3(SPINE_THREADS), 0, s, blk_sums, nblk, chunk_off, total64, host_copy, (uint4*)zero, (uint32_t)(zero_bytes / 16));
+                        uint32_t* tile_bounds, size_t half_words) {
+    hipLaunchKernelGGL(k_chunk_spine, dim3(1), dim3(SPINE_THREADS), 0, s, blk_sums, nblk, chunk_off, total64, host_copy, (uint4*)tile_bounds,
+                       (uint32_t)(half_words / 4));
 }
 
 void launch_expand(hipStream_t s, const FrameParams& fp, uint32_t first, uint32_t n, int tiles_x, const uint32_t* cnt, const uint32_t* blk_sums,
-                   const uint32_t* chunk_off, uint32_t blk_base, const uint2* tilebox, void* keys, bool key16, uint32_t* vals, uint16_t* bmask,
+                   const uint32_t* chunk_off, uint32_t blk_base, const uint2* tilebox, uint32_t* keys, bool wide, uint32_t* vals, uint16_t* bmask,
                    const unsigned long long* pairs_total, uint32_t cap) {
     if (!n) return;
-    if (key16)
-        hipLaunchKernelGGL(k_expand<uint16_t>, dim3(setup_num_blocks(n)), dim3(SETUP_THREADS), 0, s, fp, first, n, tiles_x, cnt, blk_sums, chunk_off,
-                           blk_base, tilebox, (uint16_t*)keys, vals, bmask, pairs_total, cap);
+    if (wide)
+        hipLaunchKernelGGL(k_expand<true>, dim3(setup_num_blocks(n)), dim3(SETUP_THREADS), 0, s, fp, first, n, tiles_x, cnt, blk_sums, chunk_off,
+                           blk_base, tilebox, keys, vals, bmask, pairs_total, cap);
     else
-        hipLaunchKernelGGL(k_expand<uint32_t>, dim3(setup_num_blocks(n)), dim3(SETUP_THREADS), 0, s, fp, first, n, tiles_x, cnt, blk_sums, chunk_off,
-                           blk_base, tilebox, (uint32_t*)keys, vals, bmask, pairs_total, cap);
-}
-
-uint32_t radix_num_workers(uint32_t P) { return (uint32_t)(((uint64_t)P + RADIX_CHUNK - 1) / RADIX_CHUNK); }
-
-template <typename K>
-static void radix_pass_t(hipStream_t s, const K* keys_in, const uint32_t* vals_in, const uint16_t* msk_in, K* keys_out, uint32_t* vals_out, uint16_t* msk_out,
-                         const unsigned long long* pairs_total, uint32_t cap, int shift, int bits, uint32_t* hist, uint32_t* scan_tmp) {
-    uint32_t nblk = radix_num_workers(cap);
-    hipLaunchKernelGGL(k_radix_hist<K>, dim3(nblk), dim3(256), 0, s, keys_in, pairs_total, cap, shift, bits, nblk, hist);
-    hipLaunchKernelGGL(k_radix_scan_rows, dim3(1u << bits), dim3(ROWSCAN_THREADS), 0, s, hist, nblk, scan_tmp);
-    hipLaunchKernelGGL(k_radix_scatter<K>, dim3(nblk), dim3(256), 0, s, keys_in, vals_in, msk_in, pairs_total, cap, shift, bits, nblk, hist, scan_tmp,
-                       keys_out, vals_out, msk_out);
-}
-
-void launch_radix_pass(hipStream_t s, const void* keys_in, const uint32_t* vals_in, const uint16_t* msk_in, void* keys_out,
-                       uint32_t* vals_out, uint16_t* msk_out, bool key16, const unsigned long long* pairs_total, uint32_t cap, int shift, int bits,
+        hipLaunchKernelGGL(k_expand<false>, dim3(setup_num_blocks(n)), dim3(SETUP_THREADS), 0, s, fp, first, n, tiles_x, cnt, blk_sums, chunk_off,
+                           blk_base, tilebox, keys, vals, bmask, pairs_total, cap);
+}
+
+static uint32_t radix_waves(uint32_t cap) { return cap >= RADIX_BIG_CAP ? 8u : 4u; }
+uint32_t radix_num_workers(uint32_t cap) { const uint64_t chunk = radix_waves(cap) * RADIX_WAVE_CHUNK; return (uint32_t)((cap + chunk - 1) / chunk); }
+
+template <int WAVES, bool WIDE, bool LAST>
+static void radix_pass_t(hipStream_t s, const RadixPass& ps, const unsigned long long* pairs_total, uint32_t cap, uint32_t* hist, uint32_t* scan_tmp) {
+    const uint32_t nblk = radix_num_workers(cap);
+    hipLaunchKernelGGL(k_radix_hist, dim3(nblk), dim3(256), 0, s, ps.keys_in, pairs_total, cap, ps.shift, ps.bits, (uint32_t)(WAVES * RADIX_WAVE_CHUNK),
+                       nblk, hist);
+    hipLaunchKernelGGL(k_radix_scan_rows, dim3(1u << ps.bits), dim3(ROWSCAN_THREADS), 0, s, hist, nblk, scan_tmp);
+    hipLaunchKernelGGL((k_radix_scatter<WAVES, WIDE, LAST>), dim3(nblk), dim3(WAVES * 64), 0, s, ps.keys_in, ps.vals_in, ps.msk_in, pairs_total, cap,
+                       ps.shift, ps.bits, nblk, hist, scan_tmp, ps.keys_out, ps.vals_out, ps.msk_out, ps.tile_start, ps.tile_end);
+}
+
+template <int WAVES>
+static void radix_pass_w(hipStream_t s, const RadixPass& ps, bool wide, bool last, const unsigned long long* pairs_total, uint32_t cap,
+                         uint32_t* hist, uint32_t* scan_tmp) {
+    if (wide) { if (last) radix_pass_t<WAVES, true, true>(s, ps, pairs_total, cap, hist, scan_tmp); else radix_pass_t<WAVES, true, false>(s, ps, pairs_total, cap, hist, scan_tmp); }
+    else { if (last) radix_pass_t<WAVES, false, true>(s, ps, pairs_total, cap, hist, scan_tmp); else radix_pass_t<WAVES, false, false>(s, ps, pairs_total, cap, hist, scan_tmp); }
+}
+
+void launch_radix_pass(hipStream_t s, const RadixPass& ps, bool wide, bool last, const unsigned long long* pairs_total, uint32_t cap,
                        uint32_t* hist, uint32_t* scan_tmp) {
     if (!cap) return;
-    if (key16) radix_pass_t<uint16_t>(s, (const uint16_t*)keys_in, vals_in, msk_in, (uint16_t*)keys_out, vals_out, msk_out, pairs_total, cap, shift, bits, hist, scan_tmp);
-    else radix_pass_t<uint32_t>(s, (const uint32_t*)keys_in, vals_in, msk_in, (uint32_t*)keys_out, vals_out, msk_out, pairs_total, cap, shift, bits, hist, scan_tmp);
-}
-
-void launch_bounds(hipStream_t s, const void* keys, bool key16, const unsigned long long* pairs_total, uint32_t cap,
-                   uint32_t* tile_start, uint32_t* tile_end) {
-    if (!cap) return;
-    if (key16) hipLaunchKernelGGL(k_bounds<uint16_t>, dim3((unsigned)(((uint64_t)cap + 1023) / 1024)), dim3(256), 0, s, (const uint16_t*)keys, pairs_total, cap, tile_start, tile_end);
-    else hipLaunchKernelGGL(k_bounds<uint32_t>, dim3((unsigned)(((uint64_t)cap + 1023) / 1024)), dim3(256), 0, s, (const uint32_t*)keys, pairs_total, cap, tile_start, tile_end);
-}
-
-}
+    if (radix_waves(cap) == 8) radix_pass_w<8>(s, ps, wide, last, pairs_total, cap, hist, scan_tmp);
+    else radix_pass_w<4>(s, ps, wide, last, pairs_total, cap, hist, scan_tmp);
+}
+
+}
diff --git a/tinyrenderder_amd/csrc/kernels_raster.hip b/tinyrenderder_amd/csrc/kernels_raster.hip
--- a/tinyrenderder_amd/csrc/kernels_raster.hip
+++ b/tinyrenderder_amd/csrc/kernels_raster.hip
@@ -818,6 +818,7 @@
     if (k < ntiles_strip) {
         t = (uint32_t)(fp.strip_ty0 * fp.tiles_x + k);
         beg = tile_start[t]; end = tile_end[t];
+        if (end <= beg) beg = end = 0;
         const uint32_t n = end - beg;
         const int ty = (int)(t / (uint32_t)fp.tiles_x);
         if ((n || fp.init_from_clear) && tile_row_owned(fp, ty)) {
diff --git a/tinyrenderder_amd/csrc/launch.h b/tinyrenderder_amd/csrc/launch.h
--- a/tinyrenderder_amd/csrc/launch.h
+++ b/tinyrenderder_amd/csrc/launch.h
@@ -8,20 +8,22 @@
 void launch_setup(hipStream_t s, const FrameParams& fp, const DrawDesc& draw, DrawDesc* draws_dev, int draw_idx, uint32_t n,
                   TriRec* recs, TriW* recs_w, uint32_t* cnt, uint2* tilebox, DevStats* stats, uint32_t* blk_sums, uint32_t blk_base);
 void launch_chunk_spine(hipStream_t s, const uint32_t* blk_sums, uint32_t nblk, uint32_t* chunk_off, unsigned long long* total64, unsigned long long* host_copy,
-                        void* zero, size_t zero_bytes);
+                        uint32_t* tile_bounds, size_t half_words);
 
 
 void launch_expand(hipStream_t s, const FrameParams& fp, uint32_t first, uint32_t n, int tiles_x, const uint32_t* cnt, const uint32_t* blk_sums,
-                   const uint32_t* chunk_off, uint32_t blk_base, const uint2* tilebox, void* keys, bool key16, uint32_t* vals, uint16_t* bmask,
+                   const uint32_t* chunk_off, uint32_t blk_base, const uint2* tilebox, uint32_t* keys, bool wide, uint32_t* vals, uint16_t* bmask,
                    const unsigned long long* pairs_total, uint32_t cap);
 
-uint32_t radix_num_workers(uint32_t P);
-void launch_radix_pass(hipStream_t s, const void* keys_in, const uint32_t* vals_in, const uint16_t* msk_in, void* keys_out,
-                       uint32_t* vals_out, uint16_t* msk_out, bool key16, const unsigned long long* pairs_total, uint32_t cap, int shift, int bits,
+uint32_t radix_num_workers(uint32_t cap);
+struct RadixPass {
+    const uint32_t* keys_in; const uint32_t* vals_in; const uint16_t* msk_in;
+    uint32_t* keys_out; uint32_t* vals_out; uint16_t* msk_out;
+    uint32_t* tile_start; uint32_t* tile_end;
+    int shift, bits;
+};
+void launch_radix_pass(hipStream_t s, const RadixPass& ps, bool wide, bool last, const unsigned long long* pairs_total, uint32_t cap,
                        uint32_t* hist, uint32_t* scan_tmp);
-
-void launch_bounds(hipStream_t s, const void* keys, bool key16, const unsigned long long* pairs_total, uint32_t cap,
-                   uint32_t* tile_start, uint32_t* tile_end);
 
 uint32_t owned_tiles(const FrameParams& fp);
 uint32_t raster_max_items(const FrameParams& fp);
diff --git a/tinyrenderder_amd/csrc/trgl_api.cpp b/tinyrenderder_amd/csrc/trgl_api.cpp
--- a/tinyrenderder_amd/csrc/trgl_api.cpp
+++ b/tinyrenderder_amd/csrc/trgl_api.cpp
@@ -96,7 +96,8 @@
 
     std::string err;
 
-    uint32_t* tile_end() const { return tile_start.p + (size_t)tiles_x * tiles_y; }
+    size_t bounds_half() const { return ((size_t)tiles_x * tiles_y + 3) & ~size_t(3); }
+    uint32_t* tile_end() const { return tile_start.p + bounds_half(); }
 };
 
 #define HIPCHK(ctx, expr)                                                                      \
@@ -146,13 +147,13 @@
 }
 
 static int init_ctx(trgl_ctx* c) {
-    const size_t npx = (size_t)c->W * c->H, ntiles = (size_t)c->tiles_x * c->tiles_y;
+    const size_t npx = (size_t)c->W * c->H;
     HIPCHK(c, hipStreamCreateWithFlags(&c->own_stream, hipStreamNonBlocking));
     c->stream = c->own_stream;
     int r;
     if ((r = c->fb.alloc(c, npx * c->bpp)) || (r = c->zb.alloc(c, npx)) || (r = c->tex_dev.alloc(c, TRGL_MAX_TEXTURES))) return r;
     HIPCHK(c, hipMemset(c->tex_dev.p, 0, sizeof(c->tex_host)));
-    if ((r = c->tile_start.alloc(c, ntiles * 2 + 4))) return r;
+    if ((r = c->tile_start.alloc(c, c->bounds_half() * 2 + 4))) return r;
     if ((r = c->n_items.alloc(c, 2))) return r;
     HIPCHK(c, hipMemset(c->n_items.p, 0, 8));
     if ((r = c->draws_dev.alloc(c, TRGL_MAX_DRAWS)) || (r = c->stats_dev.alloc(c, 1))) return r;
@@ -446,9 +447,9 @@
     const unsigned long long* pairs_dev = &c->stats_dev.p->pairs_total;
     int r;
     uint32_t blk_base = 0;
-    const bool key16 = ntiles <= 65536;
+    const bool wide = ntiles > 65536;
     for (auto& d : c->draws) {
-        launch_expand(s, fp, d.first, d.n, c->tiles_x, c->cnt.p, c->blk_sums.p, c->chunk_off.p, blk_base, c->tilebox.p, c->keys[0].p, key16, c->vals[0].p,
+        launch_expand(s, fp, d.first, d.n, c->tiles_x, c->cnt.p, c->blk_sums.p, c->chunk_off.p, blk_base, c->tilebox.p, c->keys[0].p, wide, c->vals[0].p,
                       c->bmask[0].p, pairs_dev, cap);
         blk_base += setup_num_blocks(d.n);
     }
@@ -460,11 +461,11 @@
     if ((r = c->scan_tmp.grow(c, 256 + 16))) return r;
     int cur = 0;
     for (int ps = 0; ps < passes; ++ps) {
-        launch_radix_pass(s, c->keys[cur].p, c->vals[cur].p, c->bmask[cur].p, c->keys[cur ^ 1].p, c->vals[cur ^ 1].p, c->bmask[cur ^ 1].p, key16, pairs_dev, cap,
-                          ps * bits_per, bits_per, c->hist.p, c->scan_tmp.p);
+        const RadixPass rp{ c->keys[cur].p, c->vals[cur].p, c->bmask[cur].p, c->keys[cur ^ 1].p, c->vals[cur ^ 1].p, c->bmask[cur ^ 1].p,
+                            c->tile_start.p, c->tile_end(), ps * bits_per, bits_per };
+        launch_radix_pass(s, rp, wide, ps == passes - 1, pairs_dev, cap, c->hist.p, c->scan_tmp.p);
         cur ^= 1;
     }
-    launch_bounds(s, c->keys[cur].p, key16, pairs_dev, cap, c->tile_start.p, c->tile_end());
     *cur_out = cur;
     return TRGL_OK;
 }
@@ -500,7 +501,6 @@
     int r;
     if ((r = resolve_events(c))) return r;
     const uint64_t N = c->queued_tris;
-    const size_t ntiles = (size_t)c->tiles_x * c->tiles_y;
     hipStream_t s = c->stream;
     FrameParams fp = frame_params(c);
 
@@ -540,13 +540,13 @@
         }
         if (c->profiling) HIPCHK(c, hipEventRecord(c->ev[1], s));
         launch_chunk_spine(s, c->blk_sums.p, nblk, c->chunk_off.p, &c->stats_dev.p->pairs_total, &c->stats_pinned->pairs_total,
-                           c->tile_start.p, (ntiles * 8 + 15) & ~size_t(15));
+                           c->tile_start.p, c->bounds_half());
         HIPCHK(c, hipEventRecord(c->ev_pairs, s));
         cap = (uint32_t)c->keys[0].cap;
         if ((r = queue_binning(c, fp, cap, &cur))) return r;
     } else {
         if (c->profiling) HIPCHK(c, hipEventRecord(c->ev[1], s));
-        HIPCHK(c, hipMemsetAsync(c->tile_start.p, 0, ntiles * 8, s));
+        HIPCHK(c, hipMemsetAsync(c->tile_start.p, 0, c->bounds_half() * 8, s));
     }
     if (c->profiling) HIPCHK(c, hipEventRecord(c->ev[2], s));
     c->rp.active = true; c->rp.fp = fp; c->rp.flush_kind = flush_kind; c->rp.cap = cap; c->rp.cur = cur; c->rp.N = N;
```

Result: faster. 4.090 billion (median of 6 runs) (+2.0%).
